# oleg-savchenko/jax_nbody_emulator_with_dj

Hardware: AMD Instinct MI355X
Metric: voxels/sec (disp+vel) on 512^3 box, ndiv=4 (higher is better)
Workload: dtype f32-equivalent: f16x3 split MFMA (3 f16 MFMAs per product, f32 accumulate)

## Files before the change

### include/nbe.h

```cpp
#ifndef NBE_H
#define NBE_H

#include <stddef.h>
#include <stdint.h>

#ifdef __cplusplus
extern "C" {
#endif

typedef struct nbe_ctx nbe_ctx;

typedef void (*nbe_progress_cb)(int done, int total, void* user);

typedef struct nbe_layer_desc {
    const char* block;
    const char* layer;
    int cout, cin, k;
    const float* weight;
    const float* bias;
    const float* style_weight;
    const float* style_bias;
    const float* dweight;
} nbe_layer_desc;

// ... 172 lines not shown
                          double tail_slope, double tail_intercept, double boxsize, double scale, uint64_t seed, int flags,
                          int max_blocks, void* stream);
int nbe_spectrum_colour(void* spectrum, int64_t n, const void* k_table, const void* pk_table, int ntable,
                        double tail_slope, double tail_intercept, double boxsize, double scale, void* stream);
int nbe_gaussian_filter(void* spectrum, int64_t n, double sigma_over_L, void* stream);
int nbe_block_average(const void* src, int64_t n_in, void* dst, int64_t n_out, void* stream);
int nbe_trilinear_upsample(const void* src, int64_t n_in, void* dst, int64_t n_out, void* stream);

#define NBE_VELOCITY_BITS 20
#define NBE_VELOCITY_SUMS 6
int nbe_velocity_words(const void* velocity, int dtype, int lattice, int64_t count, int exponent, const void* sorted,
                       int max_blocks, void* words, void* stream);
int nbe_pair_velocity(const void* sortedA, const void* keysA, const void* wordsA, int64_t countA, const void* sortedB,
                      const void* keysB, const void* wordsB, int64_t countB, int ncell, const int64_t* thresholds, int nbins,
                      int max_blocks, void* sums, void* stream);
int nbe_pair_velocity_form(const void* sortedA, const void* keysA, const void* wordsA, int64_t countA, const void* sortedB,
                           const void* keysB, const void* wordsB, int64_t countB, int ncell, const int64_t* thresholds,
                           int nbins, int max_blocks, int form, void* sums, void* stream);
int nbe_halo_velocity_profiles(const void* sortedA, const void* keysA, const void* wordsA, int64_t countA, const void* sortedB,
                               const void* keysB, const void* wordsB, int64_t countB, int ncell, const int64_t* thresholds,
                               int nbins, int max_blocks, void* sums, void* stream);
int nbe_halo_velocity_profiles_form(const void* sortedA, const void* keysA, const void* wordsA, int64_t countA,
                                    const void* sortedB, const void* keysB, const void* wordsB, int64_t countB, int ncell,
                                    const int64_t* thresholds, int nbins, int max_blocks, int form, void* sums, void* stream);

#define NBE_PROFILE_WAVE_CENTRES 4096
#define NBE_PROFILE_WAVE_BELOW 3000
int nbe_halo_profiles(const void* sortedA, const void* keysA, int64_t countA, const void* sortedB, const void* keysB,
                      int64_t countB, int ncell, const int64_t* thresholds, int nbins, int max_blocks, void* counts,
                      void* stream);
int nbe_halo_profiles_form(const void* sortedA, const void* keysA, int64_t countA, const void* sortedB, const void* keysB,
                           int64_t countB, int ncell, const int64_t* thresholds, int nbins, int max_blocks, int form,
                           void* counts, void* stream);


int nbe_test_layer(nbe_ctx* ctx, int kind, int crop, int flags, const float* x, const float* dx, int cin,
                   int D, int H, int W, const float* w, const float* dw, const float* bias, int cout,
                   const float* res, const float* dres, float* y, float* dy);
int nbe_test_layer_gauged(nbe_ctx* ctx, int flags, const float* x, const float* dx, int cin, int D, int H, int W,
                          const float* w, const float* beta, const float* bias, int cout, float* y, float* dy);
int nbe_test_layer_gauged_res(nbe_ctx* ctx, int flags, const float* x, const float* dx, int cin, int D, int H, int W,
                              const float* w, const float* beta, const float* bias, int cout, const float* res,
                              const float* dres, float* y, float* dy);
enum { NBE_PATH_SKIP_FUSED = 1,
       NBE_PATH_TWO_SOURCE = 2,
       NBE_PATH_WINO_0 = 4,
       NBE_PATH_WINO_1 = 8,
       NBE_PATH_NARROW = 16,
       NBE_PATH_UP8 = 32,
       NBE_PATH_SKIP_NODX = 64,
       NBE_PATH_TWO_SOURCE_SKIP = 128   };
int nbe_test_block(nbe_ctx* ctx, const char* block, int pad, int two_source, const float* x, const float* dx, int D, int H, int W,
                   const float* x2, const float* dx2, float* y, float* dy, float* h, float* dh, float* gauges, int* paths);
int nbe_test_modulate(nbe_ctx* ctx, const float* weight, const float* style_weight, const float* style_bias,
                      int cout, int cin, int k, float s0, float s1, float eps, int first_layer,
                      float* w_n, float* dw_tot);

int nbe_probe_begin(nbe_ctx* ctx, const int64_t origin[3], int nout);
int nbe_probe_slots(nbe_ctx* ctx);
int nbe_probe_layout(nbe_ctx* ctx, int slot, char* name, int name_cap, int dims[3], int64_t* word_offset);
int nbe_probe_read(nbe_ctx* ctx, void* words, int64_t nwords);
int nbe_probe_end(nbe_ctx* ctx);

int nbe_profile_enable(nbe_ctx* ctx, int on);
int nbe_profile_reset(nbe_ctx* ctx);
int nbe_profile_count(nbe_ctx* ctx);
int nbe_profile_entry(nbe_ctx* ctx, int i, char* name, int name_cap, double* ms, int64_t* launches, double* flops);
int64_t nbe_workspace_bytes(nbe_ctx* ctx);
int nbe_debug_phase_cycles(nbe_ctx* ctx, double* out16);

#ifdef __cplusplus
}
#endif
#endif
```

### jax_nbody_emulator_with_dj_amd/_lib.py

```python

import ctypes as C
import os
import subprocess

_HERE = os.path.dirname(os.path.abspath(__file__))
LIB_PATH = os.environ.get("NBE_LIB") or os.path.join(_HERE, "libnbe.so")
CSRC = os.path.join(_HERE, "csrc")
SOURCES = ("nbe_kernels.hip", "nbe_kernels_h3.hip", "nbe_density.hip", "nbe_lpt.hip", "nbe_fof.hip", "nbe_pairs.hip",
           "nbe_profiles.hip", "nbe_pairvel.hip", "nbe_engine.cpp", "nbe_engine_net.cpp", "nbe_engine_weights.cpp", "nbe_engine_box.cpp", "nbe_engine_brick.cpp",
           "nbe_engine_probe.cpp", "nbe_engine_test.cpp")


class NBEError(RuntimeError):
    pass


class NBERangeError(NBEError):
    """A call on an f16-based context produced non-finite values from a finite input (include/nbe.h, "Range")."""


class LayerDesc(C.Structure):
    _fields_ = [
        ("block", C.c_char_p), ("layer", C.c_char_p),
        ("cout", C.c_int), ("cin", C.c_int), ("k", C.c_int),
# ... 84 lines not shown
    "nbe_pair_coords": (C.c_int, [C.c_void_p, C.c_int, C.c_int64, C.c_double, C.c_int, C.c_int, C.c_void_p, C.c_void_p,
                                  C.c_void_p, C.c_void_p]),
    "nbe_pair_count": (C.c_int, [C.c_void_p, C.c_void_p, C.c_int64, C.c_void_p, C.c_void_p, C.c_int64, C.c_int,
                                 C.POINTER(C.c_int64), C.c_int, C.c_int, C.c_int, C.c_int, C.c_void_p, C.c_void_p]),
    "nbe_pair_count_form": (C.c_int, [C.c_void_p, C.c_void_p, C.c_int64, C.c_void_p, C.c_void_p, C.c_int64, C.c_int,
                                      C.POINTER(C.c_int64), C.c_int, C.c_int, C.c_int, C.c_int, C.c_int, C.c_void_p,
                                      C.c_void_p]),
    "nbe_halo_profiles": (C.c_int, [C.c_void_p, C.c_void_p, C.c_int64, C.c_void_p, C.c_void_p, C.c_int64, C.c_int,
                                    C.POINTER(C.c_int64), C.c_int, C.c_int, C.c_void_p, C.c_void_p]),
    "nbe_halo_profiles_form": (C.c_int, [C.c_void_p, C.c_void_p, C.c_int64, C.c_void_p, C.c_void_p, C.c_int64, C.c_int,
                                         C.POINTER(C.c_int64), C.c_int, C.c_int, C.c_int, C.c_void_p, C.c_void_p]),
    "nbe_velocity_words": (C.c_int, [C.c_void_p, C.c_int, C.c_int, C.c_int64, C.c_int, C.c_void_p, C.c_int, C.c_void_p,
                                     C.c_void_p]),
    "nbe_pair_velocity": (C.c_int, [C.c_void_p, C.c_void_p, C.c_void_p, C.c_int64, C.c_void_p, C.c_void_p, C.c_void_p,
                                    C.c_int64, C.c_int, C.POINTER(C.c_int64), C.c_int, C.c_int, C.c_void_p, C.c_void_p]),
    "nbe_pair_velocity_form": (C.c_int, [C.c_void_p, C.c_void_p, C.c_void_p, C.c_int64, C.c_void_p, C.c_void_p, C.c_void_p,
                                         C.c_int64, C.c_int, C.POINTER(C.c_int64), C.c_int, C.c_int, C.c_int, C.c_void_p,
                                         C.c_void_p]),
    "nbe_halo_velocity_profiles": (C.c_int, [C.c_void_p, C.c_void_p, C.c_void_p, C.c_int64, C.c_void_p, C.c_void_p,
                                             C.c_void_p, C.c_int64, C.c_int, C.POINTER(C.c_int64), C.c_int, C.c_int,
                                             C.c_void_p, C.c_void_p]),
    "nbe_halo_velocity_profiles_form": (C.c_int, [C.c_void_p, C.c_void_p, C.c_void_p, C.c_int64, C.c_void_p, C.c_void_p,
                                                  C.c_void_p, C.c_int64, C.c_int, C.POINTER(C.c_int64), C.c_int, C.c_int,
                                                  C.c_int, C.c_void_p, C.c_void_p]),
    "nbe_zeldovich_spectrum": (C.c_int, [C.c_void_p, C.c_int64, C.c_double, C.c_double, C.c_void_p, C.c_void_p]),
    "nbe_divergence_spectrum": (C.c_int, [C.c_void_p, C.c_int64, C.c_double, C.c_void_p, C.c_void_p]),
    "nbe_lpt2_hessian_spectrum": (C.c_int, [C.c_void_p, C.c_int64, C.c_int, C.c_int, C.c_void_p, C.c_int, C.c_void_p]),
    "nbe_lpt2_source": (C.c_int, [C.c_void_p, C.c_int64, C.c_void_p, C.c_int, C.c_void_p]),
    "nbe_lpt2_spectrum": (C.c_int, [C.c_void_p, C.c_void_p, C.c_int64, C.c_double, C.c_double, C.c_double, C.c_void_p,
                                    C.c_int, C.c_void_p]),
    "nbe_spectrum_resize": (C.c_int, [C.c_void_p, C.c_int64, C.c_void_p, C.c_int64, C.c_int, C.c_void_p]),
    "nbe_spectrum_inject": (C.c_int, [C.c_void_p, C.c_int64, C.c_void_p, C.c_int64, C.c_void_p, C.c_void_p, C.c_int,
                                      C.c_double, C.c_double, C.c_double, C.c_uint64, C.c_void_p]),
    "nbe_gaussian_spectrum": (C.c_int, [C.c_void_p, C.c_int64, C.c_void_p, C.c_void_p, C.c_int, C.c_double, C.c_double,
                                        C.c_double, C.c_double, C.c_uint64, C.c_int, C.c_int, C.c_void_p]),
    "nbe_spectrum_colour": (C.c_int, [C.c_void_p, C.c_int64, C.c_void_p, C.c_void_p, C.c_int, C.c_double, C.c_double,
                                      C.c_double, C.c_double, C.c_void_p]),
    "nbe_gaussian_filter": (C.c_int, [C.c_void_p, C.c_int64, C.c_double, C.c_void_p]),
    "nbe_block_average": (C.c_int, [C.c_void_p, C.c_int64, C.c_void_p, C.c_int64, C.c_void_p]),
    "nbe_trilinear_upsample": (C.c_int, [C.c_void_p, C.c_int64, C.c_void_p, C.c_int64, C.c_void_p]),
    "nbe_growth_factor": (C.c_double, [C.c_double, C.c_double]),
    "nbe_vel_norm": (C.c_double, [C.c_double, C.c_double]),
    "nbe_test_layer": (C.c_int, [C.c_void_p, C.c_int, C.c_int, C.c_int, C.c_void_p, C.c_void_p, C.c_int,
                                 C.c_int, C.c_int, C.c_int, C.c_void_p, C.c_void_p, C.c_void_p, C.c_int,
                                 C.c_void_p, C.c_void_p, C.c_void_p, C.c_void_p]),
    "nbe_test_layer_gauged": (C.c_int, [C.c_void_p, C.c_int, C.c_void_p, C.c_void_p, C.c_int, C.c_int, C.c_int, C.c_int,
                                        C.c_void_p, C.c_void_p, C.c_void_p, C.c_int, C.c_void_p, C.c_void_p]),
    "nbe_test_layer_gauged_res": (C.c_int, [C.c_void_p, C.c_int, C.c_void_p, C.c_void_p, C.c_int, C.c_int, C.c_int, C.c_int,
                                            C.c_void_p, C.c_void_p, C.c_void_p, C.c_int, C.c_void_p, C.c_void_p, C.c_void_p,
                                            C.c_void_p]),
    "nbe_test_block": (C.c_int, [C.c_void_p, C.c_char_p, C.c_int, C.c_int, C.c_void_p, C.c_void_p, C.c_int, C.c_int, C.c_int,
                                 C.c_void_p, C.c_void_p, C.c_void_p, C.c_void_p, C.c_void_p, C.c_void_p, C.c_void_p,
                                 C.POINTER(C.c_int)]),
    "nbe_test_modulate": (C.c_int, [C.c_void_p, C.c_void_p, C.c_void_p, C.c_void_p, C.c_int, C.c_int, C.c_int,
                                    C.c_float, C.c_float, C.c_float, C.c_int, C.c_void_p, C.c_void_p]),
    "nbe_probe_begin": (C.c_int, [C.c_void_p, C.POINTER(C.c_int64), C.c_int]),
    "nbe_probe_slots": (C.c_int, [C.c_void_p]),
    "nbe_probe_layout": (C.c_int, [C.c_void_p, C.c_int, C.c_char_p, C.c_int, C.POINTER(C.c_int), C.POINTER(C.c_int64)]),
    "nbe_probe_read": (C.c_int, [C.c_void_p, C.c_void_p, C.c_int64]),
    "nbe_probe_end": (C.c_int, [C.c_void_p]),
    "nbe_profile_enable": (C.c_int, [C.c_void_p, C.c_int]),
    "nbe_profile_reset": (C.c_int, [C.c_void_p]),
    "nbe_profile_count": (C.c_int, [C.c_void_p]),
    "nbe_profile_entry": (C.c_int, [C.c_void_p, C.c_int, C.c_char_p, C.c_int, C.POINTER(C.c_double),
                                    C.POINTER(C.c_int64), C.POINTER(C.c_double)]),
    "nbe_workspace_bytes": (C.c_int64, [C.c_void_p]),
    "nbe_debug_phase_cycles": (C.c_int, [C.c_void_p, C.POINTER(C.c_double)]),
}

_lib = None


def _source_files():
    return [f for f in sorted(os.listdir(CSRC)) if f.endswith((".hip", ".cpp", ".h"))]


def source_hash():
    import hashlib
    h = hashlib.sha256()
    for f in _source_files():
        h.update(f.encode())
        h.update(open(os.path.join(CSRC, f), "rb").read())
    return h.hexdigest()[:16]


def build(force=False, verbose=False):
    srcs = [os.path.join(CSRC, s) for s in SOURCES]
    deps = [os.path.join(CSRC, f) for f in _source_files()] + [os.path.join(_HERE, "..", "include", "nbe.h")]
    if not force and os.path.exists(LIB_PATH):
        if all(os.path.getmtime(LIB_PATH) >= os.path.getmtime(d) for d in deps):
            return LIB_PATH
    hipcc = os.environ.get("HIPCC", "/opt/rocm/bin/hipcc")
    cmd = [hipcc, "--offload-arch=gfx950", "-O3", "-std=c++17", "-fPIC", "-shared", "-o", LIB_PATH] + srcs
    if os.environ.get("NBE_BUILD_DBG") == "1":
        cmd.insert(1, "-DNBE_DBG=1")
    if verbose:
        print(" ".join(cmd))
    subprocess.run(cmd, check=True)
    return LIB_PATH


def lib():
    global _lib
    if _lib is None:
        if not os.path.exists(LIB_PATH):
            raise NBEError(
                "libnbe.so is missing at %s. Build it with `python -c 'import __graft_entry__ as g; g.build()'` "
                "(hipcc, gfx950). There is no CPU fallback." % LIB_PATH)
        l = C.CDLL(LIB_PATH)
        for name, (res, args) in SIGNATURES.items():
            fn = getattr(l, name)
            fn.restype = res
            fn.argtypes = args
        _lib = l
    return _lib


class _PinnedBlock:

    def __init__(self, ptr, nbytes):
        self.ptr, self.nbytes = ptr, nbytes

    def __del__(self):
        try:
            if self.ptr:
                lib().nbe_host_free(C.c_void_p(self.ptr))
                self.ptr = 0
        except Exception:
            pass


def pinned_empty(shape, dtype):
    import numpy as np
    dtype = np.dtype(dtype)
    n = int(np.prod(shape)) * dtype.itemsize
    ptr = lib().nbe_host_alloc(max(n, 1)) if n >= (1 << 20) else None
    if not ptr:
        return np.empty(shape, dtype)
    blk = _PinnedBlock(int(ptr), n)
    buf = (C.c_char * n).from_address(int(ptr))
    buf._nbe_block = blk
    return np.frombuffer(buf, dtype=dtype, count=int(np.prod(shape))).reshape(shape)


def check(rc):
    if rc != 0:
        msg = lib().nbe_last_error().decode("utf-8", "replace")
        raise (NBERangeError if rc == 2 else NBEError)(msg)
```

### jax_nbody_emulator_with_dj_amd/csrc/nbe_conv_select.h

```cpp
#pragma once
#include "nbe_kernels.h"
#include <algorithm>
#include <cstdio>
#include <string>

namespace nbe {

constexpr int H3_CHUNK = 16;
constexpr int HP_ROWS = 8, HP_COLS = 32;
constexpr int H2_ROWS = 16;
#ifndef NBE_STEM_ROWS
#define NBE_STEM_ROWS 1
#endif
constexpr int ST_ROWS = NBE_STEM_ROWS, ST_COLS = 128 / ST_ROWS;
constexpr int UP_MAXCH = 4;
constexpr int HNZ_MAXCH = 4;
constexpr int HNZ_R = 4;
constexpr int NBE_MAX_WSTAGES = 32;
constexpr int NBE_MAX_WSKIP = 16;
constexpr int H3W_F16_CHUNKS = 2;

enum ConvKernel : int {
    CONV_NONE = 0,
    CONV_STEM,
// ... 59 lines not shown
        if (nskip > 0 && ((nskip & 1) || (ka.s_csplit < nskip && (ka.s_csplit & 1)) || (ka.flags & F_SKIP_NODX))) return false;
        nchunk /= H3W_F16_CHUNKS; nskip /= H3W_F16_CHUNKS; if (csplit < (1 << 29)) csplit /= H3W_F16_CHUNKS;
    }
    if (!ka.ww || (!f16 && (ka.flags & F_RES)) || !h3w_pairs_planes(ka.Dv) || 4 * nchunk > NBE_MAX_WSTAGES || (!novel && !ka.beta)) return false;
    if (nskip > 0 && (!ka.wws || 2 * nskip > NBE_MAX_WSKIP)) return false;
    if (!cout_tiles_ok(ka, ctiles, 64)) return false;
    return std::max(ka.in_pstride, csplit < nchunk ? ka.in2_pstride : 0L) * 16 + 16L * (HP_ROWS + 2) * ka.W < (1L << 32) - (1L << 20);
}

inline ConvKernel conv_select(const PackedW& pw, const ConvKArgs& ka, bool vel, bool has_dx) {
    const int ct = pw.ctiles;
    const bool flat3 = pw.mode == MODE_FLAT3;
    const bool plain = ka.in_off == 0 && ka.osz == 1;
    if (!prec_is_half(pw.prec)) {
        if (!ka.beta) return CONV_MFMA;
        return (flat3 && vel && has_dx) ? CONV_MFMA_G : CONV_NONE;
    }
    const bool split = pw.prec == PREC_F16X3;
    if (ka.stem_w && !(vel && has_dx) && flat3 && plain && !(ka.flags & F_RES) && ka.nskip == 0 && !ka.beta)
        return stem_ok(ka) ? CONV_STEM : CONV_NONE;
    if ((ka.nskip > 0 || ka.csplit < ka.nchunk) && !(ka.beta && split)) {
        if (split && !vel && flat3 && plain) return h3w_ok(ka, ct, true, false) ? CONV_H3W_NOVEL : CONV_NONE;
        if (!split && vel && has_dx && ka.beta && flat3 && plain) return h3w_ok(ka, ct, false, true) ? CONV_H3W_F16 : CONV_NONE;
        return CONV_NONE;
    }
    if (ka.beta) {
        if (!(flat3 && vel && has_dx && plain)) return CONV_NONE;
        if (split) {
            if (pw.cout_t == 16) {
                if (h3nz_ok(ka, ct, pw.cout)) return CONV_H3NZ;
                return h3g_ok(ka, ct, true) ? CONV_H3G_NARROW : CONV_NONE;
            }
            if (h3w_ok(ka, ct, false, false)) return CONV_H3W_F16X3;
            return h3g_ok(ka, ct, false) ? CONV_H3G_WIDE : CONV_NONE;
        }
        if (h3w_ok(ka, ct, false, true)) return CONV_H3W_F16;
        return h2q_ok(ka, ct) ? CONV_H2Q_F16_G : CONV_NONE;
    }
    if (flat3) {
        if (!plain) return CONV_NONE;
        if (split && vel && has_dx) return h3q_ok(ka, ct) ? CONV_H3Q : CONV_NONE;
        if (split && !vel && h3w_ok(ka, ct, true, false)) return CONV_H3W_NOVEL;
        if (split && !vel) return h2q_ok(ka, ct) ? CONV_H2Q_SPLIT : CONV_NONE;
        if (!split && vel && has_dx) return h2q_ok(ka, ct) ? CONV_H2Q_F16 : CONV_NONE;
        return CONV_H3P;
    }
    if (pw.mode == MODE_FLAT1) {
        if (!ka.up8) return CONV_H3_FLAT1;
        return ((vel && has_dx) || !vel) && up8_ok(ka) ? CONV_UP8 : CONV_NONE;
    }
    return CONV_H3_DOWN;
}

inline std::string conv_label(ConvKernel k, const PackedW& pw, bool vel, bool has_dx) {
    const char* m = pw.mode == MODE_FLAT3 ? "FLAT3" : pw.mode == MODE_FLAT1 ? "FLAT1" : "DOWN";
    const bool f16 = pw.prec == PREC_F16;
    char b[96];
    switch (k) {
    case CONV_NONE: return "none";
    case CONV_STEM: return vel ? "stem_h3<FLAT3,vel,nodx>" : "stem_h3<FLAT3,novel>";
    case CONV_UP8: return vel ? "up_h3<8 parities,vel,dx>" : "up_h3<8 parities,novel>";
    case CONV_H3W_F16X3: return "conv_h3w<FLAT3,vel,dx>";
    case CONV_H3W_NOVEL: return "conv_h3w<FLAT3,novel>";
    case CONV_H3W_F16: return "conv_h1w<FLAT3,vel,dx>";
    case CONV_H3G_WIDE: case CONV_H3G_NARROW: case CONV_H3NZ: case CONV_H2Q_F16_G:
        snprintf(b, sizeof b, "%s<%s,vel,dx>", k == CONV_H2Q_F16_G ? "conv_h1g" : conv_is_narrow(k) ? "conv_h3n" : "conv_h3g", m);
        return b;
    case CONV_MFMA_G: snprintf(b, sizeof b, "conv_mfma_g<%s,vel,dx,ni%d>", m, pw.ni); return b;
    case CONV_MFMA:
        snprintf(b, sizeof b, "conv_mfma<%s,%s,%s,ni%d>", m, vel ? "vel" : "novel", (vel && has_dx) ? "dx" : "nodx", pw.ni);
        return b;
    default:
        snprintf(b, sizeof b, "%s<%s,%s,%s>", f16 ? "conv_h1" : "conv_h3", m, vel ? "vel" : "novel", (vel && has_dx) ? "dx" : "nodx");
        return b;
    }
}

}
```

### jax_nbody_emulator_with_dj_amd/csrc/nbe_engine_box.cpp

```cpp
#include "nbe_engine_internal.h"

#include <sched.h>

static int host_threads() {
    static const int n = [] {
        if (const char* e = getenv("NBE_HOST_THREADS")) return std::max(1, atoi(e));
        unsigned hw = std::thread::hardware_concurrency();
        cpu_set_t set;
        if (sched_getaffinity(0, sizeof set, &set) == 0) hw = std::min<unsigned>(hw ? hw : 64, (unsigned)CPU_COUNT(&set));
        return (int)std::max(1u, std::min(hw ? hw : 4u, 16u));
    }();
    return n;
}
template <typename F>
static void parallel_for(int nt, F&& fn) {
    std::vector<std::thread> th;
    for (int i = 1; i < nt; ++i) th.emplace_back([&fn, i, nt] { fn(i, nt); });
    fn(0, nt);
    for (auto& t : th) t.join();
}
static void parallel_memcpy(void* dst, const void* src, size_t bytes) {
    const int nt = bytes < (size_t(8) << 20) ? 1 : host_threads();
    parallel_for(nt, [&](int i, int n) {
        const size_t per = ((bytes + n - 1) / n + 4095) & ~size_t(4095), b = std::min(bytes, per * i), e = std::min(bytes, b + per);
// ... 86 lines not shown
    return look > 0 ? pipe_upload(c, t1, t1 + look) : 0;
}

int pipe_output(nbe_ctx* c, int z, int n, int a1, int a2, int e1, int e2) {
    auto& P = c->pipe;
    if (e1 < 0) e1 = P.O1;
    if (e2 < 0) e2 = P.O2;
    HIPCHK(hipEventRecord(c->ev_down, c->stream));
    HIPCHK(hipStreamWaitEvent(c->down_stream, c->ev_down, 0));
    const int64_t plane = (int64_t)P.O1 * P.O2 * P.esz;
    const bool whole = a1 == 0 && a2 == 0 && e1 == P.O1 && e2 == P.O2;
    for (int f = 0; f < (P.hvel ? 2 : 1); ++f) {
        char* h = f ? P.hvel : P.hdisp;
        char* d = f ? P.dvel : P.ddisp;
        for (int ch = 0; ch < c->out_chan; ++ch) {
            if (whole) {
                const int64_t off = ((int64_t)ch * P.O0 + z) * plane;
                HIPCHK(hipMemcpyAsync(h + off, d + off, (size_t)n * plane, hipMemcpyDeviceToHost, c->down_stream));
            } else {
                hipMemcpy3DParms mp;
                memset(&mp, 0, sizeof mp);
                mp.srcPtr = make_hipPitchedPtr(d, (size_t)P.O2 * P.esz, (size_t)P.O2 * P.esz, (size_t)P.O1);
                mp.dstPtr = make_hipPitchedPtr(h, (size_t)P.O2 * P.esz, (size_t)P.O2 * P.esz, (size_t)P.O1);
                mp.srcPos = make_hipPos((size_t)a2 * P.esz, (size_t)a1, (size_t)ch * P.O0 + z);
                mp.dstPos = mp.srcPos;
                mp.extent = make_hipExtent((size_t)e2 * P.esz, (size_t)e1, (size_t)n);
                mp.kind = hipMemcpyDeviceToHost;
                HIPCHK(hipMemcpy3DAsync(&mp, c->down_stream));
            }
        }
    }
    return 0;
}

static int64_t workspace_need(nbe_ctx* c, int D, int H, int W, int slab, bool pyx, bool pz) {
    const int keep_slab = c->slab; const bool keep_pyx = c->pyx, keep_pz = c->pz;
    c->slab = slab; c->pyx = pyx; c->pz = pz;
    c->dry = true;
    c->arena.reset();
    Tensor tin = talloc(c, c->in_chan, D, H, W), y;
    tin.pad = c->pyx ? 1 : 0;
    HeadOut ho{};
    const int rc = c->slab > 0 ? network_stream(c, tin, ho, c->slab) : network(c, tin, &y);
    c->dry = false;
    c->slab = keep_slab; c->pyx = keep_pyx; c->pz = keep_pz;
    return rc ? -1 : c->arena.high;
}

int ensure_workspace(nbe_ctx* c, int D, int H, int W) {
    const int64_t need = workspace_need(c, D, H, W, c->slab, c->pyx, c->pz);
    if (need < 0) return 1;
    if (need > c->ws_bytes) {
        c->sst.valid = false;
        if (c->ws) { HIPCHK(hipStreamSynchronize(c->stream)); HIPCHK(hipFree(c->ws)); c->ws = nullptr; c->ws_bytes = 0; }
        HIPCHK(hipMalloc((void**)&c->ws, need));
        HIPCHK(hipMemsetAsync(c->ws, 0, need, c->stream));
        c->ws_bytes = need;
    }
    return 0;
}

int run_subbox(nbe_ctx* c, const float* box, int Db, int Hb, int Wb, int o0, int o1, int o2,
                      int D, int H, int W, float Dz, float vel_fac, void* disp, void* velo, int out_dtype,
                      int OD, int OH, int OW, int a0, int a1, int a2) {
    c->sst.valid = false;
    c->arena.reset();
    Tensor tin = talloc(c, c->in_chan, D, H, W), y;
    tin.pad = c->pyx ? 1 : 0;
    if (tin.pad) set_org(tin, 0, 48, 48);
    if (!c->pipe.active && !c->pipe.slabwise)
        launch_gather(box, c->in_chan, Db, Hb, Wb, o0, o1, o2, tin.p, Dz / 6.0f * c->act_scale, c->prec, c->stream);
    const HeadOut ho{disp, velo, out_dtype, OD, OH, OW, a0, a1, a2, Dz, vel_fac};
    if (c->slab > 0) return network_stream(c, tin, ho, c->slab);
    if (network(c, tin, &y)) return 1;
    run_head(c, y, tin, ho, 0);
    return 0;
}

void drop_graphs(nbe_ctx* c) {
    for (auto& kv : c->graphs) {
        if (kv.second.exec) (void)hipGraphExecDestroy(kv.second.exec);
        if (kv.second.graph) (void)hipGraphDestroy(kv.second.graph);
    }
    c->graphs.clear();
}

static int run_tile(nbe_ctx* c, const float* box, int Db, int Hb, int Wb, int o0, int o1, int o2,
                    int D, int H, int W, float Dz, float vel_fac, void* disp, void* velo, int out_dtype,
                    int OD, int OH, int OW, int a0, int a1, int a2) {
    const bool off = getenv("NBE_GRAPH") && atoi(getenv("NBE_GRAPH")) == 0;
    if (off || c->prof || c->prog_cb || c->pipe.active || c->pipe.slabwise || c->dry || c->probe.on)
        return run_subbox(c, box, Db, Hb, Wb, o0, o1, o2, D, H, W, Dz, vel_fac, disp, velo, out_dtype, OD, OH, OW, a0, a1, a2);
    nbe_ctx::GraphKey k;
    memset(&k, 0, sizeof k);
    k.box = box; k.disp = disp; k.velo = velo; k.ws = c->ws;
    const int geo[18] = {Db, Hb, Wb, o0, o1, o2, D, H, W, out_dtype, OD, OH, OW, a0, a1, a2, c->slab, c->prec};
    memcpy(k.geo, geo, sizeof geo);
    k.f[0] = Dz; k.f[1] = vel_fac; k.f[2] = c->act_scale;
    k.epoch = c->epoch; k.flags = (c->pyx ? 1 : 0) | (c->pz ? 2 : 0) | (c->gauge_active ? 4 : 0) | (c->fuse ? 8 : 0) | (wino_env_off() ? 16 : 0);
    nbe_ctx::GraphVal& g = c->graphs[k];
    g.used = ++c->graph_clock;
    if (!g.exec && g.seen++ == 0) {
        if (c->graphs.size() > 16) {
            auto lru = c->graphs.begin();
            for (auto it = c->graphs.begin(); it != c->graphs.end(); ++it) if (it->second.used < lru->second.used) lru = it;
            if (lru->second.exec) (void)hipGraphExecDestroy(lru->second.exec);
            if (lru->second.graph) (void)hipGraphDestroy(lru->second.graph);
            c->graphs.erase(lru);
        }
        return run_subbox(c, box, Db, Hb, Wb, o0, o1, o2, D, H, W, Dz, vel_fac, disp, velo, out_dtype, OD, OH, OW, a0, a1, a2);
    }
    if (!c->ev_g0) { HIPCHK(hipEventCreateWithFlags(&c->ev_g0, hipEventDisableTiming)); HIPCHK(hipEventCreateWithFlags(&c->ev_g1, hipEventDisableTiming)); }
    hipStream_t user = c->stream;
    if (!g.exec) {
        c->stream = c->own_stream;
        hipError_t e = hipStreamBeginCapture(c->own_stream, hipStreamCaptureModeThreadLocal);
        int rc = 0;
        if (e == hipSuccess) {
            rc = run_subbox(c, box, Db, Hb, Wb, o0, o1, o2, D, H, W, Dz, vel_fac, disp, velo, out_dtype, OD, OH, OW, a0, a1, a2);
            e = hipStreamEndCapture(c->own_stream, &g.graph);
            if (e == hipSuccess && !rc) e = hipGraphInstantiate(&g.exec, g.graph, nullptr, nullptr, 0);
        }
        c->stream = user;
        if (rc || e != hipSuccess || !g.exec) {
            (void)hipGetLastError();
            if (g.graph) { (void)hipGraphDestroy(g.graph); g.graph = nullptr; }
            g.exec = nullptr; g.seen = -1000000;
            return run_subbox(c, box, Db, Hb, Wb, o0, o1, o2, D, H, W, Dz, vel_fac, disp, velo, out_dtype, OD, OH, OW, a0, a1, a2);
        }
    }
    if (user != c->own_stream) { HIPCHK(hipEventRecord(c->ev_g0, user)); HIPCHK(hipStreamWaitEvent(c->own_stream, c->ev_g0, 0)); }
    HIPCHK(hipGraphLaunch(g.exec, c->own_stream));
    if (user != c->own_stream) { HIPCHK(hipEventRecord(c->ev_g1, c->own_stream)); HIPCHK(hipStreamWaitEvent(user, c->ev_g1, 0)); }
    ++c->graph_replays;
    return 0;
}

extern "C" {

int nbe_plan_tiles(const int64_t region[3], const int ndiv[3], int max_tile, int out_ndiv[3]) {
    if (!region || !ndiv || !out_ndiv) return fail("null argument");
    bool ok = max_tile > 0;
    for (int a = 0; a < 3 && ok; ++a) {
        if (ndiv[a] < 1 || region[a] < 1) return fail("sizes and ndiv must be positive");
        const int64_t crop = region[a] / ndiv[a];
        if (crop % 8 != 0 || crop * ndiv[a] != region[a]) ok = false;
    }
    for (int a = 0; a < 3; ++a) {
        out_ndiv[a] = ndiv[a];
        if (!ok) continue;
        const int64_t crop = region[a] / ndiv[a];
        int best = 1;
        for (int m = 1; m <= ndiv[a]; ++m)
            if (ndiv[a] % m == 0 && crop * m <= max_tile) best = m;
        out_ndiv[a] = ndiv[a] / best;
    }
    return 0;
}

}

int choose_slab(nbe_ctx* c, int D, int H, int W, int64_t budget, int64_t* need_out, bool pyx, bool pz) {
    const int forced = c->slab_forced;
    int result = -1;
    const int cand[4] = {0, 128, 64, 32};
    for (int i = 0; i < 4 && result < 0; ++i) {
        int S = cand[i];
        if (pyx && S == 0) { if (forced == 0) break; continue; }
        if (forced == 0 && S != 0) break;
        if (forced > 0) { if (i > (pyx ? 1 : 0)) break; S = forced & ~1; }
        if (!pyx && S > 0 && D - 8 <= S) continue;
        const int64_t need = workspace_need(c, D, H, W, S, pyx, pyx && pz);
        if (need >= 0 && need <= budget) { result = S; if (need_out) *need_out = need; }
    }
    return result;
}

static bool choose_schedule(nbe_ctx* c, int e0, int e1, int e2, bool spans_yx, bool whole_z, int64_t budget, bool fallback32) {
    const int D = e0 + 96;
    if (spans_yx && !check_dims_pyx(D, e1 + 2, e2 + 2)) {
        const int sl = choose_slab(c, D, e1 + 2, e2 + 2, budget, nullptr, true, whole_z);
        if (sl > 0) { c->slab = sl; c->pyx = true; c->pz = whole_z; return true; }
// ... 166 lines not shown
        P.hdisp = (char*)disp; P.hvel = c->vel ? (char*)vel : nullptr; P.esz = esz; P.O0 = O0; P.O1 = O1; P.O2 = O2;
        if (!c->up_stream) {
            HIPCHK(hipStreamCreateWithFlags(&c->up_stream, hipStreamNonBlocking));
            HIPCHK(hipStreamCreateWithFlags(&c->down_stream, hipStreamNonBlocking));
            HIPCHK(hipEventCreateWithFlags(&c->ev_up, hipEventDisableTiming));
            HIPCHK(hipEventCreateWithFlags(&c->ev_down, hipEventDisableTiming));
            for (int i = 0; i < nbe_ctx::NSTAGE; ++i) HIPCHK(hipEventCreateWithFlags(&c->stage_free[i], hipEventDisableTiming));
        }
        const int64_t sb = (int64_t)PIPE_CHUNK * S1 * S2 * 4 * c->in_chan;
        if (!P.in_pinned && sb > c->stage_bytes) {
            for (int i = 0; i < nbe_ctx::NSTAGE; ++i) {
                if (c->stage_buf[i]) (void)hipHostFree(c->stage_buf[i]);
                c->stage_buf[i] = nullptr;
                HIPCHK(hipHostMalloc((void**)&c->stage_buf[i], sb, hipHostMallocDefault));
            }
            c->stage_bytes = sb;
        }
    }
    c->last_piped = P.active || P.tiles;
    r.piped = P.active || P.tiles;
    if (!in_dev) {
        if (in_bytes > c->box_in_bytes) { (void)hipFree(c->box_in); c->box_in = nullptr; c->box_in_bytes = 0;
                                          HIPCHK(hipMalloc((void**)&c->box_in, in_bytes)); c->box_in_bytes = in_bytes; }
        if (r.piped) {
            HIPCHK(hipStreamSynchronize(c->stream));
        } else {
            HIPCHK(hipMemcpyAsync(c->box_in, box, in_bytes, hipMemcpyHostToDevice, c->stream));
        }
        r.bd = c->box_in;
    }
    r.dd = (char*)disp; r.vd = (char*)vel;
    if (!out_dev) {
        const int64_t need = out_bytes * (c->vel ? 2 : 1);
        if (need > c->box_out_bytes) { (void)hipFree(c->box_out); c->box_out = nullptr; c->box_out_bytes = 0;
                                       HIPCHK(hipMalloc((void**)&c->box_out, need)); c->box_out_bytes = need; }
        r.dd = c->box_out; r.vd = c->box_out + out_bytes;
        P.ddisp = r.dd; P.dvel = c->vel ? r.vd : nullptr;
    }
    return 0;
}

static int region_tiles(nbe_ctx* c, RegionCall& r) {
    const void* box = r.box; void *disp = r.disp, *vel = r.vel;
    const int64_t *origin = r.origin, *oorigin = r.oorigin;
    const int* order = r.order; const int norder = r.norder; const int* ndiv = r.ndiv;
    const int S0 = r.S0, S1 = r.S1, S2 = r.S2, O0 = r.O0, O1 = r.O1, O2 = r.O2;
    const int c0 = r.c0, c1 = r.c1, c2 = r.c2, hal = r.hal, D = r.D, H = r.H, W = r.W;
    const int64_t out_bytes = r.out_bytes;
    const bool in_dev = r.in_dev, out_dev = r.out_dev, piped = r.piped;
    const float Dz = r.Dz, vel_fac = r.vel_fac;
    const float* bd = r.bd; char *dd = r.dd, *vd = r.vd;
    nbe_progress_cb cb = r.cb; void* user = r.user;
    auto& P = c->pipe;
    if ((r.zero_out || !out_dev) && !piped) {
        HIPCHK(hipMemsetAsync(dd, 0, out_bytes, c->stream));
        if (c->vel) HIPCHK(hipMemsetAsync(vd, 0, out_bytes, c->stream));
    }
    const bool trace = piped && getenv("NBE_PIPE_TRACE") && atoi(getenv("NBE_PIPE_TRACE")) != 0;
    const auto t_start = std::chrono::steady_clock::now();
    auto ms_since = [&]() { return std::chrono::duration<double, std::milli>(std::chrono::steady_clock::now() - t_start).count(); };
    double t_up0 = 0, t_range = 0, t_enq = 0;
    std::unique_ptr<Progress> reporter;
    if (cb) reporter.reset(new Progress(cb, user, c->device));
    struct ProgGuard { nbe_ctx* c; ~ProgGuard() { c->prog = nullptr; c->prog_cb = nullptr; } } prog_guard{c};
    c->prog = reporter.get();
    P.slabwise = P.tiles && c->slab > 0;
    if (piped) {
        P.o0 = -48;
        const int zs = c->pyx && c->pz ? 40 : 0;
        if (P.active || P.slabwise ? pipe_upload(c, zs, zs + std::min(c->slab, PIPE_EDGE) + 8) : pipe_upload(c, 0, D)) return 1;
        t_up0 = ms_since();
        if (prepare_range(c, nullptr, (int64_t)c->in_chan * S0 * S1 * S2, Dz, (const float*)box)) return 1;
        t_range = ms_since();
    } else if (prepare_range(c, bd, (int64_t)c->in_chan * S0 * S1 * S2, Dz)) return 1;
    const int total = ndiv[0] * ndiv[1] * ndiv[2];
    const int n = order ? norder : total;
    for (int k = 0; k < n; ++k) {
        const int idx = order ? order[k] : k;
        if (idx < 0 || idx >= total) return fail("sub-box index %d out of range (0..%d)", idx, total - 1);
        const int a0 = (idx / (ndiv[1] * ndiv[2])) * c0, a1 = ((idx / ndiv[2]) % ndiv[1]) * c1, a2 = (idx % ndiv[2]) * c2;
        c->prog_cb = cb; c->prog_user = user; c->prog_k = k; c->prog_n = n;
        if (P.tiles) {
            P.o0 = a0 - 48; P.o1 = a1 - hal; P.o2 = a2 - hal; P.gz = 0;
            if (!P.slabwise) {
                if (pipe_upload(c, 0, D)) return 1;
                HIPCHK(hipEventRecord(c->ev_up, c->up_stream));
                HIPCHK(hipStreamWaitEvent(c->stream, c->ev_up, 0));
            }
        }
        if (c->probe.on) {
            auto& Pb = c->probe;
            const int ta[3] = {(int)oorigin[0] + a0, (int)oorigin[1] + a1, (int)oorigin[2] + a2}, te[3] = {c0, c1, c2};
            Pb.tile = true;
            for (int d = 0; d < 3; ++d) {
                Pb.o[d] = Pb.p[d] - ta[d];
                if (Pb.o[d] < 0 || Pb.o[d] + Pb.nout > te[d] || Pb.o[d] % 8 != 0) Pb.tile = false;
            }
        }
        if (run_tile(c, bd, S0, S1, S2, (int)origin[0] + a0 - 48, (int)origin[1] + a1 - hal, (int)origin[2] + a2 - hal,
                       D, H, W, Dz, vel_fac, dd, vd, r.out_dtype, O0, O1, O2,
                       (int)oorigin[0] + a0, (int)oorigin[1] + a1, (int)oorigin[2] + a2)) return 1;
        if (P.tiles) {
            if (P.out_async && pipe_output(c, a0, c0, a1, a2, c1, c2)) return 1;
            if (k + 1 < n) {
                const int idn = k + 1;
                P.o0 = (idn / (ndiv[1] * ndiv[2])) * c0 - 48;
                if (pipe_upload(c, 0, D)) return 1;
// ... 118 lines not shown
```

### jax_nbody_emulator_with_dj_amd/csrc/nbe_engine_brick.cpp

```cpp
#include "nbe_engine_internal.h"

static Planes brick_planes(nbe_ctx* c, const Tensor& like, const void* buf, int nplanes) {
    Planes p = like.p;
    p.D = nplanes;
    p.pstride = (p.vox() + 63) & ~int64_t(63);
    p.x = (float*)buf;
    p.dx = c->vel ? (float*)buf + (int64_t)p.G * p.pstride * 4 : nullptr;
    return p;
}
void brick_send(nbe_ctx* c, const Tensor& t, int in, int n, void* lo, void* hi) {
    if (c->dry) return;
    for (int s = 0; s < 2; ++s)
        launch_crop(zview(t, s ? t.p.D - in - n : in, n).p, 0, brick_planes(c, t, s ? hi : lo, n), 0, c->vel, c->stream, 0);
}
void brick_recv(nbe_ctx* c, const Tensor& like, const void* lo, const void* hi, int n, const Tensor& dst, int wrap) {
    if (c->dry) return;
    for (int s = 0; s < 2; ++s) {
        const Planes face = brick_planes(c, like, s ? hi : lo, n), to = zview(dst, s ? dst.p.D - n : 0, n).p;
        if (wrap) launch_wrap_pad(face, to, wrap, c->vel, c->stream, 0);
        else launch_crop(face, 0, to, 0, c->vel, c->stream, 0);
    }
}
static int64_t brick_halo_bytes(nbe_ctx* c, int nplanes, int Hd, int Wd) {
    Planes p; p.G = planes_for(c->mid, c->prec); p.D = nplanes; p.H = Hd; p.W = Wd;
// ... 65 lines not shown
    *D = (int)b0 + 96; *H = (int)S1 + 2; *W = (int)S2 + 2;
    if (check_dims_pyx(*D, *H, *W)) return 1;
    HIPCHK(hipSetDevice(c->device));
    c->pyx = true; c->pz = false; c->zx = true;
    if (c->bp_slab > 0 && c->bp_size[0] == b0 && c->bp_size[1] == S1 && c->bp_size[2] == S2 && c->ws_bytes >= c->bp_need) {
        c->slab = c->bp_slab;
        if (need_out) *need_out = c->bp_need;
        return 0;
    }
    const int64_t budget = plan_budget(c, 0);
    int64_t need = 0;
    const int sl = choose_slab(c, *D, *H, *W, budget < 0 ? INT64_MAX / 4 : budget, &need, true, false);
    if (sl <= 0) { c->zx = false; return fail("brick of %lld x %lld x %lld does not fit the device memory that is free", (long long)b0, (long long)S1, (long long)S2); }
    c->slab = sl;
    c->bp_size[0] = b0; c->bp_size[1] = S1; c->bp_size[2] = S2; c->bp_slab = sl; c->bp_need = need;
    if (need_out) *need_out = need;
    return 0;
}

int64_t nbe_brick_halo_bytes(nbe_ctx* c, const int64_t bsize[3], int which) {
    if (!c || !bsize || which < 0 || which > 3) return -1;
    if (which == 3) return brick_halo_bytes(c, BRICK_H0, (int)bsize[1] + 2, (int)bsize[2] + 2);
    if (which == 0) return (int64_t)c->in_chan * BRICK_RAW * bsize[1] * bsize[2] * 4;
    if (which == 1) return brick_halo_bytes(c, BRICK_H1, (int)bsize[1] / 2, (int)bsize[2] / 2) + 16;
    return brick_halo_bytes(c, BRICK_H2, (int)bsize[1] / 4, (int)bsize[2] / 4);
}

int nbe_brick_plan(nbe_ctx* c, const int64_t bsize[3]) {
    if (!c || !bsize) return 0;
    int D, H, W;
    const int keep_slab = c->slab; const bool kp = c->pyx, kz = c->pz;
    int rc = brick_setup(c, bsize, &D, &H, &W);
    if (!rc) { rc = ensure_workspace(c, D, H, W); if (rc) { c->bp_slab = 0; (void)hipGetLastError(); } }
    const int sl = rc ? 0 : c->slab;
    c->zx = false; c->slab = keep_slab; c->pyx = kp; c->pz = kz;
    (void)nbe_last_error();
    return sl;
}

struct BrickOff { nbe_ctx* c; ~BrickOff() { c->phase = 0; c->zx = false; c->bio.skip_ready = nullptr; c->bio.skip_recv_lo = nullptr; } };

int nbe_brick_encode(nbe_ctx* c, const void* box, const int64_t bsize[3], float Dz, float vel_fac, void* send_lo, void* send_hi,
                     void* skip_send_lo, void* skip_send_hi) {
    if (!c || !box || !send_lo || !send_hi || !skip_send_lo || !skip_send_hi) return fail("null argument");
    if (!is_device_ptr(box) || !is_device_ptr(send_lo) || !is_device_ptr(send_hi) || !is_device_ptr(skip_send_lo) || !is_device_ptr(skip_send_hi))
        return fail("nbe_brick_encode takes device pointers");
    int D, H, W;
    if (brick_setup(c, bsize, &D, &H, &W)) return 1;
    BrickOff off{c};
    if (ensure_workspace(c, D, H, W)) return 1;
    const int Dh = (int)bsize[0] + 2 * BRICK_RAW;
    if (prepare_range(c, (const float*)box, (int64_t)c->in_chan * Dh * bsize[1] * bsize[2], Dz)) return 1;
    c->arena.reset();
    Tensor tin = talloc(c, c->in_chan, D, H, W);
    tin.pad = 1; set_org(tin, 0, 48, 48);
    launch_gather((const float*)box, c->in_chan, Dh, (int)bsize[1], (int)bsize[2], 0, -1, -1, zview(tin, 48 - BRICK_RAW, Dh).p,
                  Dz / 6.0f * c->act_scale, c->prec, c->stream);
    c->phase = 1; c->bio.send_lo = send_lo; c->bio.send_hi = send_hi; c->bio.skip_send_lo = skip_send_lo; c->bio.skip_send_hi = skip_send_hi;
    c->sst.D = D; c->sst.H = H; c->sst.W = W;
    c->sst.Dz = Dz; c->sst.vel_fac = vel_fac; c->sst.act_scale = c->act_scale; c->sst.ws = c->ws;
    const HeadOut ho{nullptr, nullptr, NBE_F32, (int)bsize[0], (int)bsize[1], (int)bsize[2], 0, 0, 0, Dz, vel_fac};
    if (network_stream(c, tin, ho, c->slab)) return 1;
    const int64_t body = brick_halo_bytes(c, BRICK_H1, (int)bsize[1] / 2, (int)bsize[2] / 2);
    unsigned bits; memcpy(&bits, &c->act_scale, 4);
    launch_tag_word((unsigned*)((char*)send_lo + body), bits, nullptr, nullptr, 0, c->stream);
    launch_tag_word((unsigned*)((char*)send_hi + body), bits, nullptr, nullptr, 0, c->stream);
    HIPCHK(hipGetLastError());
    return 0;
}

static int brick_resume(nbe_ctx* c, int phase) {
    if (!c->sst.valid) return fail("brick call without a preceding nbe_brick_encode (or another call has used this context's workspace in between)");
    if (c->sst.ws != c->ws) return fail("the workspace was reallocated since nbe_brick_encode");
    HIPCHK(hipSetDevice(c->device));
    c->pyx = true; c->pz = false; c->zx = true; c->phase = phase;
    return 0;
}

int nbe_brick_interior(nbe_ctx* c) {
    if (!c) return fail("null context");
    if (brick_resume(c, 2)) return 1;
    BrickOff off{c};
    const HeadOut ho{};
    if (network_stream(c, c->sst.tin, ho, c->sst.S)) return 1;
    HIPCHK(hipGetLastError());
    return 0;
}

int nbe_brick_exchange(nbe_ctx* c, const void* recv_lo, const void* recv_hi, void* send2_lo, void* send2_hi) {
    if (!c || !recv_lo || !recv_hi || !send2_lo || !send2_hi) return fail("null argument");
    if (brick_resume(c, 3)) return 1;
    BrickOff off{c};
    c->bio.recv_lo = recv_lo; c->bio.recv_hi = recv_hi; c->bio.send_lo = send2_lo; c->bio.send_hi = send2_hi;
    if (c->flags) {
        const int64_t body = brick_halo_bytes(c, BRICK_H1, (c->sst.H - 2) / 2, (c->sst.W - 2) / 2);
        unsigned bits; memcpy(&bits, &c->sst.act_scale, 4);
        launch_tag_word(nullptr, bits, (const unsigned*)((const char*)recv_lo + body), c->flags + 1, 2u, c->stream);
        launch_tag_word(nullptr, bits, (const unsigned*)((const char*)recv_hi + body), c->flags + 1, 2u, c->stream);
    }
    const HeadOut ho{};
    if (network_stream(c, c->sst.tin, ho, c->sst.S)) return 1;
    HIPCHK(hipGetLastError());
    return 0;
}

int nbe_brick_finish(nbe_ctx* c, const void* recv_lo, const void* recv_hi, const void* skip_recv_lo, const void* skip_recv_hi,
// ... 19 lines not shown
```

### jax_nbody_emulator_with_dj_amd/csrc/nbe_engine_internal.h

```cpp
#pragma once

#include "../../include/nbe.h"
#include "nbe_conv_select.h"

#include <cmath>
#include <cstdarg>
#include <cstdio>
#include <cstdlib>
#include <cstring>
#include <algorithm>
#include <atomic>
#include <chrono>
#include <condition_variable>
#include <deque>
#include <functional>
#include <map>
#include <memory>
#include <mutex>
#include <string>
#include <thread>
#include <vector>

#pragma GCC visibility push(hidden)

// ... 8 lines not shown
    } while (0)

static inline int roundup(int v, int m) { return (v + m - 1) / m * m; }

struct Arena {
    struct Blk { int64_t off, size; bool used; };
    std::vector<Blk> blks;
    int64_t high = 0;
    void reset() { blks.clear(); blks.push_back({0, INT64_MAX / 2, false}); high = 0; }
    int64_t alloc(int64_t bytes) {
        bytes = (bytes + 255) & ~int64_t(255);
        for (size_t i = 0; i < blks.size(); ++i) {
            if (!blks[i].used && blks[i].size >= bytes) {
                Blk rest{blks[i].off + bytes, blks[i].size - bytes, false};
                blks[i].size = bytes; blks[i].used = true;
                if (rest.size > 0) blks.insert(blks.begin() + i + 1, rest);
                if (blks[i].off + bytes > high) high = blks[i].off + bytes;
                return blks[i].off;
            }
        }
        return -1;
    }
    void release(int64_t off) {
        for (size_t i = 0; i < blks.size(); ++i) {
            if (blks[i].off == off && blks[i].used) {
                blks[i].used = false;
                if (i + 1 < blks.size() && !blks[i + 1].used) { blks[i].size += blks[i + 1].size; blks.erase(blks.begin() + i + 1); }
                if (i > 0 && !blks[i - 1].used) { blks[i - 1].size += blks[i].size; blks.erase(blks.begin() + i); }
                return;
            }
        }
    }
};

struct Layer {
    std::string block, layer;
    int cout = 0, cin = 0, k = 0, kind = 0;
    bool first = false;
    float *weight = nullptr, *sw = nullptr, *sb = nullptr;
    float *wn = nullptr, *dwn = nullptr;
    PackedW pw;
    PackedW pwn;
    float* bias0 = nullptr;
    float *alpha = nullptr, *beta = nullptr;
    const float* gout = nullptr;
    const float* a_in = nullptr;
    bool g6 = false;
    const Layer* fskip = nullptr;
    const float* b_sub = nullptr;
    float* bias_f = nullptr;
    float* dwn_f = nullptr;
};

struct Tensor { Planes p; int64_t off = -1; int pad = 0; int org[3] = {0, 0, 0}; };

struct ProfEntry { std::string name; double ms = 0; int64_t launches = 0; double flops = 0; };

struct Progress {
    struct Item { hipEvent_t ev; int done, total; };
    nbe_progress_cb cb; void* user; int device;
    std::thread th; std::mutex mu; std::condition_variable cv; std::deque<Item> q; bool stop = false;
    Progress(nbe_progress_cb cb_, void* user_, int dev) : cb(cb_), user(user_), device(dev) {
        th = std::thread([this] {
            (void)hipSetDevice(device);
            for (;;) {
                Item it;
                {
                    std::unique_lock<std::mutex> lk(mu);
                    cv.wait(lk, [this] { return stop || !q.empty(); });
                    if (q.empty()) return;
                    it = q.front(); q.pop_front();
                }
                (void)hipEventSynchronize(it.ev);
                (void)hipEventDestroy(it.ev);
                cb(it.done, it.total, user);
            }
        });
    }
    void post(hipStream_t s, int done, int total) {
        hipEvent_t ev;
        if (hipEventCreateWithFlags(&ev, hipEventDisableTiming) != hipSuccess) return;
        (void)hipEventRecord(ev, s);
        { std::lock_guard<std::mutex> lk(mu); q.push_back({ev, done, total}); }
        cv.notify_one();
    }
    ~Progress() {
        { std::lock_guard<std::mutex> lk(mu); stop = true; }
        cv.notify_one();
        if (th.joinable()) th.join();
    }
};

struct nbe_ctx {
    int device = 0;
    hipStream_t own_stream = nullptr, stream = nullptr;
    int in_chan = 3, out_chan = 3, mid = 64;
    float eps = 1e-8f;
    bool vel = true;
    bool have_weights = false, style = false, modulated = false;
    float mod_Om = NAN, mod_Dz = NAN;
    std::map<std::string, Layer> layers;
    Arena arena;
    char* ws = nullptr;
    int64_t ws_bytes = 0;
    bool dry = false;
    int slab = 0;
    int slab_forced = -1;
// ... 29 lines not shown
    int* wino_flag = nullptr; bool wino_ok = false;
    bool direct_z = false;
    float act_scale = 1.f;
    float bias_scale = 1.f;
    bool bias_dirty = true;
    float bias_max = 0.f;
    float preset_absmax = -1.f;
    bool input_finite = true;
    bool range_pending = false;
    unsigned* flags = nullptr;
    float* box_in = nullptr; int64_t box_in_bytes = 0;
    char* box_out = nullptr; int64_t box_out_bytes = 0;
    struct HostPipe {
        bool active = false, out_async = false;
        bool tiles = false;
        bool slabwise = false;
        int o1 = 0, o2 = 0;
        const float* hbox = nullptr;
        bool in_pinned = false;
        int C = 0, S0 = 0, S1 = 0, S2 = 0, o0 = 0;
        std::vector<char> up;
        int gz = 0;
        char *hdisp = nullptr, *hvel = nullptr;
        char *ddisp = nullptr, *dvel = nullptr;
        int esz = 4, O0 = 0, O1 = 0, O2 = 0;
        int nstage = 0;
    } pipe;
    bool last_piped = false;
    hipStream_t up_stream = nullptr, down_stream = nullptr;
    static constexpr int NSTAGE = 3;
    char* stage_buf[NSTAGE] = {nullptr, nullptr, nullptr}; int64_t stage_bytes = 0;
    hipEvent_t stage_free[NSTAGE] = {nullptr, nullptr, nullptr};
    hipEvent_t ev_up = nullptr, ev_down = nullptr;
    struct GraphKey {
        const void *box, *disp, *velo, *ws;
        int geo[18]; float f[3]; int epoch, flags;
        bool operator<(const GraphKey& o) const { return memcmp(this, &o, sizeof *this) < 0; }
    };
    struct GraphVal { hipGraphExec_t exec = nullptr; hipGraph_t graph = nullptr; int seen = 0; uint64_t used = 0; };
    std::map<GraphKey, GraphVal> graphs;
    uint64_t graph_clock = 0, graph_replays = 0;
    int epoch = 0;
    hipEvent_t ev_g0 = nullptr, ev_g1 = nullptr;
    struct Probe {
        bool on = false, tile = false;
        int p[3] = {0, 0, 0}, nout = 0;
        int o[3] = {0, 0, 0};
        struct Slot { std::string name; int C, n, nw, level; int64_t off; };
        std::vector<Slot> slots;
        unsigned* bits = nullptr; int64_t words = 0;
        unsigned* count = nullptr;
    } probe;
    int* paths = nullptr;
    bool prof = false;
    std::vector<ProfEntry> prof_entries;
    struct Pending { int entry; hipEvent_t a, b; };
    std::vector<Pending> pending;
    std::vector<hipEvent_t> ev_pool;
};

struct HeadOut { void* disp; void* velo; int out_dtype; int OD, OH, OW, a0, a1, a2; float Dz, vel_fac; };

static constexpr int PIPE_EDGE = 32;

static constexpr int BRICK_H1 = 6, BRICK_H2 = 10;
static constexpr int BRICK_H0 = 4;

bool is_device_ptr(const void* p);
int require_ready(nbe_ctx* c);
int prepare_range(nbe_ctx* c, const float* dev_src, int64_t n, float Dz, const float* host_src = nullptr);
int check_range(nbe_ctx* c);

int planes_for(int C, int prec);
Tensor talloc(nbe_ctx* c, int C, int D, int H, int W, bool zero_rest = true);
Tensor tallocp(nbe_ctx* c, int C, int D, int Hi, int Wi, int pad, bool zero_rest = true);
void fill_halo(nbe_ctx* c, const Tensor& t);
void tfree(nbe_ctx* c, Tensor& t);
Tensor zview(const Tensor& t, int z0, int nz);
void set_org(Tensor& t, int z, int y, int x);
bool wino_f16_layer(int prec, bool vel, int cin_pad);
bool wino_env_off();
bool up8_launch(const nbe_ctx* c, const Layer& L, bool has_dx);
int run_conv(nbe_ctx* c, const Layer& L, const ConvLaunch& cl_in, bool has_dx);
const Layer* find_layer(nbe_ctx* c, const char* block, const char* layer);
bool block_fused(const nbe_ctx* c, const Layer* L1, int nres);
bool two_source_width(const nbe_ctx* c);
Tensor alloc_hidden(nbe_ctx* c, int cmid, int nz, const Tensor& x, bool fused);
int resblock_part(nbe_ctx* c, const char* name, const Tensor& x, const Tensor& h, const Tensor& s,
                  int js, int ns, int jh, int nh, bool has_dx, bool final_act, const int* zr, const Tensor* x2 = nullptr,
                  bool halo_s = true);
int resblock(nbe_ctx* c, const char* name, const Tensor& x, bool has_dx, bool final_act, int cout, int cmid, Tensor* out,
             Tensor* hidden_out = nullptr, const int* zr = nullptr, const Tensor* x2 = nullptr);
int down_conv(nbe_ctx* c, const Layer& L, const Tensor& x, Tensor& o, bool probe, const int* zr = nullptr);
int downblock(nbe_ctx* c, const char* name, const Tensor& x, Tensor* out);
int upblock(nbe_ctx* c, const char* name, const Tensor& x, const Tensor& cat, int xcrop = 0, int g0 = -1);
void crop_into(nbe_ctx* c, const Tensor& src, int crop, const Tensor& dst, int cz = -1);
int check_dims(int D, int H, int W);
int check_dims_pyx(int D, int H, int W);
void run_head(nbe_ctx* c, const Tensor& y, const Tensor& xin, const HeadOut& h, int zoff);
int network(nbe_ctx* c, const Tensor& tin, Tensor* yout);
int network_stream(nbe_ctx* c, const Tensor& tin, const HeadOut& ho, int S);

PackedW layer_geometry(int prec, int kind, int cout, int cin);
bool packs_narrow(int prec, bool vel, const Layer& L);
bool packs_wino(int prec, bool vel, const Layer& L);
bool packs_wino_skip(int prec, bool vel, bool style, const Layer& L);
bool packs_stem(int prec, const Layer& L);
int alloc_wino(PackedW& pw);
int alloc_stem(PackedW& pw);
int wino_flag_round_trip(nbe_ctx* c, const std::function<void()>& packs);
void release_layer(Layer& L);
void free_layers(nbe_ctx* c);
int pack_wino(nbe_ctx* c);

unsigned host_absmax_bits(const float* x, int64_t n);
int pipe_input(nbe_ctx* c, const Tensor& tin, int t0, int t1, int look, float scale);
int pipe_output(nbe_ctx* c, int z, int n, int a1 = 0, int a2 = 0, int e1 = -1, int e2 = -1);
int ensure_workspace(nbe_ctx* c, int D, int H, int W);
int run_subbox(nbe_ctx* c, const float* box, int Db, int Hb, int Wb, int o0, int o1, int o2,
               int D, int H, int W, float Dz, float vel_fac, void* disp, void* velo, int out_dtype,
               int OD, int OH, int OW, int a0, int a1, int a2);
void drop_graphs(nbe_ctx* c);
int64_t plan_budget(nbe_ctx* c, int64_t reserve);
int choose_slab(nbe_ctx* c, int D, int H, int W, int64_t budget, int64_t* need_out, bool pyx = false, bool pz = false);

void brick_send(nbe_ctx* c, const Tensor& t, int in, int n, void* lo, void* hi);
void brick_recv(nbe_ctx* c, const Tensor& like, const void* lo, const void* hi, int n, const Tensor& dst, int wrap);
int brick_interior(nbe_ctx* c, nbe_ctx::StreamState& st);
int brick_edges(nbe_ctx* c, nbe_ctx::StreamState& st);
int brick_level2(nbe_ctx* c, nbe_ctx::StreamState& st, Tensor* t_out);

void probe_act(nbe_ctx* c, const Layer& L, const Planes& out, int g0, const int org[3], int ez, int ey, int ex, bool periodic,
               const int* zr = nullptr);
int prof_entry(nbe_ctx* c, const std::string& name);
hipEvent_t get_event(nbe_ctx* c);
void prof_collect(nbe_ctx* c);

#pragma GCC visibility pop
```

### jax_nbody_emulator_with_dj_amd/csrc/nbe_engine_net.cpp

```cpp
#include "nbe_engine_internal.h"

int planes_for(int C, int prec) { return roundup(C, 16) / (prec == PREC_F16 ? 8 : 4); }

static Planes ws_planes(nbe_ctx* c, int G, int D, int H, int W, int64_t* off_out) {
    Planes p;
    p.G = G; p.D = D; p.H = H; p.W = W;
    p.pstride = (p.vox() + 63) & ~int64_t(63);
    const int64_t one = (int64_t)G * p.pstride * 16;
    const int64_t slack = ((int64_t)2 * H * W + 2 * W + 1024) * 16;
    const int64_t off = c->arena.alloc(one * (c->vel ? 2 : 1) + slack);
    *off_out = off;
    if (!c->dry) {
        p.x = (float*)(c->ws + off);
        p.dx = c->vel ? (float*)(c->ws + off + one) : nullptr;
    }
    return p;
}

Tensor talloc(nbe_ctx* c, int C, int D, int H, int W, bool zero_rest) {
    Tensor t;
    t.p = ws_planes(c, planes_for(C, c->prec), D, H, W, &t.off);
    const int gw = c->prec == PREC_F16 ? (C + 7) / 8 : c->prec == PREC_F16X3 ? 2 * ((C + 7) / 8) : (C + 3) / 4;
    if (zero_rest && !c->dry && t.off >= 0 && gw < t.p.G) {
        const size_t off = (size_t)gw * t.p.pstride * 4, bytes = (size_t)(t.p.G - gw) * t.p.pstride * 16;
        launch_zero(t.p.x + off, (int64_t)bytes, c->stream);
        if (t.p.dx) launch_zero(t.p.dx + off, (int64_t)bytes, c->stream);
    }
    return t;
}
Tensor tallocp(nbe_ctx* c, int C, int D, int Hi, int Wi, int pad, bool zero_rest) {
    Tensor t = talloc(c, C, D, Hi + 2 * pad, Wi + 2 * pad, zero_rest);
    t.pad = pad;
    return t;
}
static Planes inner(const Tensor& t) {
    Planes p = t.p;
    const int64_t sh = (int64_t)t.pad * (t.p.W + 1) * 4;
    if (p.x) p.x += sh;
    if (p.dx) p.dx += sh;
    return p;
}
void fill_halo(nbe_ctx* c, const Tensor& t) {
    if (t.pad > 0 && !c->dry) launch_fill_yx(t.p, t.pad, c->vel, c->stream);
}
void tfree(nbe_ctx* c, Tensor& t) { if (t.off >= 0) c->arena.release(t.off); t.off = -1; }
Tensor zview(const Tensor& t, int z0, int nz) {
    Tensor v = t;
    v.off = -1;
    const int64_t sh = (int64_t)z0 * t.p.H * t.p.W * 4;
    if (v.p.x) v.p.x += sh;
    if (v.p.dx) v.p.dx += sh;
    v.p.D = nz;
    v.org[0] += z0;
    return v;
}
static void org_conv(const Tensor& x, int nconv, int out[3]) {
    const int p = x.pad ? nconv : 0;
    out[0] = x.org[0]; out[1] = x.org[1] - p; out[2] = x.org[2] - p;
}
void set_org(Tensor& t, int z, int y, int x) { t.org[0] = z; t.org[1] = y; t.org[2] = x; }

bool wino_f16_layer(int prec, bool vel, int cin_pad) {
    return prec == PREC_F16 && vel && cin_pad % (H3_CHUNK * H3W_F16_CHUNKS) == 0 && h3w_stages_fit(cin_pad, H3W_F16_CHUNKS);
}
bool wino_env_off() { return getenv("NBE_WINO") && atoi(getenv("NBE_WINO")) == 0; }
bool up8_launch(const nbe_ctx* c, const Layer& L, bool has_dx) { return prec_is_half(c->prec) && (!c->vel || has_dx) && up8_fits(L.pw.cin_pad); }

int run_conv(nbe_ctx* c, const Layer& L, const ConvLaunch& cl_in, bool has_dx) {
    if (c->dry) return 0;
    ConvLaunch cl = cl_in;
    const bool g6 = c->gauge_active && L.g6 && has_dx;
    const bool nov = !c->vel && c->prec == PREC_F16X3 && L.kind == 0 && L.pw.ww && c->wino_ok;
    if (c->gauge_active) { cl.gout = L.gout; cl.beta = g6 ? L.beta : nullptr; }
    if (cl.skw) {
        if (!((g6 || nov) && c->fuse && L.fskip)) return fail("internal error: fused skip requested for %s/%s", L.block.c_str(), L.layer.c_str());
        cl.bias = L.bias_f;
    }
    const PackedW& pw = (g6 && L.kind == 0 && L.pwn.w) ? L.pwn : L.pw;
    cl.wino = c->wino_ok && !c->direct_z && !wino_env_off();
    hipEvent_t ea = nullptr, eb = nullptr;
    if (c->prof) {
        ea = get_event(c); eb = get_event(c);
        (void)hipEventRecord(ea, c->stream);
    }
    ConvKernel k;
    if (launch_conv(pw, cl, c->vel, has_dx, c->stream, &k))
        return fail("internal error: no kernel for layer %s/%s (mode %d, gauged %d, input tangent %d, crop offset %ld, output stride %d, selected %s)",
                    L.block.c_str(), L.layer.c_str(), L.pw.mode, (int)g6, (int)has_dx, (long)cl.in_off, cl.osz, conv_kernel_name(k));
    if (c->paths)
        *c->paths |= (cl.skw ? NBE_PATH_SKIP_FUSED : 0) | (cl.skw && (cl.flags & F_SKIP_NODX) ? NBE_PATH_SKIP_NODX : 0) |
                     (cl.csplit_ch ? NBE_PATH_TWO_SOURCE : 0) | (cl.skw && cl.sk_split_ch ? NBE_PATH_TWO_SOURCE_SKIP : 0) |
                     (conv_is_wino(k) ? (L.layer == "conv_1" ? NBE_PATH_WINO_1 : NBE_PATH_WINO_0) : 0) |
                     (conv_is_narrow(k) ? NBE_PATH_NARROW : 0) | (k == CONV_UP8 ? NBE_PATH_UP8 : 0);
    if (c->prof) {
        (void)hipEventRecord(eb, c->stream);
        std::string pn = conv_label(k, pw, c->vel, has_dx);
        static const bool per_layer = getenv("NBE_PROF_LAYERS") && atoi(getenv("NBE_PROF_LAYERS")) == 1;
        if (per_layer) pn += " " + L.block + "/" + L.layer;
        const int pe = prof_entry(c, pn);
        c->pending.push_back({pe, ea, eb});
        const double nout = (double)cl.Dv * cl.Hv * cl.Wv * (cl.set < 0 ? 8.0 : 1.0);
        const int taps = L.kind == 0 ? 27 : L.kind == 2 ? 8 : 1;
        const double gemms = c->vel ? ((has_dx && !g6) ? 3.0 : 2.0) : 1.0;
        c->prof_entries[pe].flops += 2.0 * nout * L.cout * L.cin * taps * gemms;
        if (cl.skw) c->prof_entries[pe].flops += 2.0 * nout * L.cout * L.fskip->cin * (!c->vel ? 1.0 : (cl.flags & F_SKIP_NODX) ? 2.0 : 3.0);
        c->prof_entries[pe].launches += 1;
        if (c->pending.size() > 4096) prof_collect(c);
    }
    return 0;
}

const Layer* find_layer(nbe_ctx* c, const char* block, const char* layer) {
    auto it = c->layers.find(std::string(block) + "/" + layer);
    return it == c->layers.end() ? nullptr : &it->second;
}


static constexpr int L1_CTX = BRICK_H1, L2_CTX = BRICK_H2;

static bool wino_only_fuse(const nbe_ctx* c) { return !c->vel || c->prec == PREC_F16; }
bool block_fused(const nbe_ctx* c, const Layer* L1, int nres) {
    return c->fuse && L1->fskip != nullptr && (!wino_only_fuse(c) || (!c->direct_z && !wino_env_off() && h3w_pairs_planes(nres)));
}

bool two_source_width(const nbe_ctx* c) { return c->mid % two_source_chunk(c->prec) == 0; }

Tensor alloc_hidden(nbe_ctx* c, int cmid, int nz, const Tensor& x, bool fused) {
    const int pad = x.pad, sy = pad ? 0 : 2;
    if (fused && !pad) return talloc(c, cmid, nz, x.p.H, x.p.W);
    return tallocp(c, cmid, nz, x.p.H - 2 * pad - sy, x.p.W - 2 * pad - sy, pad);
}

int resblock_part(nbe_ctx* c, const char* name, const Tensor& x, const Tensor& h, const Tensor& s,
                         int js, int ns, int jh, int nh, bool has_dx, bool final_act, const int* zr, const Tensor* x2, bool halo_s) {
    const Layer *Ls = find_layer(c, name, "skip"), *L0 = find_layer(c, name, "conv_0"), *L1 = find_layer(c, name, "conv_1");
    if (!Ls || !L0 || !L1) return fail("missing layers of block %s", name);
    const int H = x.p.H, W = x.p.W, pad = x.pad;
    const bool fused = block_fused(c, L1, ns);
    if (fused && (h.p.H != H || h.p.W != W)) return fail("internal: hidden tensor of fused block %s lacks the input's pitch", name);
    if (x2 && (!fused || x2->p.H != H || x2->p.W != W || x2->pad != pad)) return fail("internal: two-source input of block %s", name);
    const Tensor sv = zview(s, js, ns), hv = zview(h, jh, nh);
    const Tensor xs = zview(x, js, ns + 4);
    const int64_t sk_off = (2L * H + (pad ? pad : 2)) * W + (pad ? pad : 2);
    if (!fused) {
        ConvLaunch cl; cl.in = xs.p; cl.in_off = sk_off;
        cl.Dv = ns; cl.Hv = s.p.H - 2 * pad; cl.Wv = s.p.W - 2 * pad; cl.out = inner(sv); cl.flags = 0;
        if (run_conv(c, *Ls, cl, has_dx)) return 1;
    }
    int og[3];
    {
        ConvLaunch cl; cl.in = zview(x, jh, nh + 2).p; cl.Dv = nh; cl.Hv = H - 2; cl.Wv = W - 2; cl.out = inner(hv); cl.flags = F_ACT;
        if (x2) { cl.in2 = zview(*x2, jh, nh + 2).p; cl.csplit_ch = c->mid; }
        if (run_conv(c, *L0, cl, has_dx)) return 1;
        org_conv(x, 1, og); og[0] += jh;
        const int zh[3] = {zr ? zr[0] : 0, zr ? zr[1] + 2 : 0, zr ? zr[2] : 0};
        probe_act(c, *L0, cl.out, 0, og, cl.Dv, cl.Hv, cl.Wv, pad != 0, zr ? zh : nullptr);
    }
    fill_halo(c, hv);
    {
        ConvLaunch cl; cl.in = zview(h, js, ns + 2).p; cl.Dv = ns; cl.Hv = s.p.H - 2 * pad; cl.Wv = s.p.W - 2 * pad; cl.out = inner(sv);
        if (fused) { cl.sk = xs.p; cl.sk_off = sk_off; cl.skw = L1->pwn.w ? &Ls->pwn : &Ls->pw; cl.flags = (final_act ? F_ACT : 0) | (has_dx ? 0 : F_SKIP_NODX);
                     if (x2) { cl.sk2 = zview(*x2, js, ns + 4).p; cl.sk_split_ch = c->mid; } }
        else { cl.res = inner(sv); cl.flags = F_RES | (final_act ? F_ACT : 0); }
        if (run_conv(c, *L1, cl, true)) return 1;
        org_conv(x, 2, og); og[0] += js;
        if (final_act) probe_act(c, *L1, cl.out, 0, og, cl.Dv, cl.Hv, cl.Wv, pad != 0, zr);
    }
    if (halo_s) fill_halo(c, sv);
    return 0;
}

int resblock(nbe_ctx* c, const char* name, const Tensor& x, bool has_dx, bool final_act, int cout, int cmid, Tensor* out,
                    Tensor* hidden_out, const int* zr, const Tensor* x2) {
    const Layer* L1 = find_layer(c, name, "conv_1");
    if (!L1) return fail("missing layers of block %s", name);
    const int D = x.p.D, pad = x.pad;
    const int sy = pad ? 0 : 2;
    Tensor s = tallocp(c, cout, D - 4, x.p.H - 2 * pad - 2 * sy, x.p.W - 2 * pad - 2 * sy, pad);
    Tensor h = alloc_hidden(c, cmid, D - 2, x, block_fused(c, L1, D - 4));
    if (s.off < 0 || h.off < 0) return fail("workspace exhausted in block %s", name);
    if (resblock_part(c, name, x, h, s, 0, D - 4, 0, D - 2, has_dx, final_act, zr, x2)) return 1;
    tfree(c, h);
    if (hidden_out) *hidden_out = h;
    int og[3];
    org_conv(x, 2, og);
    set_org(s, og[0], og[1], og[2]);
    *out = s;
    return 0;
}

static void carry_planes(nbe_ctx* c, const Tensor& t, int src, int dst, int n) {
    if (c->dry || n <= 0) return;
    launch_crop(zview(t, src, n).p, 0, zview(t, dst, n).p, 0, c->vel, c->stream, 0);
}

int down_conv(nbe_ctx* c, const Layer& L, const Tensor& x, Tensor& o, bool probe, const int* zr) {
    ConvLaunch cl; cl.in = inner(x); cl.Dv = o.p.D; cl.Hv = o.p.H - 2 * o.pad; cl.Wv = o.p.W - 2 * o.pad; cl.out = inner(o); cl.flags = F_ACT;
    if (run_conv(c, L, cl, true)) return 1;
    set_org(o, x.org[0] / 2, x.org[1] / 2, x.org[2] / 2);
    if (probe) probe_act(c, L, cl.out, 0, o.org, cl.Dv, cl.Hv, cl.Wv, x.pad != 0, zr);
    return 0;
}

static void wrap_z(nbe_ctx* c, const Tensor& t, int cz) {
    const int own = t.p.D - 2 * cz;
    for (int done = 0; done < cz; done += own) {
        const int n = std::min(own, cz - done);
        carry_planes(c, t, cz - done - n + own, cz - done - n, n);
        carry_planes(c, t, cz + done, cz + own + done, n);
    }
}

int downblock(nbe_ctx* c, const char* name, const Tensor& x, Tensor* out) {
    const Layer* L = find_layer(c, name, "conv_0");
    if (!L) return fail("missing layer %s/conv_0", name);
    Tensor o = talloc(c, c->mid, x.p.D / 2, x.p.H / 2, x.p.W / 2);
    if (o.off < 0) return fail("workspace exhausted in %s", name);
    if (down_conv(c, *L, x, o, true)) return 1;
    *out = o;
    return 0;
}

static int mid_planes(const nbe_ctx* c) { return c->mid / (c->prec == PREC_F16 ? 8 : 4); }

int upblock(nbe_ctx* c, const char* name, const Tensor& x, const Tensor& cat, int xcrop, int g0) {
    const Layer* L = find_layer(c, name, "conv_0");
    if (!L) return fail("missing layer %s/conv_0", name);
    xcrop += x.pad;
    const int Hx = x.p.H - 2 * xcrop, Wx = x.p.W - 2 * xcrop;
    if (cat.p.D != 2 * x.p.D || cat.p.H - 2 * cat.pad != 2 * Hx || cat.p.W - 2 * cat.pad != 2 * Wx)
        return fail("internal: concat geometry mismatch in %s", name);
    const bool up8 = up8_launch(c, *L, true);
    const int out_g0 = g0 >= 0 ? g0 : mid_planes(c);
    for (int p = 0; p < (up8 ? 1 : 8); ++p) {
        ConvLaunch cl; cl.in = x.p; cl.in_off = ((int64_t)xcrop * x.p.W + xcrop);
        cl.Dv = x.p.D; cl.Hv = Hx; cl.Wv = Wx; cl.out = inner(cat);
        cl.out_g0 = out_g0; cl.osz = 2; cl.oz = (p >> 2) & 1; cl.oy = (p >> 1) & 1; cl.ox = p & 1;
        cl.flags = F_ACT; cl.set = up8 ? -1 : p;
        if (run_conv(c, *L, cl, true)) return 1;
    }
    const int xc = xcrop - x.pad;
    const int og[3] = {2 * x.org[0], 2 * (x.org[1] + xc), 2 * (x.org[2] + xc)};
    probe_act(c, *L, inner(cat), out_g0, og, 2 * x.p.D, 2 * Hx, 2 * Wx, cat.pad != 0);
    return 0;
}

void crop_into(nbe_ctx* c, const Tensor& src, int crop, const Tensor& dst, int cz) {
    if (c->dry) return;
    Planes s = src.p; s.G = mid_planes(c);
    launch_crop(s, crop, dst.p, 0, c->vel, c->stream, cz);
}

int check_dims(int D, int H, int W) {
    const int v[3] = {D, H, W};
    for (int i = 0; i < 3; ++i)
        if (v[i] < 104 || v[i] % 8 != 0)
            return fail("input spatial size %d unsupported: each of (D,H,W) must be >= 104 and a multiple of 8 "
                        "(all-VALID U-Net with three 2x levels, receptive-field crop 48)", v[i]);
    return 0;
}

void run_head(nbe_ctx* c, const Tensor& y, const Tensor& xin, const HeadOut& h, int zoff) {
    if (c->dry) return;
    const float inv_s = 1.0f / c->act_scale;
    HeadScale hs;
    hs.k_disp = 6.0f * inv_s; hs.k_dy = h.vel_fac * 6.0f * inv_s; hs.k_x0 = h.vel_fac * 6.0f / h.Dz * inv_s;
    hs.bad = c->flags ? (int*)(c->flags + 1) : nullptr;
    launch_head(y.p, xin.p, 48, c->out_chan, hs, c->vel, h.disp, h.velo, h.out_dtype, h.OD, h.OH, h.OW,
                h.a0 + zoff, h.a1, h.a2, c->prec, c->stream, y.pad);
}

static int stream_encode(nbe_ctx* c, const Tensor& tin, const HeadOut& ho, int S, Tensor* skip0_out, Tensor* td_out) {
    const int m = c->mid, pad = tin.pad;
    const int D = tin.p.D, H = tin.p.H, W = tin.p.W;
    const int Hi = H - 2 * pad, Wi = W - 2 * pad;
    const int Y = D - 8;
    const bool zx = pad && c->zx;
    const bool pz = pad && (c->pz || zx);
    const int zlo = pz ? (zx ? 44 : 40) : 0, zhi = pz ? (zx ? Y - 44 : Y - 40) : Y;
    Tensor skip0 = pad ? tallocp(c, m, Y - 80, Hi, Wi, pad) : talloc(c, m, Y - 80, H - 88, W - 88);
    const int cz1 = (pz && !zx) ? L1_CTX : 0, dpad = (pad && !zx) ? 1 : 0;
    const int D1 = pz ? (D - 96) / 2 : Y / 2;
    Tensor td = pad ? tallocp(c, m, D1 + 2 * cz1, Hi / 2, Wi / 2, dpad) : talloc(c, m, Y / 2, (H - 8) / 2, (W - 8) / 2);
    if (skip0.off < 0 || td.off < 0) return fail("workspace exhausted (level 0)");
    const Layer* Ld = find_layer(c, "down_l0", "conv_0");
    if (!Ld) return fail("missing layer down_l0/conv_0");
    const int sy = pad ? 0 : 2;
    const Layer* L00 = find_layer(c, "conv_l00", "conv_1");
    if (!L00) return fail("missing layer conv_l00/conv_1");
    Tensor h0 = alloc_hidden(c, m, S + 6, tin, block_fused(c, L00, S + 4)), a = tallocp(c, m, S + 4, Hi - 2 * sy, Wi - 2 * sy, pad);
    const Layer *L01 = find_layer(c, "conv_l01", "conv_1"), *Lr00 = find_layer(c, "conv_r00", "conv_1"), *Lr01 = find_layer(c, "conv_r01", "conv_1");
    if (!L01 || !Lr00 || !Lr01) return fail("missing conv_1 layers of the level-0 blocks");
    Tensor h1 = alloc_hidden(c, m, S + 2, a, block_fused(c, L01, S));
    Tensor y0r = pz ? Tensor() : tallocp(c, m, S, Hi - 4 * sy, Wi - 4 * sy, pad);
    if (h0.off < 0 || a.off < 0 || h1.off < 0 || (!pz && y0r.off < 0)) return fail("workspace exhausted (level-0 encoder slabs)");
    const int zr00[3] = {zlo, zhi + 4, pz ? D - 96 : 0}, zr01[3] = {zlo, zhi, pz ? D - 96 : 0};
    for (int z = zlo, n = 0; z < zhi; z += n) {
        n = std::min(((c->pipe.active || c->pipe.slabwise) && z == zlo) ? std::min(S, PIPE_EDGE) : S, zhi - z);
        const int n_next = std::min(S, zhi - (z + n));
        const bool first = z == zlo;
        Tensor y0 = pz ? zview(skip0, z - 40, n) : zview(y0r, 0, n);
        if ((c->pipe.active || c->pipe.slabwise) && !c->dry && pipe_input(c, tin, z, z + n + 8, n_next, ho.Dz / 6.0f * c->act_scale)) return 1;
        { int og[3]; org_conv(zview(tin, z, n + 8), 2, og); set_org(a, og[0], og[1], og[2]);
          org_conv(a, 2, og); set_org(y0, og[0], og[1], og[2]); }
        if (first) {
            if (resblock_part(c, "conv_l00", zview(tin, z, n + 8), h0, a, 0, n + 4, 0, n + 6, false, true, zr00)) return 1;
            if (resblock_part(c, "conv_l01", a, h1, y0, 0, n, 0, n + 2, true, true, zr01)) return 1;
        } else {
            if (resblock_part(c, "conv_l00", zview(tin, z, n + 8), h0, a, 4, n, 6, n, false, true, zr00)) return 1;
            if (resblock_part(c, "conv_l01", a, h1, y0, 0, n, 2, n, true, true, zr01)) return 1;
        }
        if (z + n < zhi) {
            carry_planes(c, h0, n, 0, 6);
            carry_planes(c, a, n, 0, 4);
            carry_planes(c, h1, n, 0, 2);
        }
        const int i0 = std::max(0, 40 - z), i1 = std::min(n, Y - 40 - z);
        if (!pz && i1 > i0) crop_into(c, y0, pad ? 0 : 40, zview(skip0, z + i0 - 40, i1 - i0), i0);
        {
            const int d0 = pz ? std::max(z, 44) : z, d1 = pz ? std::min(z + n, Y - 44) : z + n;
            if (d1 > d0) {
                const Tensor tv = zview(td, cz1 + (d0 - (pz ? 44 : 0)) / 2, (d1 - d0) / 2);
                Tensor yv = zview(y0, d0 - z, d1 - d0);
                ConvLaunch cl; cl.in = inner(yv); cl.Dv = tv.p.D; cl.Hv = tv.p.H - 2 * dpad; cl.Wv = tv.p.W - 2 * dpad; cl.out = inner(tv); cl.flags = F_ACT;
                if (run_conv(c, *Ld, cl, true)) return 1;
                const int og[3] = {yv.org[0] / 2, yv.org[1] / 2, yv.org[2] / 2};
                const int zd[3] = {22, 22 + (D - 96) / 2, pz ? (D - 96) / 2 : 0};
                probe_act(c, *Ld, cl.out, 0, og, cl.Dv, cl.Hv, cl.Wv, pad != 0, zd);
            }
        }
    }
    tfree(c, h0); tfree(c, a); tfree(c, h1);
    if (!pz) tfree(c, y0r);
    set_org(skip0, 0, pad ? 4 : 0, pad ? 4 : 0);
    set_org(td, pz ? 22 - cz1 : 0, pad ? 22 : 0, pad ? 22 : 0);
    *skip0_out = skip0; *td_out = td;
    return 0;
}

static int stream_level1(nbe_ctx* c, int pad, bool pz, Tensor td, Tensor* cat1_out, Tensor* y1_out, Tensor* t_out) {
    const int m = c->mid;
    Tensor t = td, y1, cat1;
    *y1_out = Tensor();
    if (!pad) {
        if (resblock(c, "conv_l1", t, true, true, m, m, &y1)) return 1;
        tfree(c, t);
        cat1 = talloc(c, 2 * m, y1.p.D - 32, y1.p.H - 32, y1.p.W - 32);
        if (cat1.off < 0) return fail("workspace exhausted (cat1)");
        crop_into(c, y1, 16, cat1);
        if (downblock(c, "down_l1", y1, &t)) return 1;
        tfree(c, y1);
        *cat1_out = cat1; *t_out = t;
        return 0;
    }
    const int cz1 = pz ? L1_CTX : 0, cz2 = pz ? L2_CTX : 0;
    fill_halo(c, zview(t, cz1, t.p.D - 2 * cz1));
    wrap_z(c, t, cz1);
    const int zr1[3] = {t.org[0], t.org[0] + t.p.D - 4, t.p.D - 2 * cz1};
    if (resblock(c, "conv_l1", t, true, true, m, m, &y1, nullptr, pz ? zr1 : nullptr)) return 1;
    tfree(c, t);

    const int zc = pz ? 0 : 16;
    const Layer *Lr1 = find_layer(c, "conv_r1", "conv_1"), *Ld1 = find_layer(c, "down_l1", "conv_0");
    if (!Lr1 || !Ld1) return fail("missing layer conv_r1/conv_1 or down_l1/conv_0");
    const bool two = block_fused(c, Lr1, y1.p.D - 2 * zc - 4) && two_source_width(c);
    if (!two) {
        cat1 = tallocp(c, 2 * m, y1.p.D - 2 * zc, y1.p.H - 2, y1.p.W - 2, 1);
        if (cat1.off < 0) return fail("workspace exhausted (cat1)");
        crop_into(c, y1, 0, cat1, zc);
        set_org(cat1, y1.org[0] + zc - 16, y1.org[1] - 16, y1.org[2] - 16);
    }
    Tensor y1d = pz ? zview(y1, 4, y1.p.D - 8) : y1;
    t = talloc(c, m, y1d.p.D / 2 + 2 * cz2, (y1.p.H - 2) / 2 + 2 * L2_CTX, (y1.p.W - 2) / 2 + 2 * L2_CTX);
    if (t.off < 0) return fail("workspace exhausted (level 2 input)");
    Tensor tp = zview(t, cz2, y1d.p.D / 2);
    tp.pad = L2_CTX;
    const int zd[3] = {y1d.org[0] / 2, y1d.org[0] / 2 + tp.p.D, tp.p.D};
    if (down_conv(c, *Ld1, y1d, tp, true, pz ? zd : nullptr)) return 1;
    fill_halo(c, tp);
    wrap_z(c, t, cz2);
    set_org(t, tp.org[0] - cz2, tp.org[1] - L2_CTX, tp.org[2] - L2_CTX);
    if (two) *y1_out = y1; else tfree(c, y1);
    *cat1_out = cat1; *t_out = t;
    return 0;
}

static int lower_levels(nbe_ctx* c, Tensor t, Tensor cat1, Tensor y1, Tensor* r_out) {
    const int m = c->mid;
    Tensor y2, cat2, r;
    if (resblock(c, "conv_l2", t, true, true, m, m, &y2)) return 1;
    tfree(c, t);
    cat2 = talloc(c, 2 * m, y2.p.D - 8, y2.p.H - 8, y2.p.W - 8);
    if (cat2.off < 0) return fail("workspace exhausted (cat2)");
    crop_into(c, y2, 4, cat2);
    if (downblock(c, "down_l2", y2, &t)) return 1;
    tfree(c, y2);

    c->direct_z = true;
    const int rc = resblock(c, "conv_c", t, true, true, m, m, &r);
    c->direct_z = false;
    if (rc) return 1;
    tfree(c, t);

    if (upblock(c, "up_r2", r, cat2)) return 1;
    tfree(c, r);
    if (resblock(c, "conv_r2", cat2, true, true, m, 2 * m, &r)) return 1;
    tfree(c, cat2);

    const bool two = y1.off >= 0;
    Tensor sk;
    if (two) {
        cat1 = tallocp(c, m, 2 * r.p.D, y1.p.H - 2, y1.p.W - 2, 1);
        if (cat1.off < 0) return fail("workspace exhausted (up_r1)");
        sk = zview(y1, (y1.p.D - 2 * r.p.D) / 2, 2 * r.p.D);
        set_org(sk, sk.org[0] - 16, y1.org[1] - 16, y1.org[2] - 16);
        set_org(cat1, sk.org[0], sk.org[1], sk.org[2]);
    }
    if (upblock(c, "up_r1", r, cat1, cat1.pad ? 2 : 0, two ? 0 : -1)) return 1;
    fill_halo(c, cat1);
    tfree(c, r);
    if (resblock(c, "conv_r1", two ? sk : cat1, true, true, m, 2 * m, r_out, nullptr, nullptr, two ? &cat1 : nullptr)) return 1;
    tfree(c, cat1);
    if (two) tfree(c, y1);
    return 0;
}

int network(nbe_ctx* c, const Tensor& tin, Tensor* yout) {
    const int m = c->mid;
    Tensor a, y0, t, cat0, cat1, y1, r;
    if (resblock(c, "conv_l00", tin, false, true, m, m, &a)) return 1;
    if (resblock(c, "conv_l01", a, true, true, m, m, &y0)) return 1;
    tfree(c, a);
    cat0 = talloc(c, 2 * m, y0.p.D - 80, y0.p.H - 80, y0.p.W - 80);
    if (cat0.off < 0) return fail("workspace exhausted (cat0)");
    crop_into(c, y0, 40, cat0);
    if (downblock(c, "down_l0", y0, &t)) return 1;
    tfree(c, y0);

    if (stream_level1(c, 0, false, t, &cat1, &y1, &t)) return 1;
    if (lower_levels(c, t, cat1, y1, &r)) return 1;

    if (upblock(c, "up_r0", r, cat0)) return 1;
    tfree(c, r);
    if (resblock(c, "conv_r00", cat0, true, true, m, 2 * m, &r)) return 1;
    tfree(c, cat0);

    if (resblock(c, "conv_r01", r, true, false, c->out_chan, m, yout)) return 1;
    tfree(c, r);
    return 0;
}

static int stream_tail(nbe_ctx* c, const Tensor& tin, const HeadOut& ho, int S, Tensor skip0, Tensor cat1, Tensor y1, Tensor t) {
    const int m = c->mid, pad = tin.pad;
    const int sy = pad ? 0 : 2;
    const Layer *Lr00 = find_layer(c, "conv_r00", "conv_1"), *Lr01 = find_layer(c, "conv_r01", "conv_1");
    if (!Lr00 || !Lr01) return fail("missing conv_1 layers of the level-0 blocks");
    Tensor r;
    if (lower_levels(c, t, cat1, y1, &r)) return 1;
    if (2 * r.p.D != skip0.p.D || 2 * (r.p.H - 2 * r.pad) != skip0.p.H - 2 * pad || 2 * (r.p.W - 2 * r.pad) != skip0.p.W - 2 * pad)
        return fail("internal: level-0 concat geometry mismatch");

    if (pad && c->zx && !c->dry && c->bio.skip_recv_lo) {
        if (c->bio.skip_ready) HIPCHK(hipStreamWaitEvent(c->stream, c->bio.skip_ready, 0));
        brick_recv(c, skip0, c->bio.skip_recv_lo, c->bio.skip_recv_hi, BRICK_H0, skip0, 0);
    }
    const int Yo = skip0.p.D - 8;
    const int Hs = skip0.p.H - 2 * pad, Ws = skip0.p.W - 2 * pad;
    const bool two = block_fused(c, Lr00, S + 4) && two_source_width(c);
    Tensor cat = tallocp(c, two ? m : 2 * m, S + 8, Hs, Ws, pad), hq = alloc_hidden(c, 2 * m, S + 6, cat, block_fused(c, Lr00, S + 4));
    Tensor q = tallocp(c, m, S + 4, Hs - 2 * sy, Ws - 2 * sy, pad), hy = alloc_hidden(c, m, S + 2, q, block_fused(c, Lr01, S));
    Tensor y = tallocp(c, c->out_chan, S, Hs - 4 * sy, Ws - 4 * sy, pad, false);
    if (cat.off < 0 || hq.off < 0 || q.off < 0 || hy.off < 0 || y.off < 0) return fail("workspace exhausted (level-0 decoder slabs)");
    for (int z = 0, n = 0; z < Yo; z += n) {
        n = std::min(S, Yo - z);
        if (c->pipe.active && c->pipe.out_async && Yo - z > PIPE_EDGE && Yo - z - n < PIPE_EDGE)
            n = Yo - z - PIPE_EDGE;
        const bool first = z == 0;
        const int c0 = first ? 0 : 8, cn = first ? n + 8 : n;
        set_org(cat, skip0.org[0] + z, skip0.org[1], skip0.org[2]);
        { int og[3]; org_conv(cat, 2, og); set_org(q, og[0], og[1], og[2]); }
        if (!two && !c->dry) launch_crop(zview(skip0, z + c0, cn).p, 0, zview(cat, c0, cn).p, 0, c->vel, c->stream, 0);
        if (upblock(c, "up_r0", zview(r, (z + c0) / 2, cn / 2), zview(cat, c0, cn), 0, two ? 0 : -1)) return 1;
        fill_halo(c, zview(cat, c0, cn));
        const Tensor sk = two ? zview(skip0, z, std::min(S + 8, skip0.p.D - z)) : cat;
        const Tensor* up2 = two ? &cat : nullptr;
        if (first) {
            if (resblock_part(c, "conv_r00", sk, hq, q, 0, n + 4, 0, n + 6, true, true, nullptr, up2)) return 1;
            if (resblock_part(c, "conv_r01", q, hy, y, 0, n, 0, n + 2, true, false, nullptr, nullptr, false)) return 1;
        } else {
            if (resblock_part(c, "conv_r00", sk, hq, q, 4, n, 6, n, true, true, nullptr, up2)) return 1;
            if (resblock_part(c, "conv_r01", q, hy, y, 0, n, 2, n, true, false, nullptr, nullptr, false)) return 1;
        }
        if (z + n < Yo) {
            carry_planes(c, cat, n, 0, 8);
            carry_planes(c, hq, n, 0, 6);
            carry_planes(c, q, n, 0, 4);
            carry_planes(c, hy, n, 0, 2);
        }
        run_head(c, zview(y, 0, n), zview(tin, z, n + 96), ho, z);
        if (c->pipe.active && c->pipe.out_async && !c->dry && pipe_output(c, z, n)) return 1;
        if (c->prog && !c->dry && z + n < Yo)
            c->prog->post(c->pipe.active && c->pipe.out_async ? c->down_stream : c->stream,
                          c->prog_k * 1000 + (int)(1000L * (z + n) / Yo), c->prog_n * 1000);
    }
    tfree(c, cat); tfree(c, hq); tfree(c, q); tfree(c, hy); tfree(c, y);
    tfree(c, r); tfree(c, skip0);
    return 0;
}

static void stash_arena(nbe_ctx* c) { c->sst.blks = c->arena.blks; c->sst.high = c->arena.high; }

int network_stream(nbe_ctx* c, const Tensor& tin, const HeadOut& ho, int S) {
    auto& st = c->sst;
    const int pad = tin.pad;
    const bool zx = pad && c->zx;
    if (c->phase >= 2) {
        if (!st.valid || st.stage != c->phase - 1) return fail("brick calls out of order (encode, interior, exchange, finish) or the context was used in between");
        c->arena.blks = st.blks; c->arena.high = st.high;
    }
    if (c->phase <= 1) {
        if (stream_encode(c, tin, ho, S, &st.skip0, &st.td)) return 1;
        st.tin = tin; st.S = S;
        if (c->phase == 1) {
            brick_send(c, st.td, 0, BRICK_H1, c->bio.send_lo, c->bio.send_hi);
            brick_send(c, st.skip0, BRICK_H0, BRICK_H0, c->bio.skip_send_lo, c->bio.skip_send_hi);
            st.valid = true; st.stage = 1; stash_arena(c);
            return 0;
        }
    }
    if (!zx) {
        Tensor cat1, y1, t;
        if (stream_level1(c, pad, pad && c->pz, st.td, &cat1, &y1, &t)) return 1;
        return stream_tail(c, tin, ho, S, st.skip0, cat1, y1, t);
    }
    if (c->phase == 0 || c->phase == 2) {
        if (brick_interior(c, st)) return 1;
// ... 20 lines not shown
```

### jax_nbody_emulator_with_dj_amd/csrc/nbe_kernels.h

```cpp
#pragma once
#include <hip/hip_runtime.h>
#include <stdint.h>

namespace nbe {

struct Planes {
    float* x = nullptr;
    float* dx = nullptr;
    int64_t pstride = 0;
    int G = 0;
    int D = 0, H = 0, W = 0;
    int64_t vox() const { return (int64_t)D * H * W; }
};

enum Precision { PREC_F32 = 0, PREC_F16X3 = 1, PREC_F16 = 2 };
inline constexpr bool prec_is_half(int prec) { return prec == PREC_F16X3 || prec == PREC_F16; }
inline constexpr int prec_parts(int prec) { return prec == PREC_F16X3 ? 2 : 1; }
constexpr float H3_SCALE = 2048.0f, H3_INV = 1.0f / 2048.0f;
constexpr int H3_RANGE_UP = 6;

constexpr int NBE_MAX_GROUPS = 64;

enum ConvMode { MODE_FLAT3 = 0, MODE_FLAT1 = 1, MODE_DOWN = 2 };
enum ConvFlags { F_ACT = 1, F_RES = 2, F_SKIP_NODX = 4 };

constexpr int TILE_VOX = 256;
inline constexpr int mode_taps(int mode) { return mode == MODE_FLAT3 ? 3 : 1; }
inline constexpr int mode_nseg(int mode) { return mode == MODE_FLAT3 ? 9 : (mode == MODE_DOWN ? 8 : 1); }
inline constexpr int mode_ck(int mode) { return mode == MODE_FLAT3 ? 8 : 16; }
inline constexpr int prec_ck(int prec, int mode) { return prec_is_half(prec) ? 16 : mode_ck(mode); }

struct PackedW {
    float* w = nullptr;
    float* dw = nullptr;
    float* bias = nullptr;
    int prec = PREC_F32;
    int mode = 0, ni = 2;
    int cout_t = 64;
    int cin = 0, cout = 0;
    int cin_pad = 0;
    int ctiles = 0;
    int64_t floats = 0;
    int nsets = 1;
    float* ww = nullptr;
    float* stem = nullptr;
};

struct ConvLaunch {
    Planes in;
    int64_t in_off = 0;
    int Dv = 0, Hv = 0, Wv = 0;
    Planes out;
    int out_g0 = 0;
    int osz = 1, oz = 0, oy = 0, ox = 0;
    Planes res;
    int flags = 0;
    int set = 0;
    const float* gout = nullptr;
    const float* beta = nullptr;
    const float* bias = nullptr;
    Planes in2;
    int csplit_ch = 0;
    Planes sk, sk2;
    int sk_split_ch = 0;
    int64_t sk_off = 0;
    const PackedW* skw = nullptr;
    bool wino = false;
};

struct ConvGroupSrc { const char* x; const char* dx; const char* w; long psb; };

struct ConvKArgs {
    const float* x; const float* dx; long in_pstride;
    int D, H, W; long P; long in_off;
    int Dv, Hv, Wv; long Q;
    float* y; float* dy; long out_pstride; int out_g0;
    int Ho, Wo; int osz, oz, oy, ox;
    const float* r; const float* dr; long res_pstride;
    const float* bias; const float* w; const float* dw;
    int nchunk; int cout_groups; int flags; int ntiles;
    int tny, tnx;
    int zrun;
    const float* gout;
    const float* beta;
    const float* x2; const float* dx2; long in2_pstride; int csplit;
    const float* xs; const float* dxs; long s_pstride; const float* xs2; const float* dxs2; long s2_pstride; int s_csplit;
    const float* ws; const float* dws; int nskip;
    long dws_delta;
    int up8; long set_stride;
    const float* wws; long wws_set_floats;
    const float* ww;
    const float* stem_w;
    ConvGroupSrc gs[NBE_MAX_GROUPS];
};

enum ConvKernel : int;
int launch_conv(const PackedW& pw, const ConvLaunch& L, bool vel, bool has_dx, hipStream_t s, ConvKernel* ran = nullptr);

void launch_modulate(const float* weight, const float* style_weight, const float* style_bias,
                     int cout, int cin, int k3, float s0, float s1, float eps, int first_layer,
                     float* w_n, float* dw_tot , hipStream_t s,
                     const float* a_in = nullptr, float* beta_out = nullptr, const float* b_sub = nullptr);
void launch_style_alpha(const float* style_weight, const float* style_bias, int cin, float s0, float s1,
                        float* alpha, int* flag, hipStream_t s);
void launch_pack(const float* w_oidhw, int cout, int cin, int kind, const PackedW& pw, float* dst, hipStream_t s);

void launch_pack_h3w(const float* w_oidhw, int cout, int cin, int cin_pad, int ctiles, float* dst, int* flag, hipStream_t s,
                     int prec = PREC_F16X3);
void launch_pack_h3w_skip(const float* w_oidhw, int cout, int cin, const PackedW& pw, float* dst, int* flag, hipStream_t s);

void launch_gather(const float* box, int C, int Db, int Hb, int Wb, int a0, int a1, int a2,
                   const Planes& dst, float scale, int prec, hipStream_t s);
void launch_to_planes(const float* src, int C, const Planes& dst, bool tangent, float scale, int prec, hipStream_t s);
void launch_from_planes(const Planes& src, bool tangent, int C, float* dst, int prec, hipStream_t s);
void launch_crop(const Planes& src, int c, const Planes& dst, int g0, bool vel, hipStream_t s, int cz = -1);
struct HeadScale { float k_disp = 6.f, k_dy = 0.f, k_x0 = 0.f; int* bad = nullptr; };
void launch_head(const Planes& y, const Planes& xin, int c0, int C, const HeadScale& hs, bool vel,
                 void* disp, void* velo, int out_dtype, int Db, int Hb, int Wb, int a0, int a1, int a2,
                 int prec, hipStream_t s, int pad = 0);
void launch_absmax(const float* src, int64_t n, unsigned* out_bits, hipStream_t s);
void launch_zero(void* dst, int64_t bytes, hipStream_t s);
void launch_scale(const float* src, float* dst, int n, float f, hipStream_t s, const float* src2 = nullptr);

void launch_fill_yx(const Planes& t, int pad, bool vel, hipStream_t s);
void launch_wrap_pad(const Planes& src, const Planes& dst, int pad, bool vel, hipStream_t s, int padz = 0);

void launch_tag_word(unsigned* dst, unsigned v, const unsigned* expect_at, unsigned* flag, unsigned bit, hipStream_t s);

struct ProbeLaunch {
    const float* x; int64_t pstride; int H, W, g0, prec, C;
// ... 11 lines not shown
```

### jax_nbody_emulator_with_dj_amd/csrc/nbe_kernels.hip

```cpp

#include "nbe_kernels_internal.h"
#include <algorithm>
#include <cstdint>
#include <cstdio>
#include <cstdlib>

namespace nbe {

#define LDS_AS NBE_LDS_AS
#define GLB_AS NBE_GLB_AS

extern __shared__ __attribute__((aligned(16))) f32x4 lds_dyn[];

template <int MODE, bool VEL, bool HAS_DX, int NI, bool G6 = false>
__global__ __launch_bounds__(256, 2) void conv_mfma_kernel(ConvKArgs a) {
    constexpr int CK = mode_ck(MODE), GL = CK / 4, TAPS = mode_taps(MODE);
    constexpr int COUT_T = 32 * NI;
    constexpr int XV = (MODE == MODE_FLAT3) ? 320 : 256;
    constexpr int WP = TAPS * GL * COUT_T;
    constexpr int XP = GL * XV;
    constexpr bool DX = VEL && HAS_DX;
    constexpr bool DWT = VEL && !G6;
    static_assert(!G6 || (DX && MODE == MODE_FLAT3), "gauged form: 3x3x3 layers with an input tangent");
    constexpr int OFF_W = 0, OFF_DW = WP, OFF_X = OFF_DW + (DWT ? WP : 0), OFF_DXX = OFF_X + XP;
// ... 176 lines not shown
}

template <int MODE, bool VEL, bool HAS_DX, int NI, bool G6 = false>
static void launch_conv_t(const ConvKArgs& ka, int ctiles, hipStream_t s) {
    constexpr int CK = mode_ck(MODE), GL = CK / 4, TAPS = mode_taps(MODE);
    constexpr int XV = (MODE == MODE_FLAT3) ? 320 : 256;
    constexpr int WP = TAPS * GL * 32 * NI, XP = GL * XV;
    constexpr int BUF = WP * ((VEL && !G6) ? 2 : 1) + XP * ((VEL && HAS_DX) ? 2 : 1);
    constexpr size_t smem = (size_t)2 * BUF * 16 + 256 * sizeof(int);
    auto kern = conv_mfma_kernel<MODE, VEL, HAS_DX, NI, G6>;
    ensure_lds_limit((const void*)kern, smem);
    dim3 grid(ka.ntiles, ctiles, 1), block(256, 1, 1);
    hipLaunchKernelGGL(kern, grid, block, smem, s, ka);
}

int launch_conv(const PackedW& pw, const ConvLaunch& L, bool vel, bool has_dx, hipStream_t s, ConvKernel* ran) {
    if (ran) *ran = CONV_NONE;
    ConvKArgs ka;
    ka.x = L.in.x; ka.dx = L.in.dx; ka.in_pstride = L.in.pstride;
    ka.D = L.in.D; ka.H = L.in.H; ka.W = L.in.W; ka.P = L.in.vox(); ka.in_off = L.in_off;
    ka.Dv = L.Dv; ka.Hv = L.Hv; ka.Wv = L.Wv;
    if (pw.mode == MODE_DOWN) ka.Q = (long)L.Dv * L.Hv * L.Wv;
    else ka.Q = ((long)(L.Dv - 1) * L.in.H + (L.Hv - 1)) * L.in.W + L.Wv;
    ka.y = L.out.x; ka.dy = L.out.dx; ka.out_pstride = L.out.pstride; ka.out_g0 = L.out_g0;
    ka.Ho = L.out.H; ka.Wo = L.out.W; ka.osz = L.osz; ka.oz = L.oz; ka.oy = L.oy; ka.ox = L.ox;
    ka.r = L.res.x; ka.dr = L.res.dx; ka.res_pstride = L.res.pstride;
    ka.bias = L.bias ? L.bias : pw.bias;
    const int set = L.set < 0 ? 0 : L.set;
    ka.up8 = L.set < 0 ? 1 : 0; ka.set_stride = (long)pw.floats * 4;
    ka.stem_w = pw.stem;
    ka.ww = L.wino ? pw.ww : nullptr;
    ka.wws = (L.wino && L.skw) ? L.skw->ww : nullptr; ka.wws_set_floats = L.skw ? L.skw->floats : 0;
    ka.w = pw.w + (size_t)set * pw.floats;
    ka.dw = pw.dw ? pw.dw + (size_t)set * pw.floats : nullptr;
    ka.nchunk = pw.cin_pad / prec_ck(pw.prec, pw.mode);
    ka.cout_groups = prec_is_half(pw.prec) ? (pw.cout + 7) / 8 : (pw.cout + 3) / 4;
    ka.flags = L.flags;
    ka.gout = L.gout; ka.beta = L.beta;
    ka.x2 = L.in2.x; ka.dx2 = L.in2.dx; ka.in2_pstride = L.in2.pstride;
    if (L.csplit_ch % 16 != 0 || L.sk_split_ch % 16 != 0) return 1;
    ka.csplit = L.csplit_ch > 0 ? L.csplit_ch / 16 : (1 << 30);
    ka.xs = ka.dxs = ka.xs2 = ka.dxs2 = nullptr; ka.s_pstride = ka.s2_pstride = 0; ka.s_csplit = 1 << 30;
    ka.ws = ka.dws = nullptr; ka.nskip = 0; ka.dws_delta = 0;
    if (L.skw) {
        if (L.sk.H != L.in.H || L.sk.W != L.in.W) return 1;
        const int64_t o = (L.sk_off - L.sk.W - 1) * 4;
        ka.xs = L.sk.x + o; ka.dxs = (L.flags & F_SKIP_NODX) ? ka.xs : L.sk.dx + o; ka.s_pstride = L.sk.pstride;
        if (L.sk_split_ch > 0) { ka.xs2 = L.sk2.x + o; ka.dxs2 = L.sk2.dx + o; ka.s2_pstride = L.sk2.pstride; ka.s_csplit = L.sk_split_ch / 16; }
        ka.ws = L.skw->w; ka.dws = L.skw->dw; ka.nskip = L.skw->cin_pad / 16;
    }
    ka.ntiles = (int)((ka.Q + TILE_VOX - 1) / TILE_VOX);
    const ConvKernel k = conv_select(pw, ka, vel, has_dx);
    if (ran) *ran = k;
    if (prec_is_half(pw.prec)) return launch_conv_h3(k, pw, ka, vel, has_dx, s);
    const int ct = pw.ctiles;
#define NBE_DISPATCH(MODE)                                                                   \
    if (vel) {                                                                               \
        if (has_dx) { if (pw.ni == 2) launch_conv_t<MODE, true, true, 2>(ka, ct, s);        \
                      else launch_conv_t<MODE, true, true, 1>(ka, ct, s); }                 \
        else        { if (pw.ni == 2) launch_conv_t<MODE, true, false, 2>(ka, ct, s);       \
                      else launch_conv_t<MODE, true, false, 1>(ka, ct, s); }                \
    } else {                                                                                 \
        if (pw.ni == 2) launch_conv_t<MODE, false, false, 2>(ka, ct, s);                     \
        else launch_conv_t<MODE, false, false, 1>(ka, ct, s);                                \
    }
    switch (k) {
    case CONV_MFMA_G:
        if (pw.ni == 2) launch_conv_t<MODE_FLAT3, true, true, 2, true>(ka, ct, s);
        else launch_conv_t<MODE_FLAT3, true, true, 1, true>(ka, ct, s);
        return 0;
    case CONV_MFMA:
        if (pw.mode == MODE_FLAT3) { NBE_DISPATCH(MODE_FLAT3) }
        else if (pw.mode == MODE_FLAT1) { NBE_DISPATCH(MODE_FLAT1) }
        else { NBE_DISPATCH(MODE_DOWN) }
        return 0;
    default: return 1;
    }
#undef NBE_DISPATCH
}


__device__ __forceinline__ double block_sum(double v, double* scratch) {
#pragma unroll
    for (int off = 32; off > 0; off >>= 1) v += __shfl_down(v, off, 64);
    const int lane = threadIdx.x & 63, wave = threadIdx.x >> 6;
    __syncthreads();
    if (lane == 0) scratch[wave] = v;
    __syncthreads();
    double t = 0.0;
    for (int i = 0; i < (int)(blockDim.x >> 6); ++i) t += scratch[i];
    return t;
}

__global__ __launch_bounds__(256) void modulate_kernel(const float* __restrict__ weight,
                                                       const float* __restrict__ sw,
                                                       const float* __restrict__ sb,
                                                       int cin, int k3, float s0, float s1, float eps,
                                                       int first_layer, float* __restrict__ w_n,
                                                       float* __restrict__ dw_tot, const float* __restrict__ a_in,
                                                       float* __restrict__ beta_out, const float* __restrict__ b_sub) {
    __shared__ double scratch[4];
    const int co = blockIdx.x;
    const int n = cin * k3;
    const float* wr = weight + (size_t)co * n;
    double sww = 0.0, swd = 0.0;
    for (int e = threadIdx.x; e < n; e += blockDim.x) {
// ... 380 lines not shown
```

### jax_nbody_emulator_with_dj_amd/csrc/nbe_kernels_h3.hip

```cpp

#include "nbe_kernels_internal.h"
#include <cstdlib>
#include <cstdio>
#include <algorithm>

#ifndef NBE_DBG
#define NBE_DBG 0
#endif

namespace nbe {

extern __shared__ __attribute__((aligned(16))) f32x4 lds_h3[];

__device__ __forceinline__ void split4(const f32x4 v, half4& hi, half4& lo) {
#pragma unroll
    for (int e = 0; e < 4; ++e) {
        hi[e] = (_Float16)v[e];
        lo[e] = (_Float16)__builtin_fmaf((float)hi[e], -H3_SCALE, v[e] * H3_SCALE);
    }
}
__device__ __forceinline__ f32x4 join4(const half4 hi, const half4 lo) {
    f32x4 v;
#pragma unroll
    for (int e = 0; e < 4; ++e) v[e] = (float)hi[e] + (float)lo[e] * H3_INV;
    return v;
}

template <bool VEL, bool SPLIT>
__device__ __forceinline__ void h3_store2(const ConvKArgs& a, int ct, int it, int lh, const long (&o)[2],
                                          const bool (&ok)[2], const f32x16 (&ym)[2], const f32x16 (&yc)[2],
                                          const f32x16 (&dm)[2], const f32x16 (&dc)[2]) {
    constexpr int PARTS = SPLIT ? 2 : 1;
    const bool act = a.flags & F_ACT, res = a.flags & F_RES;
    int unit[4];
    bool uok[4];
    f32x4 bv[4], gv[4];
    const bool gauge = VEL && a.gout;
#pragma unroll
    for (int k = 0; k < 4; ++k) {
        unit[k] = ct * 8 + 4 * it + k;
        uok[k] = unit[k] < a.cout_groups;
        if (!uok[k]) unit[k] = a.cout_groups - 1;
        bv[k] = *(const f32x4*)(a.bias + unit[k] * 8 + 4 * lh);
        if (gauge) gv[k] = *(const f32x4*)(a.gout + unit[k] * 8 + 4 * lh);
    }
    half4 rh[8], rl[8], dh[8], dl[8];
    if (res) {
#pragma unroll
        for (int p = 0; p < 8; ++p) {
            const long rb = ((long)(PARTS * unit[p & 3]) * a.res_pstride + o[p >> 2]) * 16 + 8 * lh;
            const long rlo = rb + a.res_pstride * 16;
            rh[p] = *(const half4*)((const char*)a.r + rb);
            if (SPLIT) rl[p] = *(const half4*)((const char*)a.r + rlo);
            if (VEL) {
                dh[p] = *(const half4*)((const char*)a.dr + rb);
                if (SPLIT) dl[p] = *(const half4*)((const char*)a.dr + rlo);
            }
        }
    }
#pragma unroll
    for (int p = 0; p < 8; ++p) {
        const int jt = p >> 2, k = p & 3;
        f32x4 v, dv;
#pragma unroll
        for (int e = 0; e < 4; ++e) {
            v[e] = ym[jt][4 * k + e] + (SPLIT ? yc[jt][4 * k + e] * H3_INV : 0.f) + bv[k][e];
            dv[e] = dm[jt][4 * k + e] + (SPLIT ? dc[jt][4 * k + e] * H3_INV : 0.f);
        }
        if (res) {
            if (SPLIT) {
                v += join4(rh[p], rl[p]);
                if (VEL) dv += join4(dh[p], dl[p]);
            } else {
#pragma unroll
                for (int e = 0; e < 4; ++e) {
                    v[e] += (float)rh[p][e];
                    if (VEL) dv[e] += (float)dh[p][e];
                }
            }
        }
        if (act) {
#pragma unroll
            for (int e = 0; e < 4; ++e) {
                if (VEL) dv[e] = v[e] > 0.f ? dv[e] : 0.01f * dv[e];
                v[e] = v[e] >= 0.f ? v[e] : 0.01f * v[e];
            }
        }
        if (gauge) {
#pragma unroll
            for (int e = 0; e < 4; ++e) dv[e] += gv[k][e] * v[e];
        }
        if (uok[k] && ok[jt]) {
            const long ob = ((long)(a.out_g0 + PARTS * unit[k]) * a.out_pstride + o[jt]) * 16 + 8 * lh;
            const long ol = ob + a.out_pstride * 16;
            half4 hi, lo;
            split4(v, hi, lo);
            *(half4*)((char*)a.y + ob) = hi;
            if (SPLIT) *(half4*)((char*)a.y + ol) = lo;
            if (VEL) {
                split4(dv, hi, lo);
                *(half4*)((char*)a.dy + ob) = hi;
                if (SPLIT) *(half4*)((char*)a.dy + ol) = lo;
            }
        }
    }
}


template <int MODE, bool SPLIT>
struct H3Geom {
    static constexpr int PARTS = SPLIT ? 2 : 1, UN = 2 * PARTS;
    static_assert(MODE != MODE_FLAT3, "3x3x3 layers run on the patch kernels");
    static constexpr int XV = 256;
    static constexpr int WP = UN * 64;
    static constexpr int XP = UN * XV;
};

template <int MODE, bool VEL, bool HAS_DX, bool SPLIT>
__global__ __launch_bounds__(512, 2) void conv_h3_kernel(ConvKArgs a) {
    typedef H3Geom<MODE, SPLIT> G;
    constexpr int XV = G::XV, WP = G::WP, XP = G::XP, PARTS = G::PARTS, UN = G::UN;
    constexpr bool DX = VEL && HAS_DX;
    constexpr int WB = WP * (VEL ? 2 : 1);
    constexpr int XB = XP * (DX ? 2 : 1);
    constexpr int OFF_DW = WP, OFF_DXX = XP;
    constexpr int XRING = 2 * WB;
    constexpr int NW_TOT = WB / 64, NX_TOT = (XB + 63) / 64;
    constexpr int NWS = (NW_TOT + 7) / 8, NXS = (NX_TOT + 7) / 8;
    static_assert(WB % 64 == 0, "weight stage must be whole wave-instructions");
    static_assert(XP % 32 == 0, "activation planes must be half-wave multiples");
    static_assert(NWS + NXS <= 9, "more DMA slots per wave than MFMA pairs in one stage");

    f32x4* lds = lds_h3;
    const int tid = threadIdx.x;
    const int lane = tid & 63;
    const int wave = __builtin_amdgcn_readfirstlane(tid >> 6);
    const int li = lane & 31, lh = lane >> 5;
    const int it = wave & 1, jq = wave >> 1;

    const int tile = xcd_tile(blockIdx.x, a.ntiles);
    const int ct = blockIdx.y;
    const long q0 = (long)tile * TILE_VOX;
    const int nstage = mode_nseg(MODE) * a.nchunk;
    const long HW = (long)a.H * a.W;

    int* inbase = (int*)(lds + XRING + 2 * XB);
    if (MODE == MODE_DOWN) {
        if (tid < TILE_VOX) {
            long o = q0 + tid;
            if (o > a.Q - 1) o = a.Q - 1;
            const int hw = a.Hv * a.Wv;
            const int zo = (int)(o / hw), rem = (int)(o - (long)zo * hw);
            const int yo = rem / a.Wv, xo = rem - yo * a.Wv;
            inbase[tid] = (int)((2L * zo * a.H + 2 * yo) * a.W + 2 * xo);
        }
        __syncthreads();
// ... 74 lines not shown
        if (SPLIT && k == 1) yc[jt] = __builtin_amdgcn_mfma_f32_32x32x16_f16(o.wh, o.xl[jt], yc[jt], 0, 0, 0);
        if (SPLIT && k == 2) yc[jt] = __builtin_amdgcn_mfma_f32_32x32x16_f16(o.wl, o.xh[jt], yc[jt], 0, 0, 0);
        if (VEL) {
            if (k == 3) dm[jt] = __builtin_amdgcn_mfma_f32_32x32x16_f16(o.dwh, o.xh[jt], dm[jt], 0, 0, 0);
            if (SPLIT && k == 4) dc[jt] = __builtin_amdgcn_mfma_f32_32x32x16_f16(o.dwh, o.xl[jt], dc[jt], 0, 0, 0);
            if (SPLIT && k == 5) dc[jt] = __builtin_amdgcn_mfma_f32_32x32x16_f16(o.dwl, o.xh[jt], dc[jt], 0, 0, 0);
        }
        if (DX) {
            if (k == 6) dm[jt] = __builtin_amdgcn_mfma_f32_32x32x16_f16(o.wh, o.dxh[jt], dm[jt], 0, 0, 0);
            if (SPLIT && k == 7) dc[jt] = __builtin_amdgcn_mfma_f32_32x32x16_f16(o.wh, o.dxl[jt], dc[jt], 0, 0, 0);
            if (SPLIT && k == 8) dc[jt] = __builtin_amdgcn_mfma_f32_32x32x16_f16(o.wl, o.dxh[jt], dc[jt], 0, 0, 0);
        }
    };

    {
        const long x0 = seg_offset(0);
#pragma unroll
        for (int t = 0; t < NXS; ++t) dma_x(t, x0, 0);
#pragma unroll
        for (int t = 0; t < NWS; ++t) dma_w(t, 0);
        wait_all();
        barrier();
    }

    int ring = 0;
    for (int s = 0; s < nstage; ++s) {
        const bool pw = s + 1 < nstage, px = s + 1 < nstage;
        const long xoff2 = px ? seg_offset(s + 1) : 0;
        const int ring2 = ring ^ 1;
        const half8* wb = (const half8*)(lds + (s & 1) * WB);
        const half8* xb = (const half8*)(lds + XRING + ring * XB);
        Ops o0, o1;
        load_ops(wb, xb, o0);
        __builtin_amdgcn_sched_barrier(0);
#pragma unroll
        for (int i = 0; i < 18; ++i) {
            mfma1(o0, i);
            if (i & 1) {
                const int t = i >> 1;
                if (t < NWS) { if (pw) dma_w(t, s + 1); }
                else if (t - NWS < NXS) { if (px) dma_x(t - NWS, xoff2, ring2); }
                __builtin_amdgcn_sched_barrier(0);
            }
        }
        __builtin_amdgcn_sched_barrier(0);
        __builtin_amdgcn_sched_barrier(0);
        wait_all();
        barrier();
        ring = ring == 1 ? 0 : ring + 1;
    }

    long o[2];
    bool ok[2];
#pragma unroll
    for (int jt = 0; jt < 2; ++jt) {
        const long q = q0 + jq * 64 + 32 * jt + li;
        ok[jt] = q < a.Q;
        if (MODE == MODE_DOWN) {
            o[jt] = q;
            if (a.Ho != a.Hv || a.Wo != a.Wv) {
                const int hw = a.Hv * a.Wv;
                const int z = (int)(q / hw), rem = (int)(q - (long)z * hw);
                const int yy = rem / a.Wv, xx = rem - yy * a.Wv;
                o[jt] = ((long)z * a.Ho + yy) * a.Wo + xx;
            }
        } else {
            const int z = (int)(q / HW), rem = (int)(q - (long)z * HW);
            const int yy = rem / a.W, xx = rem - yy * a.W;
            ok[jt] = ok[jt] && xx < a.Wv && yy < a.Hv && z < a.Dv;
            o[jt] = ((long)(z * a.osz + a.oz) * a.Ho + (yy * a.osz + a.oy)) * a.Wo + (xx * a.osz + a.ox);
        }
        if (!ok[jt]) o[jt] = 0;
    }
    h3_store2<VEL, SPLIT>(a, ct, it, lh, o, ok, ym, yc, dm, dc);
}

constexpr int UP_XV = 256;
template <bool SPLIT> struct UpGeom {
    static constexpr int UN = SPLIT ? 4 : 2;
    static constexpr int XC = 2 * UN * UP_XV;
    static constexpr int WS = 2 * 2 * UN * 64;
    static constexpr int WBASE = UP_MAXCH * XC;
    static constexpr int LDS_UNITS = WBASE + 2 * WS;
};

template <bool SPLIT, bool VEL = true>
__global__ __launch_bounds__(512, 2) void up_h3_kernel(ConvKArgs a) {
    constexpr int UN = UpGeom<SPLIT>::UN, UP_XC = UpGeom<SPLIT>::XC, UP_WS = UpGeom<SPLIT>::WS, UP_WBASE = UpGeom<SPLIT>::WBASE;
    constexpr int PS = SPLIT ? 2 : 1;
    f32x4* lds = lds_h3;
    const half8* L8 = (const half8*)lds_h3;
    const int tid = threadIdx.x;
    const int lane = tid & 63;
    const int wave = __builtin_amdgcn_readfirstlane(tid >> 6);
    const int li = lane & 31, lh = lane >> 5;
    const int it = wave & 1, jq = wave >> 1;
    const int tile = xcd_tile(blockIdx.x, a.ntiles);
    const int ct = blockIdx.y;
    const long q0 = (long)tile * UP_XV;
    const int nchunk = a.nchunk, nstage = 2 * 4 * nchunk;
    const long HW = (long)a.H * a.W;

    for (int c = 0; c < nchunk; ++c) {
#pragma unroll
        for (int k = 0; k < (VEL ? UN : UN / 2); ++k) {
            const int n = wave + 8 * k;
            const int t = n / (4 * UN), u = (n >> 2) % UN, qd = n & 3;
            const long v = q0 + a.in_off + qd * 64 + lane;
            const char* src = (const char*)(t ? a.dx : a.x) + (((long)c * UN + u) * a.in_pstride + v) * 16;
            dma16((const float*)src, lds + c * UP_XC + (t * UN + u) * UP_XV + qd * 64);
        }
    }
    auto dma_w = [&](int st) {
        const int c = st % nchunk, pp = (st / nchunk) & 3;
#pragma unroll
        for (int k = 0; k < UN / 2; ++k) {
            const int n = wave + 8 * k;
            const int par = n / (2 * UN), d = (n / UN) & 1, m = n % UN;
            if (!VEL && d) continue;
            const char* src = (const char*)(d ? a.dw : a.w) + (long)(2 * pp + par) * a.set_stride +
                              (((long)ct * nchunk + c) * (UN * 64) + m * 64 + lane) * 16;
            dma16((const float*)src, lds + UP_WBASE + (st & 1) * UP_WS + n * 64);
        }
    };
    dma_w(0);
    asm volatile("s_waitcnt vmcnt(0)" ::: "memory");
    __syncthreads();
// ... 4 lines not shown
        for (int jt = 0; jt < 2; ++jt)
#pragma unroll
            for (int e = 0; e < 16; ++e) { ym[jt][e] = 0.f; yc[jt][e] = 0.f; dm[jt][e] = 0.f; dc[jt][e] = 0.f; }
    };
    zero_acc();

    for (int st = 0; st < nstage; ++st) {
        const int c = st % nchunk, pp = (st / nchunk) & 3, half = st / (4 * nchunk);
        if (st + 1 < nstage) dma_w(st + 1);
        const half8* wb = L8 + UP_WBASE + (st & 1) * UP_WS;
        const half8* xb = L8 + c * UP_XC;
        const int xo = (PS * lh) * UP_XV + half * 128 + jq * 32 + li;
        const half8 xh = xb[xo];
        half8 dxh = xh, xl = xh, dxl = xh;
        if (VEL) dxh = xb[UN * UP_XV + xo];
        if (SPLIT) { xl = xb[xo + UP_XV]; if (VEL) dxl = xb[UN * UP_XV + xo + UP_XV]; }
#pragma unroll
        for (int jt = 0; jt < 2; ++jt) {
            const int wo = jt * (2 * UN * 64) + (PS * lh) * 64 + 32 * it + li;
            const half8 wh = wb[wo];
            half8 dwh = wh;
            if (VEL) dwh = wb[UN * 64 + wo];
            if (!SPLIT) {
                ym[jt] = __builtin_amdgcn_mfma_f32_32x32x16_f16(wh, xh, ym[jt], 0, 0, 0);
                if (VEL) {
                    dm[jt] = __builtin_amdgcn_mfma_f32_32x32x16_f16(dwh, xh, dm[jt], 0, 0, 0);
                    dm[jt] = __builtin_amdgcn_mfma_f32_32x32x16_f16(wh, dxh, dm[jt], 0, 0, 0);
                }
                continue;
            }
            const half8 wl = wb[wo + 64];
            ym[jt] = __builtin_amdgcn_mfma_f32_32x32x16_f16(wh, xh, ym[jt], 0, 0, 0);
            yc[jt] = __builtin_amdgcn_mfma_f32_32x32x16_f16(wh, xl, yc[jt], 0, 0, 0);
            yc[jt] = __builtin_amdgcn_mfma_f32_32x32x16_f16(wl, xh, yc[jt], 0, 0, 0);
            if (!VEL) continue;
            const half8 dwl = wb[UN * 64 + wo + 64];
            dm[jt] = __builtin_amdgcn_mfma_f32_32x32x16_f16(dwh, xh, dm[jt], 0, 0, 0);
            dc[jt] = __builtin_amdgcn_mfma_f32_32x32x16_f16(dwh, xl, dc[jt], 0, 0, 0);
            dc[jt] = __builtin_amdgcn_mfma_f32_32x32x16_f16(dwl, xh, dc[jt], 0, 0, 0);
            dm[jt] = __builtin_amdgcn_mfma_f32_32x32x16_f16(wh, dxh, dm[jt], 0, 0, 0);
            dc[jt] = __builtin_amdgcn_mfma_f32_32x32x16_f16(wh, dxl, dc[jt], 0, 0, 0);
            dc[jt] = __builtin_amdgcn_mfma_f32_32x32x16_f16(wl, dxh, dc[jt], 0, 0, 0);
        }
        const bool epi = c == nchunk - 1;
        if (epi) {
            asm volatile("s_waitcnt vmcnt(0)" ::: "memory");
            const long q = q0 + half * 128 + jq * 32 + li;
            const int z = (int)(q / HW), rem = (int)(q - (long)z * HW);
            const int yy = rem / a.W, xx = rem - yy * a.W;
            const bool okq = q < a.Q && xx < a.Wv && yy < a.Hv && z < a.Dv;
            const long o0 = okq ? ((long)(2 * z + (pp >> 1)) * a.Ho + (2 * yy + (pp & 1))) * a.Wo + 2 * xx : 0;
            const long o[2] = {o0, o0 + (okq ? 1 : 0)};
            const bool ok[2] = {okq, okq};
            h3_store2<VEL, SPLIT>(a, ct, it, lh, o, ok, ym, yc, dm, dc);
            zero_acc();
            asm volatile("s_waitcnt lgkmcnt(0)\n\ts_barrier" ::: "memory");
        } else {
            asm volatile("s_waitcnt vmcnt(0) lgkmcnt(0)" ::: "memory");
            __syncthreads();
        }
    }
}

template <bool SPLIT, bool VEL = true>
static int launch_up_h3(ConvKArgs ka, int ctiles, hipStream_t s) {
    constexpr size_t smem = (size_t)UpGeom<SPLIT>::LDS_UNITS * 16;
    static_assert(smem <= 160 * 1024, "LDS budget of one CU");
    if (!up8_ok(ka)) return 2;
    ensure_lds_limit((const void*)up_h3_kernel<SPLIT, VEL>, smem);
    dim3 grid(ka.ntiles, ctiles, 1), block(512, 1, 1);
    hipLaunchKernelGGL((up_h3_kernel<SPLIT, VEL>), grid, block, smem, s, ka);
    return 0;
}

constexpr int HP_RS = HP_COLS + 2;
constexpr int HP_PL = (HP_ROWS + 2) * HP_RS;

template <bool VEL, bool HAS_DX, bool SPLIT>
__global__ __launch_bounds__(512, 2) void conv_h3p_kernel(ConvKArgs a) {
    constexpr bool DX = VEL && HAS_DX;
    constexpr int PARTS = SPLIT ? 2 : 1, UN = 2 * PARTS;
    constexpr int HP_XP = UN * HP_PL;
    constexpr int HP_XPP = (HP_XP + 63) / 64 * 64;
    constexpr int WP = 3 * UN * 64;
    constexpr int WB = WP * (VEL ? 2 : 1);
    constexpr int XB = HP_XPP * (DX ? 2 : 1);
    constexpr int OFF_DW = WP, OFF_DXX = HP_XPP;
    constexpr int XBASE = 2 * WB;
    constexpr int NW_TOT = WB / 64, NX_TOT = XB / 64;
    constexpr int NWS = (NW_TOT + 7) / 8;
    constexpr int XPARTS = 3;
    constexpr int NXS = (NX_TOT + 8 * XPARTS - 1) / (8 * XPARTS);
    static_assert(NWS + NXS <= 9 && NXS <= 4, "DMA slots per wave");

    f32x4* lds = lds_h3;
    const int tid = threadIdx.x;
    const int lane = tid & 63;
    const int wave = __builtin_amdgcn_readfirstlane(tid >> 6);
    const int li = lane & 31, lh = lane >> 5;
    const int it = wave & 1, jq = wave >> 1;

    const int tile = xcd_tile(blockIdx.x, a.ntiles);
    const int ct = blockIdx.y;
    const int z = tile % a.Dv, tyx = tile / a.Dv;
    const int ty = tyx / a.tnx, tx = tyx - ty * a.tnx;
    const int y0 = ty * HP_ROWS, x0 = tx * HP_COLS;
    const int nstage = 9 * a.nchunk;
// ... 94 lines not shown
#pragma unroll
            for (int t = 0; t < NXS; ++t) dma_x(p, t, x0off, 0);
#pragma unroll
        for (int t = 0; t < NWS; ++t) dma_w(t, 0);
        __syncthreads();
    }

    int g = 0, dy = 0;
    for (int s = 0; s < nstage; ++s) {
        const bool pw = s + 1 < nstage, px = 3 * (g + 1) < nstage;
        const long xoff = px ? patch_offset(g + 1) : 0;
        const half8* wb = (const half8*)(lds + (s & 1) * WB);
        const half8* xb = (const half8*)(lds + XBASE + (g & 1) * XB);
        const int nb = (g + 1) & 1;
        Ops o0, o1;
        load_ops(wb, xb, dy, 0, o0);
        load_ops(wb, xb, dy, 1, o1);
        __builtin_amdgcn_sched_barrier(0);
#pragma unroll
        for (int i = 0; i < 18; ++i) {
            mfma1(o0, i);
            if (i & 1) {
                const int t = i >> 1;
                if (t < NWS) { if (pw) dma_w(t, s + 1); }
                else if (t - NWS < NXS) {
                    if (px) {
                        if (dy == 0) dma_x(0, t - NWS, xoff, nb);
                        else if (dy == 1) dma_x(1, t - NWS, xoff, nb);
                        else dma_x(2, t - NWS, xoff, nb);
                    }
                }
                __builtin_amdgcn_sched_barrier(0);
            }
        }
        __builtin_amdgcn_sched_barrier(0);
        load_ops(wb, xb, dy, 2, o0);
        __builtin_amdgcn_sched_barrier(0);
        mfma_ops(o1);
        __builtin_amdgcn_sched_barrier(0);
        mfma_ops(o0);
        __builtin_amdgcn_sched_barrier(0);
        __syncthreads();
        if (++dy == 3) { dy = 0; ++g; }
    }

    long o[2];
    bool ok[2];
#pragma unroll
    for (int jt = 0; jt < 2; ++jt) {
        const int yy = y0 + 2 * jq + jt, xx = x0 + li;
        ok[jt] = yy < a.Hv && xx < a.Wv;
        o[jt] = ok[jt] ? ((long)z * a.Ho + yy) * a.Wo + xx : (long)z * a.Ho * a.Wo;
    }
    h3_store2<VEL, SPLIT>(a, ct, it, lh, o, ok, ym, yc, dm, dc);
}

constexpr int HQ_TAPU = 4 * 64;
constexpr int HQ_WA = 5 * HQ_TAPU, HQ_WB = 4 * HQ_TAPU;
constexpr int HQ_OFF_B = 2 * HQ_WA;
constexpr int HQ_PP = (HP_PL + 7) / 8 * 8;
constexpr int HQ_XT = 4 * HQ_PP;
constexpr int HQ_XB = 2 * HQ_XT;
constexpr int HQ_XBASE = HQ_OFF_B + 2 * HQ_WB;
constexpr int HQ_LDS_UNITS = HQ_XBASE + 2 * HQ_XB;

__device__ __forceinline__ float acc_read(const float& acc) {
    float v;
    asm volatile("v_accvgpr_read_b32 %0, %1" : "=v"(v) : "a"(acc));
    return v;
}

__device__ __forceinline__ void dma16s(const char* ubase, unsigned voff, f32x4* dst_wave_base) {
    const unsigned long ub = (unsigned long)ubase;
    ubase = (const char*)(((unsigned long)(unsigned)__builtin_amdgcn_readfirstlane((int)(ub >> 32)) << 32) |
                          (unsigned long)(unsigned)__builtin_amdgcn_readfirstlane((int)(unsigned)ub));
    asm volatile("" : "+v"(voff));
    __builtin_amdgcn_global_load_lds((const NBE_GLB_AS void*)(ubase + voff), (NBE_LDS_AS void*)dst_wave_base, 16, 0, 0);
}

__device__ unsigned long long h3q_stamps[16];

void h3q_read_stamps(double* out, hipStream_t s) {
    unsigned long long h[16] = {0};
    (void)hipStreamSynchronize(s);
    (void)hipMemcpyFromSymbol(h, HIP_SYMBOL(h3q_stamps), sizeof h, 0, hipMemcpyDeviceToHost);
    for (int i = 0; i < 16; ++i) out[i] = (double)h[i];
    unsigned long long z[16] = {0};
    (void)hipMemcpyToSymbol(HIP_SYMBOL(h3q_stamps), z, sizeof z, 0, hipMemcpyHostToDevice);
}

__global__ __launch_bounds__(512, 2) void conv_h3q_kernel(ConvKArgs a) {
#if NBE_DBG
    unsigned long long tk0 = __builtin_amdgcn_s_memtime(), tk[8] = {0, 0, 0, 0, 0, 0, 0, 0};
#define NBE_STAMP(i) { const unsigned long long t_ = __builtin_amdgcn_s_memtime(); tk[i] += t_ - tk0; tk0 = t_; }
#define NBE_STAGE_END(i, keep) { NBE_STAMP(i) wait_keep(keep); NBE_STAMP(i + 1) \
                                 asm volatile("s_barrier" ::: "memory"); NBE_STAMP(i + 2) }
#else
#define NBE_STAMP(i)
#define NBE_STAGE_END(i, keep) { wait_keep(keep); asm volatile("s_barrier" ::: "memory"); }
#endif
    f32x4* lds = lds_h3;
    const half8* L8 = (const half8*)lds_h3;
    const int tid = threadIdx.x;
    const int lane = tid & 63;
    const int wave = __builtin_amdgcn_readfirstlane(tid >> 6);
    const int c = lane & 15, q = lane >> 4, kh = q & 1, ks = q >> 1;
    const int it = wave & 1, jq = wave >> 1;
// ... 1319 lines not shown
```

### jax_nbody_emulator_with_dj_amd/csrc/nbe_kernels_wino.h

```cpp

#ifndef NBE_EPI_MAX
#define NBE_EPI_MAX 1
#endif
#ifndef NBE_WINO_ZROW
#define NBE_WINO_ZROW 1
#endif
#ifndef NBE_WINO_ITEMREG
#define NBE_WINO_ITEMREG 1
#endif
#ifndef NBE_WINO_LOU
#define NBE_WINO_LOU (NBE_XF_F32 ? 0 : 1)
#endif
constexpr float WINO_WSCALE = 16384.0f;
constexpr float WINO_WSCALE_F16 = 256.0f;

struct WinoSrc { const char* xa; const char* xb; long dxd; const char* w; long psb; float sb; int pad_; };

struct WinoKArgs {
    int H, W, Dv, Hv, Wv, Ho, Wo;
    int nchunk, cout_groups, flags, ntiles, tny, tnx;
    int zblock;
    float* y; float* dy; long out_pstride; int out_g0;
    const float* bias; const float* gout; const float* beta;
    const float* r; const float* dr; long res_pstride;
    float inv_scale;
    int nskip;
    long dws_delta;
    WinoSrc st[NBE_MAX_WSTAGES + NBE_MAX_WSKIP];
};

template <bool SKIP, bool NOVEL, bool F16 = false>
__global__ __launch_bounds__(512, 2) void conv_h3w_kernel(WinoKArgs a) {
    static_assert(!(F16 && NOVEL), "the float16 form has no displacement-only variant");
    typedef HGGeom<false> G;
    constexpr int NW = 8, CT = 64, TAPU = G::TAPU, WGU = G::WG, XBASE = G::XBASE, MT = 4, NT = 2, NTILE = 8;
    constexpr int ZROW = G::LDS_UNITS;
    f32x4* lds = lds_h3;
    const half8* L8 = (const half8*)lds_h3;
    half8* L8w = (half8*)lds_h3;
    const int tid = threadIdx.x;
    const int lane = tid & 63;
    const int wave = __builtin_amdgcn_readfirstlane(tid >> 6);
    const int c = lane & 15, q = lane >> 4, kh = q & 1, ks = q >> 1;

    const int nct = (a.cout_groups + 7) / 8;
    const int vt = xcd_tile(blockIdx.x, a.ntiles * nct);
    const int tile = vt / nct, ct = vt - tile * nct;
    const int npair = a.Dv >> 1;
    int zp, ty, tx;
    {
        const int zb = a.zblock;
        const int full = (npair / zb) * zb;
        const int per_blk = zb * a.tny * a.tnx;
        if (tile < (npair / zb) * per_blk) {
            const int blk = tile / per_blk, r = tile - blk * per_blk;
            const int zi = r % zb, tyx = r / zb;
            zp = blk * zb + zi; ty = tyx / a.tnx; tx = tyx - ty * a.tnx;
        } else {
            const int r = tile - (npair / zb) * per_blk, rem = npair - full;
            const int zi = r % rem, tyx = r / rem;
            zp = full + zi; ty = tyx / a.tnx; tx = tyx - ty * a.tnx;
        }
    }
    const int y0 = ty * (NOVEL ? 2 * HP_ROWS : HP_ROWS), x0 = tx * HP_COLS, z0 = 2 * zp;
    const int nst = 4 * a.nchunk;

    const long to = (((long)z0 * a.H + y0) * a.W + x0) * 16;
    const long wcm = (long)ct * nst * WGU * 16, wcs = (long)ct * a.nskip * TAPU * 16;

    struct Nxt { const char *xa, *xb, *w0; long dxd, psb; float sb; } nx;
    auto set_next = [&](int s) {
        const WinoSrc e = a.st[s];
        nx.xa = e.xa + to; nx.xb = e.xb + to; nx.dxd = e.dxd; nx.psb = e.psb; nx.w0 = e.w + (SKIP && F16 && s >= nst ? wcs : wcm); nx.sb = e.sb;
    };
// ... 440 lines not shown
            LA(wh, aP); LB(xl, XBASE + bP1 + HQ_PP); LB(xh, XBASE + bP1);
    };
    const int npairs = 2 * a.nchunk;
    for (int s2 = 0; s2 + 1 < npairs; ++s2) {
        if (s2 == a.nchunk) butterfly();
        stage(YA, DA, 2 * s2, std::integral_constant<int, 1>());
        stage(YB, DB, 2 * s2 + 1, std::integral_constant<int, 1>());
    }
    if (npairs - 1 == a.nchunk) butterfly();
    stage(YA, DA, 2 * npairs - 2, std::integral_constant<int, 1>());
    stage(YB, DB, 2 * npairs - 1, std::integral_constant<int, SKIP ? 2 : 0>());
    if (SKIP && F16) {
        for (int sc = 0; sc < a.nskip; ++sc) {
            raw_stage(YA, DA, nst + 2 * sc, true);
            raw_stage(YB, DB, nst + 2 * sc + 1, sc + 1 < a.nskip);
        }
    }
    if (SKIP && !F16) {
        sk_hi(sk_wbase(0));
        sk_lo(sk_wbase(0));
        __builtin_amdgcn_s_waitcnt(0x0F70);
        int sc = 0;
        for (; sc + 1 < a.nskip; sc += 2) {
            sk_chunk(skP, skQ, sc, sc + 1);
            sk_chunk(skQ, skP, sc + 1, sc + 2 < a.nskip ? sc + 2 : sc + 1);
        }
        if (sc < a.nskip) sk_chunk(skP, skQ, sc, -1);
    }
#undef NBE_SB
#undef SNAKE
    asm volatile("s_nop 15\n\ts_nop 15" ::: "memory");

    const bool act = a.flags & F_ACT, gauge = !NOVEL && a.gout != nullptr;
    f32x4 bv[MT], be[MT], gv[MT];
    int unit[MT];
    bool uok[MT];
#pragma unroll
    for (int mt = 0; mt < MT; ++mt) {
        unit[mt] = ct * (CT / 8) + 2 * mt + ks;
        uok[mt] = unit[mt] < a.cout_groups;
        if (!uok[mt]) unit[mt] = a.cout_groups - 1;
        bv[mt] = *(const f32x4*)(a.bias + unit[mt] * 8 + 4 * kh);
        be[mt] = f32x4{0.f, 0.f, 0.f, 0.f};
        if (!NOVEL) be[mt] = *(const f32x4*)(a.beta + unit[mt] * 8 + 4 * kh);
        gv[mt] = f32x4{0.f, 0.f, 0.f, 0.f};
        if (!NOVEL && gauge) gv[mt] = *(const f32x4*)(a.gout + unit[mt] * 8 + 4 * kh);
    }
#pragma unroll
    for (int mt = 0; mt < MT; ++mt) asm volatile("" : "+v"(bv[mt]), "+v"(be[mt]), "+v"(gv[mt]));
    long ob_mt[MT];
#pragma unroll
    for (int mt = 0; mt < MT; ++mt) ob_mt[mt] = (long)(a.out_g0 + (F16 ? 1 : 2) * unit[mt]) * a.out_pstride * 16 + 8 * kh;
    const long ol_off = a.out_pstride * 16;
    auto epilogue = [&](f32x4 (&Y)[NTILE], f32x4 (&DY)[NTILE], int z) {
        int o[NT];
        bool ook[NT], ook2[NT];
#pragma unroll
        for (int nt = 0; nt < NT; ++nt) {
            const int yy = y0 + rowp, xx = x0 + 16 * nt + c;
            ook[nt] = yy < a.Hv && xx < a.Wv;
            ook2[nt] = NOVEL && yy + HP_ROWS < a.Hv && xx < a.Wv;
            o[nt] = ook[nt] ? (z * a.Ho + yy) * a.Wo + xx : z * a.Ho * a.Wo;
        }
        half4 r0[F16 ? NTILE : 1], r1[F16 ? NTILE : 1];
        const bool res = F16 && (a.flags & F_RES);
        if (F16 && res) {
#pragma unroll
            for (int t = 0; t < NTILE; ++t) {
                const int mt = t / NT, nt = t % NT;
                const long rb = ((long)unit[mt] * a.res_pstride + (long)o[nt]) * 16 + 8 * kh;
                r0[t] = *(const half4*)((const char*)a.r + rb);
                r1[t] = *(const half4*)((const char*)a.dr + rb);
            }
#pragma unroll
            for (int t = 0; t < NTILE; ++t) asm volatile("" : "+v"(r0[t]), "+v"(r1[t]));
        }
#pragma unroll
        for (int mt = 0; mt < MT; ++mt) {
#pragma unroll
            for (int nt = 0; nt < NT; ++nt) {
                const int t = mt * NT + nt;
                f32x4 v, dv;
                __builtin_amdgcn_sched_barrier(0);
#pragma unroll
                for (int e = 0; e < 4; ++e) {
                    const float yp = acc_read(Y[t][e]) * a.inv_scale;
                    v[e] = yp + bv[mt][e];
                    dv[e] = acc_read(DY[t][e]) * a.inv_scale + be[mt][e] * yp;
                }
                if (F16 && res) {
#pragma unroll
                    for (int e = 0; e < 4; ++e) { v[e] += (float)r0[t][e]; dv[e] += (float)r1[t][e]; }
                }
                if (act) {
#pragma unroll
                    for (int e = 0; e < 4; ++e) {
                        dv[e] = v[e] > 0.f ? dv[e] : 0.01f * dv[e];
                        v[e] = (F16 || !NBE_EPI_MAX) ? (v[e] >= 0.f ? v[e] : 0.01f * v[e]) : __builtin_fmaxf(v[e], 0.01f * v[e]);
                    }
                }
                if (gauge) {
#pragma unroll
                    for (int e = 0; e < 4; ++e) dv[e] += gv[mt][e] * v[e];
                }
                if (F16) {
                    if (uok[mt] && ook[nt]) {
                        const long ob = ob_mt[mt] + (long)o[nt] * 16;
                        half4 h, dh;
#pragma unroll
                        for (int e = 0; e < 4; ++e) { h[e] = (_Float16)v[e]; dh[e] = (_Float16)dv[e]; }
                        *(half4*)((char*)a.y + ob) = h;
                        *(half4*)((char*)a.dy + ob) = dh;
                    }
                } else
                if (NOVEL) {
#pragma unroll
                    for (int e = 0; e < 4; ++e) {
                        dv[e] = acc_read(DY[t][e]) * a.inv_scale + bv[mt][e];
                        if (act) dv[e] = dv[e] >= 0.f ? dv[e] : 0.01f * dv[e];
                    }
                    const long ob = ob_mt[mt] + (long)o[nt] * 16;
                    const long ol = ob + ol_off;
                    const long r8 = (long)HP_ROWS * a.Wo * 16;
                    half4 hi, lo;
                    if (uok[mt] && ook[nt]) {
                        split4(v, hi, lo);
                        *(half4*)((char*)a.y + ob) = hi;
                        *(half4*)((char*)a.y + ol) = lo;
                    }
                    if (uok[mt] && ook2[nt]) {
                        split4(dv, hi, lo);
                        *(half4*)((char*)a.y + ob + r8) = hi;
                        *(half4*)((char*)a.y + ol + r8) = lo;
                    }
                } else
                if (uok[mt] && ook[nt]) {
                    const long ob = ob_mt[mt] + (long)o[nt] * 16;
                    const long ol = ob + ol_off;
                    half4 hi, lo;
                    split4(v, hi, lo);
                    *(half4*)((char*)a.y + ob) = hi;
                    *(half4*)((char*)a.y + ol) = lo;
                    split4(dv, hi, lo);
                    *(half4*)((char*)a.dy + ob) = hi;
                    *(half4*)((char*)a.dy + ol) = lo;
                }
            }
        }
    };
    epilogue(YA, DA, z0);
    epilogue(YB, DB, z0 + 1);
}

__global__ __launch_bounds__(256) void pack_h3w_kernel(const float* __restrict__ w, int cout, int cin, int nchunk, long total,
                                                       _Float16* __restrict__ dst, int* __restrict__ flag, int f16) {
    const long idx = (long)blockIdx.x * blockDim.x + threadIdx.x;
    if (idx >= total) return;
    long r = idx;
    const int j = (int)(r % 8); r /= 8;
    const int co = (int)(r % 64); r /= 64;
    const int u = (int)(r % 4); r /= 4;
    const int tap = (int)(r % 9); r /= 9;
    const int stage = (int)(r % (4 * nchunk)); r /= 4 * nchunk;
    const int ct = (int)r;
    const int chunk = stage >> 2, xi = stage & 3;
    const int h = u >> 1, part = u & 1;
    const int ci = f16 ? chunk * 32 + 8 * u + j : chunk * 16 + 8 * h + j, oc = ct * 64 + co;
    float v = 0.f;
    if (oc < cout && ci < cin) {
        const float* p = w + (((size_t)oc * cin + ci) * 3) * 9 + tap;
        const float w0 = p[0], w1 = p[9], w2 = p[18];
        v = xi == 0 ? w0 : xi == 1 ? 0.5f * (w0 + w1 + w2) : xi == 2 ? 0.5f * (w0 - w1 + w2) : -w2;
    }
    v *= f16 ? WINO_WSCALE_F16 : WINO_WSCALE;
    if (!(fabsf(v) <= 60000.f)) { atomicOr(flag, 1); v = 0.f; }
    const _Float16 hi = (_Float16)v;
    dst[idx] = (part == 0 || f16) ? hi : (_Float16)(v - (float)hi);
}

void launch_pack_h3w(const float* w_oidhw, int cout, int cin, int cin_pad, int ctiles, float* dst, int* flag, hipStream_t s, int prec) {
    const bool f16 = prec == PREC_F16;
    const int nchunk = cin_pad / (f16 ? 32 : 16);
    const long total = (long)ctiles * 4 * nchunk * 9 * 4 * 64 * 8;
    hipLaunchKernelGGL(pack_h3w_kernel, dim3((unsigned)((total + 255) / 256)), dim3(256), 0, s, w_oidhw, cout, cin, nchunk, total,
                       (_Float16*)dst, flag, f16 ? 1 : 0);
}

static int launch_h3w(ConvKArgs ka, int ctiles, hipStream_t s, bool novel, bool f16) {
    typedef HGGeom<false> G;
    constexpr size_t smem = (size_t)(G::LDS_UNITS + 64) * 16;
    static_assert(smem <= 160 * 1024, "LDS budget of one CU");
    if (!h3w_ok(ka, ctiles, novel, f16)) return 2;
    const float *ww = ka.ww, *wws = ka.wws;
    if (f16) {
        ka.nchunk /= H3W_F16_CHUNKS; if (ka.csplit < (1 << 29)) ka.csplit /= H3W_F16_CHUNKS;
        ka.nskip /= H3W_F16_CHUNKS; if (ka.s_csplit < (1 << 29)) ka.s_csplit /= H3W_F16_CHUNKS;
    }
    WinoKArgs wa;
    wa.H = ka.H; wa.W = ka.W; wa.Dv = ka.Dv; wa.Hv = ka.Hv; wa.Wv = ka.Wv; wa.Ho = ka.Ho; wa.Wo = ka.Wo;
    wa.nchunk = ka.nchunk; wa.cout_groups = ka.cout_groups; wa.flags = ka.flags;
    const int trows = novel ? 2 * HP_ROWS : HP_ROWS;
    wa.ntiles = (int)patch_tiles(ka, trows, HP_COLS, ka.Dv / 2);
    wa.tny = ka.tny; wa.tnx = ka.tnx;
    wa.y = ka.y; wa.dy = ka.dy; wa.out_pstride = ka.out_pstride; wa.out_g0 = ka.out_g0;
    wa.bias = ka.bias; wa.gout = novel ? nullptr : ka.gout; wa.beta = novel ? nullptr : ka.beta;
    const long rows8 = (long)HP_ROWS * ka.W * 16;
    wa.inv_scale = 1.0f / (f16 ? WINO_WSCALE_F16 : WINO_WSCALE);
    wa.r = ka.r; wa.dr = ka.dr; wa.res_pstride = ka.res_pstride;
    wa.zblock = std::min(8, ka.Dv / 2);
    wa.nskip = ka.nskip; wa.dws_delta = ka.wws_set_floats * 4;
    static const int XI[2][2] = {{1, 2}, {0, 3}};
    static const int PA[4] = {0, 1, 2, 1}, PB[4] = {2, 2, 1, 3};
    static const float SB[4] = {-1.f, 1.f, -1.f, -1.f};
    const long plane = (long)ka.H * ka.W * 16;
    for (int ph = 0; ph < 2; ++ph)
        for (int chunk = 0; chunk < ka.nchunk; ++chunk)
            for (int ab = 0; ab < 2; ++ab) {
                const int xi = XI[ph][ab];
                const ChunkSrc c = input_chunk(ka, chunk);
                WinoSrc& e = wa.st[(ph * ka.nchunk + chunk) * 2 + ab];
                e.xa = c.x + PA[xi] * plane; e.xb = c.x + PB[xi] * plane; e.dxd = novel ? rows8 : c.dx - c.x;
                e.w = (const char*)ww + (long)(chunk * 4 + xi) * G::WG * 16; e.psb = c.psb; e.sb = SB[xi]; e.pad_ = 0;
            }
    for (int sc = 0; sc < ka.nskip; ++sc)
        for (int ab = 0; ab < 2; ++ab) {
            const ChunkSrc c = skip_chunk(ka, sc);
            WinoSrc& e = wa.st[4 * ka.nchunk + 2 * sc + ab];
            e.xa = c.x + ab * plane; e.xb = e.xa; e.dxd = novel ? rows8 : c.dx - c.x; e.w = (const char*)wws + (long)sc * G::TAPU * 16; e.psb = c.psb; e.sb = 0.f; e.pad_ = 0;
        }
    const bool skip = ka.nskip > 0;
    if (novel) wa.dws_delta = 0;
    auto kern = f16 ? (skip ? conv_h3w_kernel<true, false, true> : conv_h3w_kernel<false, false, true>)
              : novel ? (skip ? conv_h3w_kernel<true, true> : conv_h3w_kernel<false, true>)
              : (skip ? conv_h3w_kernel<true, false> : conv_h3w_kernel<false, false>);
    ensure_lds_limit((const void*)kern, smem);
    dim3 grid(wa.ntiles * ctiles, 1, 1), block(512, 1, 1);
    hipLaunchKernelGGL(kern, grid, block, smem, s, wa);
    return 0;
}
```

### jax_nbody_emulator_with_dj_amd/engine.py

```python

import ctypes as C

import numpy as np

from . import _lib
from ._lib import LayerDesc, NBEError, NBERangeError, check

try:
    import torch
except Exception:
    torch = None

BLOCKS = ('conv_l00', 'conv_l01', 'down_l0', 'conv_l1', 'down_l1', 'conv_l2', 'down_l2', 'conv_c',
          'up_r2', 'conv_r2', 'up_r1', 'conv_r1', 'up_r0', 'conv_r00', 'conv_r01')


def _is_torch(x):
    return torch is not None and isinstance(x, torch.Tensor)


def _f32(a):
    return np.ascontiguousarray(np.asarray(a, dtype=np.float32))


# ... 296 lines not shown
        dres = None if dres is None else _f32(dres)
        y = np.empty((cout,) + osp, np.float32)
        dy = np.empty_like(y) if vel else None
        flags = (1 if act else 0) | (2 if res is not None else 0)
        check(self._l.nbe_test_layer(self._h, k, int(crop), flags, _ptr(x), _ptr(dx), cin, D, H, W, _ptr(w), _ptr(dw),
                                     _ptr(bias), cout, _ptr(res), _ptr(dres), _ptr(y), _ptr(dy)))
        return (y, dy) if vel else y

    def test_layer_gauged(self, x, dx, w, beta, bias, act=False, res=None, dres=None):
        x, dx, w, beta, bias = _f32(x), _f32(dx), _f32(w), _f32(beta), _f32(bias)
        cin, D, H, W = x.shape
        cout = w.shape[0]
        y = np.empty((cout, D - 2, H - 2, W - 2), np.float32)
        dy = np.empty_like(y)
        if res is not None:
            res, dres = _f32(res), _f32(dres)
            check(self._l.nbe_test_layer_gauged_res(self._h, (1 if act else 0) | 2, _ptr(x), _ptr(dx), cin, D, H, W, _ptr(w),
                                                    _ptr(beta), _ptr(bias), cout, _ptr(res), _ptr(dres), _ptr(y), _ptr(dy)))
            return y, dy
        check(self._l.nbe_test_layer_gauged(self._h, 1 if act else 0, _ptr(x), _ptr(dx), cin, D, H, W, _ptr(w), _ptr(beta),
                                            _ptr(bias), cout, _ptr(y), _ptr(dy)))
        return y, dy

    PATHS = {"skip_fused": 1, "two_source": 2, "wino_0": 4, "wino_1": 8, "narrow": 16, "up8": 32, "skip_nodx": 64,
             "two_source_skip": 128}

    def test_block(self, block, x, dx=None, x2=None, dx2=None, pad=0, two_source=False):
        x = _f32(x)
        dx, x2, dx2 = (None if a is None else _f32(a) for a in (dx, x2, dx2))
        m, vel = self.mid_chan, self.compute_vel
        _, D, H, W = x.shape
        res = block.startswith('conv_')
        if res:
            cout = self.out_chan if block == 'conv_r01' else m
            cmid = 2 * m if block in ('conv_r2', 'conv_r1', 'conv_r00') else m
            sy = 0 if pad else 2
            y = np.empty((cout, D - 4, H - 2 * sy, W - 2 * sy), np.float32)
            h = np.empty((cmid, D - 2, H - sy, W - sy), np.float32)
        elif block.startswith('down_'):
            y, h = np.empty((m, D // 2, H // 2, W // 2), np.float32), None
        else:
            y, h = np.empty((m if x2 is None else 2 * m, 2 * D, 2 * H, 2 * W), np.float32), None
        dy = np.empty_like(y) if vel else None
        dh = np.empty_like(h) if (vel and h is not None) else None
        g = np.zeros((3, 2 * m), np.float32)
        word = C.c_int(0)
        check(self._l.nbe_test_block(self._h, block.encode(), int(pad), 1 if two_source else 0, _ptr(x), _ptr(dx), D, H, W,
                                     _ptr(x2), _ptr(dx2), _ptr(y), _ptr(dy), _ptr(h), _ptr(dh), _ptr(g), C.byref(word)))
        cin = x.shape[0] if (x2 is None or not res) else 2 * m
        return {"y": y, "dy": dy, "h": h, "dh": dh, "gauge_in": g[0, :cin], "gauge_hidden": None if h is None else g[1, :h.shape[0]],
                "gauge_out": g[2, :(m if not res else y.shape[0])],
                "paths": {k for k, b in self.PATHS.items() if word.value & b}}

    def test_modulate(self, weight, style_weight, style_bias, s, first_layer, eps=1e-8, vel=True):
        weight, sw, sb = _f32(weight), _f32(style_weight), _f32(style_bias)
        cout, cin, k = weight.shape[:3]
        wn = np.empty_like(weight)
        dw = np.empty_like(weight) if vel else None
        check(self._l.nbe_test_modulate(self._h, _ptr(weight), _ptr(sw), _ptr(sb), cout, cin, k, float(s[0]),
                                        float(s[1]), float(eps), 1 if first_layer else 0, _ptr(wn), _ptr(dw)))
        return (wn, dw) if vel else wn

    def probe_begin(self, origin, nout=8):
        o = (C.c_int64 * 3)(*[int(v) for v in origin])
        check(self._l.nbe_probe_begin(self._h, o, int(nout)))

    def probe_read(self):
        out, total, lay = {}, 0, []
        for i in range(self._l.nbe_probe_slots(self._h)):
            name = C.create_string_buffer(64)
            dims, off = (C.c_int * 3)(), C.c_int64()
            check(self._l.nbe_probe_layout(self._h, i, name, 64, dims, C.byref(off)))
            lay.append((name.value.decode(), dims[0], dims[1], dims[2], off.value))
            total = max(total, off.value + dims[0] * dims[1] * dims[1] * dims[2])
        words = np.empty(total, dtype=np.uint32)
        check(self._l.nbe_probe_read(self._h, words.ctypes.data_as(C.c_void_p), total))
        for name, c, n, nw, off in lay:
            w = words[off:off + c * n * n * nw].reshape(c, n, n, nw)
            bits = np.unpackbits(w.view(np.uint8), axis=-1, bitorder='little')
            out[name] = bits[..., :n].astype(bool)
        return out

    def probe_end(self):
        check(self._l.nbe_probe_end(self._h))

    def profile_enable(self, on=True):
        check(self._l.nbe_profile_enable(self._h, 1 if on else 0))

    def profile_reset(self):
        check(self._l.nbe_profile_reset(self._h))

    def profile_read(self):
        n = self._l.nbe_profile_count(self._h)
        out = []
        for i in range(n):
            name = C.create_string_buffer(128)
            ms, la, fl = C.c_double(), C.c_int64(), C.c_double()
            check(self._l.nbe_profile_entry(self._h, i, name, 128, C.byref(ms), C.byref(la), C.byref(fl)))
            out.append({'kernel': name.value.decode(), 'ms': ms.value, 'launches': la.value, 'flops': fl.value})
        return out

    def workspace_bytes(self):
        return int(self._l.nbe_workspace_bytes(self._h))

    def debug_phase_cycles(self):
        out = (C.c_double * 16)()
# ... 3 lines not shown
```

Baseline: 101.4 million.

## Store mirrored y/x halos from conv epilogues instead of separate fill passes

Conv kernels (f16x3 Winograd, up8, down) now write each edge voxel's value into the mirrored halo positions directly from the epilogue. The separate fill_halo launch is skipped when the halo was stored. The change also caches zeroing of the input tensor's unused planes across calls and skips the output memset when the subboxes fully cover the output. This removes extra kernel launches and memory passes, at the cost of more complex epilogues, a template split for edge tiles, and cache invalidation state tied to workspace reallocation.

New measurement: 101.9 million, median of 6. Within noise of the previous version (+0.5%).

```diff
diff --git a/include/nbe.h b/include/nbe.h
--- a/include/nbe.h
+++ b/include/nbe.h
@@ -248,6 +248,9 @@
        NBE_PATH_TWO_SOURCE_SKIP = 128   };
 int nbe_test_block(nbe_ctx* ctx, const char* block, int pad, int two_source, const float* x, const float* dx, int D, int H, int W,
                    const float* x2, const float* dx2, float* y, float* dy, float* h, float* dh, float* gauges, int* paths);
+int nbe_test_block_halo(nbe_ctx* ctx, const char* block, int two_source, const float* x, const float* dx, int D, int H, int W,
+                        const float* x2, const float* dx2, float* y, float* dy, float* h, float* dh, uint64_t* ws_hash,
+                        int* halos_stored);
 int nbe_test_modulate(nbe_ctx* ctx, const float* weight, const float* style_weight, const float* style_bias,
                       int cout, int cin, int k, float s0, float s1, float eps, int first_layer,
                       float* w_n, float* dw_tot);
diff --git a/jax_nbody_emulator_with_dj_amd/_lib.py b/jax_nbody_emulator_with_dj_amd/_lib.py
--- a/jax_nbody_emulator_with_dj_amd/_lib.py
+++ b/jax_nbody_emulator_with_dj_amd/_lib.py
@@ -160,6 +160,9 @@
     "nbe_test_block": (C.c_int, [C.c_void_p, C.c_char_p, C.c_int, C.c_int, C.c_void_p, C.c_void_p, C.c_int, C.c_int, C.c_int,
                                  C.c_void_p, C.c_void_p, C.c_void_p, C.c_void_p, C.c_void_p, C.c_void_p, C.c_void_p,
                                  C.POINTER(C.c_int)]),
+    "nbe_test_block_halo": (C.c_int, [C.c_void_p, C.c_char_p, C.c_int, C.c_void_p, C.c_void_p, C.c_int, C.c_int, C.c_int,
+                                      C.c_void_p, C.c_void_p, C.c_void_p, C.c_void_p, C.c_void_p, C.c_void_p,
+                                      C.POINTER(C.c_uint64), C.POINTER(C.c_int)]),
     "nbe_test_modulate": (C.c_int, [C.c_void_p, C.c_void_p, C.c_void_p, C.c_void_p, C.c_int, C.c_int, C.c_int,
                                     C.c_float, C.c_float, C.c_float, C.c_int, C.c_void_p, C.c_void_p]),
     "nbe_probe_begin": (C.c_int, [C.c_void_p, C.POINTER(C.c_int64), C.c_int]),
@@ -217,6 +220,8 @@
                 "(hipcc, gfx950). There is no CPU fallback." % LIB_PATH)
         l = C.CDLL(LIB_PATH)
         for name, (res, args) in SIGNATURES.items():
+            if os.environ.get("NBE_LIB") and not hasattr(l, name):
+                continue
             fn = getattr(l, name)
             fn.restype = res
             fn.argtypes = args
diff --git a/jax_nbody_emulator_with_dj_amd/csrc/nbe_conv_select.h b/jax_nbody_emulator_with_dj_amd/csrc/nbe_conv_select.h
--- a/jax_nbody_emulator_with_dj_amd/csrc/nbe_conv_select.h
+++ b/jax_nbody_emulator_with_dj_amd/csrc/nbe_conv_select.h
@@ -135,6 +135,13 @@
     return CONV_H3_DOWN;
 }
 
+inline bool stores_halo(ConvKernel k, const PackedW& pw, const ConvLaunch& L, bool vel) {
+    if (L.halo != 1 || pw.prec != PREC_F16X3 || !vel) return false;
+    if (k != CONV_H3W_F16X3 && k != CONV_UP8 && k != CONV_H3_DOWN) return false;
+    if (L.osz != (k == CONV_UP8 ? 2 : 1) || (k != CONV_UP8 && (L.oz || L.oy || L.ox))) return false;
+    return L.out.H == L.osz * L.Hv + 2 && L.out.W == L.osz * L.Wv + 2;
+}
+
 inline std::string conv_label(ConvKernel k, const PackedW& pw, bool vel, bool has_dx) {
     const char* m = pw.mode == MODE_FLAT3 ? "FLAT3" : pw.mode == MODE_FLAT1 ? "FLAT1" : "DOWN";
     const bool f16 = pw.prec == PREC_F16;
diff --git a/jax_nbody_emulator_with_dj_amd/csrc/nbe_engine_box.cpp b/jax_nbody_emulator_with_dj_amd/csrc/nbe_engine_box.cpp
--- a/jax_nbody_emulator_with_dj_amd/csrc/nbe_engine_box.cpp
+++ b/jax_nbody_emulator_with_dj_amd/csrc/nbe_engine_box.cpp
@@ -162,6 +162,7 @@
     if (need < 0) return 1;
     if (need > c->ws_bytes) {
         c->sst.valid = false;
+        workspace_disturbed(c);
         if (c->ws) { HIPCHK(hipStreamSynchronize(c->stream)); HIPCHK(hipFree(c->ws)); c->ws = nullptr; c->ws_bytes = 0; }
         HIPCHK(hipMalloc((void**)&c->ws, need));
         HIPCHK(hipMemsetAsync(c->ws, 0, need, c->stream));
@@ -175,7 +176,8 @@
                       int OD, int OH, int OW, int a0, int a1, int a2) {
     c->sst.valid = false;
     c->arena.reset();
-    Tensor tin = talloc(c, c->in_chan, D, H, W), y;
+    Tensor tin = talloc(c, c->in_chan, D, H, W, false), y;
+    zero_input_rest(c, tin, c->in_chan);
     tin.pad = c->pyx ? 1 : 0;
     if (tin.pad) set_org(tin, 0, 48, 48);
     if (!c->pipe.active && !c->pipe.slabwise)
@@ -207,7 +209,8 @@
     const int geo[18] = {Db, Hb, Wb, o0, o1, o2, D, H, W, out_dtype, OD, OH, OW, a0, a1, a2, c->slab, c->prec};
     memcpy(k.geo, geo, sizeof geo);
     k.f[0] = Dz; k.f[1] = vel_fac; k.f[2] = c->act_scale;
-    k.epoch = c->epoch; k.flags = (c->pyx ? 1 : 0) | (c->pz ? 2 : 0) | (c->gauge_active ? 4 : 0) | (c->fuse ? 8 : 0) | (wino_env_off() ? 16 : 0);
+    k.epoch = c->epoch; k.flags = (c->pyx ? 1 : 0) | (c->pz ? 2 : 0) | (c->gauge_active ? 4 : 0) | (c->fuse ? 8 : 0) | (wino_env_off() ? 16 : 0) |
+                                 (store_halo_env_off() ? 32 : 0);
     nbe_ctx::GraphVal& g = c->graphs[k];
     g.used = ++c->graph_clock;
     if (!g.exec && g.seen++ == 0) {
@@ -238,6 +241,11 @@
             g.exec = nullptr; g.seen = -1000000;
             return run_subbox(c, box, Db, Hb, Wb, o0, o1, o2, D, H, W, Dz, vel_fac, disp, velo, out_dtype, OD, OH, OW, a0, a1, a2);
         }
+    }
+    if (c->input_rest.ws != c->ws) {
+        c->sst.valid = false;
+        c->arena.reset();
+        zero_input_rest(c, talloc(c, c->in_chan, D, H, W, false), c->in_chan);
     }
     if (user != c->own_stream) { HIPCHK(hipEventRecord(c->ev_g0, user)); HIPCHK(hipStreamWaitEvent(c->own_stream, c->ev_g0, 0)); }
     HIPCHK(hipGraphLaunch(g.exec, c->own_stream));
@@ -510,7 +518,8 @@
     const float* bd = r.bd; char *dd = r.dd, *vd = r.vd;
     nbe_progress_cb cb = r.cb; void* user = r.user;
     auto& P = c->pipe;
-    if ((r.zero_out || !out_dev) && !piped) {
+    const bool covered = r.zero_out && !order && (int64_t)c0 * ndiv[0] == O0 && (int64_t)c1 * ndiv[1] == O1 && (int64_t)c2 * ndiv[2] == O2;
+    if ((r.zero_out || !out_dev) && !piped && !covered) {
         HIPCHK(hipMemsetAsync(dd, 0, out_bytes, c->stream));
         if (c->vel) HIPCHK(hipMemsetAsync(vd, 0, out_bytes, c->stream));
     }
diff --git a/jax_nbody_emulator_with_dj_amd/csrc/nbe_engine_brick.cpp b/jax_nbody_emulator_with_dj_amd/csrc/nbe_engine_brick.cpp
--- a/jax_nbody_emulator_with_dj_amd/csrc/nbe_engine_brick.cpp
+++ b/jax_nbody_emulator_with_dj_amd/csrc/nbe_engine_brick.cpp
@@ -141,6 +141,7 @@
     const int Dh = (int)bsize[0] + 2 * BRICK_RAW;
     if (prepare_range(c, (const float*)box, (int64_t)c->in_chan * Dh * bsize[1] * bsize[2], Dz)) return 1;
     c->arena.reset();
+    workspace_disturbed(c);
     Tensor tin = talloc(c, c->in_chan, D, H, W);
     tin.pad = 1; set_org(tin, 0, 48, 48);
     launch_gather((const float*)box, c->in_chan, Dh, (int)bsize[1], (int)bsize[2], 0, -1, -1, zview(tin, 48 - BRICK_RAW, Dh).p,
diff --git a/jax_nbody_emulator_with_dj_amd/csrc/nbe_engine_internal.h b/jax_nbody_emulator_with_dj_amd/csrc/nbe_engine_internal.h
--- a/jax_nbody_emulator_with_dj_amd/csrc/nbe_engine_internal.h
+++ b/jax_nbody_emulator_with_dj_amd/csrc/nbe_engine_internal.h
@@ -84,7 +84,7 @@
     float* dwn_f = nullptr;
 };
 
-struct Tensor { Planes p; int64_t off = -1; int pad = 0; int org[3] = {0, 0, 0}; };
+struct Tensor { Planes p; int64_t off = -1; int pad = 0; int org[3] = {0, 0, 0}; bool halo_stored = false; };
 
 struct ProfEntry { std::string name; double ms = 0; int64_t launches = 0; double flops = 0; };
 
@@ -220,6 +220,8 @@
         unsigned* count = nullptr;
     } probe;
     int* paths = nullptr;
+    struct InputRest { const char* ws = nullptr; int64_t off = 0, pstride = 0; int G = 0; } input_rest;
+    int halos_stored = 0;
     bool prof = false;
     std::vector<ProfEntry> prof_entries;
     struct Pending { int entry; hipEvent_t a, b; };
@@ -242,14 +244,17 @@
 int planes_for(int C, int prec);
 Tensor talloc(nbe_ctx* c, int C, int D, int H, int W, bool zero_rest = true);
 Tensor tallocp(nbe_ctx* c, int C, int D, int Hi, int Wi, int pad, bool zero_rest = true);
-void fill_halo(nbe_ctx* c, const Tensor& t);
+void fill_halo(nbe_ctx* c, const Tensor& t, bool stored = false);
+void zero_input_rest(nbe_ctx* c, const Tensor& t, int C);
+inline void workspace_disturbed(nbe_ctx* c);
 void tfree(nbe_ctx* c, Tensor& t);
 Tensor zview(const Tensor& t, int z0, int nz);
 void set_org(Tensor& t, int z, int y, int x);
 bool wino_f16_layer(int prec, bool vel, int cin_pad);
 bool wino_env_off();
+bool store_halo_env_off();
 bool up8_launch(const nbe_ctx* c, const Layer& L, bool has_dx);
-int run_conv(nbe_ctx* c, const Layer& L, const ConvLaunch& cl_in, bool has_dx);
+int run_conv(nbe_ctx* c, const Layer& L, const ConvLaunch& cl_in, bool has_dx, bool* halo_stored = nullptr);
 const Layer* find_layer(nbe_ctx* c, const char* block, const char* layer);
 bool block_fused(const nbe_ctx* c, const Layer* L1, int nres);
 bool two_source_width(const nbe_ctx* c);
@@ -259,9 +264,9 @@
                   bool halo_s = true);
 int resblock(nbe_ctx* c, const char* name, const Tensor& x, bool has_dx, bool final_act, int cout, int cmid, Tensor* out,
              Tensor* hidden_out = nullptr, const int* zr = nullptr, const Tensor* x2 = nullptr);
-int down_conv(nbe_ctx* c, const Layer& L, const Tensor& x, Tensor& o, bool probe, const int* zr = nullptr);
+int down_conv(nbe_ctx* c, const Layer& L, const Tensor& x, Tensor& o, bool probe, const int* zr = nullptr, bool* halo_stored = nullptr);
 int downblock(nbe_ctx* c, const char* name, const Tensor& x, Tensor* out);
-int upblock(nbe_ctx* c, const char* name, const Tensor& x, const Tensor& cat, int xcrop = 0, int g0 = -1);
+int upblock(nbe_ctx* c, const char* name, const Tensor& x, const Tensor& cat, int xcrop = 0, int g0 = -1, bool* halo_stored = nullptr);
 void crop_into(nbe_ctx* c, const Tensor& src, int crop, const Tensor& dst, int cz = -1);
 int check_dims(int D, int H, int W);
 int check_dims_pyx(int D, int H, int W);
@@ -304,4 +309,6 @@
 hipEvent_t get_event(nbe_ctx* c);
 void prof_collect(nbe_ctx* c);
 
+inline void workspace_disturbed(nbe_ctx* c) { c->input_rest.ws = nullptr; }
+
 #pragma GCC visibility pop
diff --git a/jax_nbody_emulator_with_dj_amd/csrc/nbe_engine_net.cpp b/jax_nbody_emulator_with_dj_amd/csrc/nbe_engine_net.cpp
--- a/jax_nbody_emulator_with_dj_amd/csrc/nbe_engine_net.cpp
+++ b/jax_nbody_emulator_with_dj_amd/csrc/nbe_engine_net.cpp
@@ -17,16 +17,28 @@
     return p;
 }
 
+static void zero_rest_planes(nbe_ctx* c, const Tensor& t, int C);
 Tensor talloc(nbe_ctx* c, int C, int D, int H, int W, bool zero_rest) {
     Tensor t;
     t.p = ws_planes(c, planes_for(C, c->prec), D, H, W, &t.off);
-    const int gw = c->prec == PREC_F16 ? (C + 7) / 8 : c->prec == PREC_F16X3 ? 2 * ((C + 7) / 8) : (C + 3) / 4;
-    if (zero_rest && !c->dry && t.off >= 0 && gw < t.p.G) {
+    if (zero_rest) zero_rest_planes(c, t, C);
+    return t;
+}
+static int written_planes(const nbe_ctx* c, int C) { return c->prec == PREC_F16 ? (C + 7) / 8 : c->prec == PREC_F16X3 ? 2 * ((C + 7) / 8) : (C + 3) / 4; }
+static void zero_rest_planes(nbe_ctx* c, const Tensor& t, int C) {
+    const int gw = written_planes(c, C);
+    if (!c->dry && t.off >= 0 && gw < t.p.G) {
         const size_t off = (size_t)gw * t.p.pstride * 4, bytes = (size_t)(t.p.G - gw) * t.p.pstride * 16;
         launch_zero(t.p.x + off, (int64_t)bytes, c->stream);
         if (t.p.dx) launch_zero(t.p.dx + off, (int64_t)bytes, c->stream);
     }
-    return t;
+}
+void zero_input_rest(nbe_ctx* c, const Tensor& t, int C) {
+    if (c->dry || t.off < 0 || written_planes(c, C) >= t.p.G) return;
+    auto& r = c->input_rest;
+    if (r.ws == c->ws && r.off == t.off && r.pstride == t.p.pstride && r.G == t.p.G) return;
+    zero_rest_planes(c, t, C);
+    r.ws = c->ws; r.off = t.off; r.pstride = t.p.pstride; r.G = t.p.G;
 }
 Tensor tallocp(nbe_ctx* c, int C, int D, int Hi, int Wi, int pad, bool zero_rest) {
     Tensor t = talloc(c, C, D, Hi + 2 * pad, Wi + 2 * pad, zero_rest);
@@ -40,8 +52,10 @@
     if (p.dx) p.dx += sh;
     return p;
 }
-void fill_halo(nbe_ctx* c, const Tensor& t) {
-    if (t.pad > 0 && !c->dry) launch_fill_yx(t.p, t.pad, c->vel, c->stream);
+void fill_halo(nbe_ctx* c, const Tensor& t, bool stored) {
+    if (t.pad <= 0 || c->dry) return;
+    if (stored || t.halo_stored) ++c->halos_stored;
+    else launch_fill_yx(t.p, t.pad, c->vel, c->stream);
 }
 void tfree(nbe_ctx* c, Tensor& t) { if (t.off >= 0) c->arena.release(t.off); t.off = -1; }
 Tensor zview(const Tensor& t, int z0, int nz) {
@@ -64,11 +78,14 @@
     return prec == PREC_F16 && vel && cin_pad % (H3_CHUNK * H3W_F16_CHUNKS) == 0 && h3w_stages_fit(cin_pad, H3W_F16_CHUNKS);
 }
 bool wino_env_off() { return getenv("NBE_WINO") && atoi(getenv("NBE_WINO")) == 0; }
+bool store_halo_env_off() { return getenv("NBE_STORE_HALO") && atoi(getenv("NBE_STORE_HALO")) == 0; }
 bool up8_launch(const nbe_ctx* c, const Layer& L, bool has_dx) { return prec_is_half(c->prec) && (!c->vel || has_dx) && up8_fits(L.pw.cin_pad); }
 
-int run_conv(nbe_ctx* c, const Layer& L, const ConvLaunch& cl_in, bool has_dx) {
+int run_conv(nbe_ctx* c, const Layer& L, const ConvLaunch& cl_in, bool has_dx, bool* halo_stored) {
+    if (halo_stored) *halo_stored = false;
     if (c->dry) return 0;
     ConvLaunch cl = cl_in;
+    if (store_halo_env_off()) cl.halo = 0;
     const bool g6 = c->gauge_active && L.g6 && has_dx;
     const bool nov = !c->vel && c->prec == PREC_F16X3 && L.kind == 0 && L.pw.ww && c->wino_ok;
     if (c->gauge_active) { cl.gout = L.gout; cl.beta = g6 ? L.beta : nullptr; }
@@ -87,6 +104,7 @@
     if (launch_conv(pw, cl, c->vel, has_dx, c->stream, &k))
         return fail("internal error: no kernel for layer %s/%s (mode %d, gauged %d, input tangent %d, crop offset %ld, output stride %d, selected %s)",
                     L.block.c_str(), L.layer.c_str(), L.pw.mode, (int)g6, (int)has_dx, (long)cl.in_off, cl.osz, conv_kernel_name(k));
+    if (halo_stored) *halo_stored = stores_halo(k, pw, cl, c->vel);
     if (c->paths)
         *c->paths |= (cl.skw ? NBE_PATH_SKIP_FUSED : 0) | (cl.skw && (cl.flags & F_SKIP_NODX) ? NBE_PATH_SKIP_NODX : 0) |
                      (cl.csplit_ch ? NBE_PATH_TWO_SOURCE : 0) | (cl.skw && cl.sk_split_ch ? NBE_PATH_TWO_SOURCE_SKIP : 0) |
@@ -148,25 +166,28 @@
         if (run_conv(c, *Ls, cl, has_dx)) return 1;
     }
     int og[3];
+    bool stored = false;
     {
         ConvLaunch cl; cl.in = zview(x, jh, nh + 2).p; cl.Dv = nh; cl.Hv = H - 2; cl.Wv = W - 2; cl.out = inner(hv); cl.flags = F_ACT;
+        cl.halo = pad;
         if (x2) { cl.in2 = zview(*x2, jh, nh + 2).p; cl.csplit_ch = c->mid; }
-        if (run_conv(c, *L0, cl, has_dx)) return 1;
+        if (run_conv(c, *L0, cl, has_dx, &stored)) return 1;
         org_conv(x, 1, og); og[0] += jh;
         const int zh[3] = {zr ? zr[0] : 0, zr ? zr[1] + 2 : 0, zr ? zr[2] : 0};
         probe_act(c, *L0, cl.out, 0, og, cl.Dv, cl.Hv, cl.Wv, pad != 0, zr ? zh : nullptr);
     }
-    fill_halo(c, hv);
+    fill_halo(c, hv, stored);
     {
         ConvLaunch cl; cl.in = zview(h, js, ns + 2).p; cl.Dv = ns; cl.Hv = s.p.H - 2 * pad; cl.Wv = s.p.W - 2 * pad; cl.out = inner(sv);
+        cl.halo = halo_s ? pad : 0;
         if (fused) { cl.sk = xs.p; cl.sk_off = sk_off; cl.skw = L1->pwn.w ? &Ls->pwn : &Ls->pw; cl.flags = (final_act ? F_ACT : 0) | (has_dx ? 0 : F_SKIP_NODX);
                      if (x2) { cl.sk2 = zview(*x2, js, ns + 4).p; cl.sk_split_ch = c->mid; } }
         else { cl.res = inner(sv); cl.flags = F_RES | (final_act ? F_ACT : 0); }
-        if (run_conv(c, *L1, cl, true)) return 1;
+        if (run_conv(c, *L1, cl, true, &stored)) return 1;
         org_conv(x, 2, og); og[0] += js;
         if (final_act) probe_act(c, *L1, cl.out, 0, og, cl.Dv, cl.Hv, cl.Wv, pad != 0, zr);
     }
-    if (halo_s) fill_halo(c, sv);
+    if (halo_s) fill_halo(c, sv, stored);
     return 0;
 }
 
@@ -194,9 +215,10 @@
     launch_crop(zview(t, src, n).p, 0, zview(t, dst, n).p, 0, c->vel, c->stream, 0);
 }
 
-int down_conv(nbe_ctx* c, const Layer& L, const Tensor& x, Tensor& o, bool probe, const int* zr) {
+int down_conv(nbe_ctx* c, const Layer& L, const Tensor& x, Tensor& o, bool probe, const int* zr, bool* halo_stored) {
     ConvLaunch cl; cl.in = inner(x); cl.Dv = o.p.D; cl.Hv = o.p.H - 2 * o.pad; cl.Wv = o.p.W - 2 * o.pad; cl.out = inner(o); cl.flags = F_ACT;
-    if (run_conv(c, L, cl, true)) return 1;
+    cl.halo = halo_stored ? o.pad : 0;
+    if (run_conv(c, L, cl, true, halo_stored)) return 1;
     set_org(o, x.org[0] / 2, x.org[1] / 2, x.org[2] / 2);
     if (probe) probe_act(c, L, cl.out, 0, o.org, cl.Dv, cl.Hv, cl.Wv, x.pad != 0, zr);
     return 0;
@@ -223,7 +245,8 @@
 
 static int mid_planes(const nbe_ctx* c) { return c->mid / (c->prec == PREC_F16 ? 8 : 4); }
 
-int upblock(nbe_ctx* c, const char* name, const Tensor& x, const Tensor& cat, int xcrop, int g0) {
+int upblock(nbe_ctx* c, const char* name, const Tensor& x, const Tensor& cat, int xcrop, int g0, bool* halo_stored) {
+    if (halo_stored) *halo_stored = false;
     const Layer* L = find_layer(c, name, "conv_0");
     if (!L) return fail("missing layer %s/conv_0", name);
     xcrop += x.pad;
@@ -237,7 +260,8 @@
         cl.Dv = x.p.D; cl.Hv = Hx; cl.Wv = Wx; cl.out = inner(cat);
         cl.out_g0 = out_g0; cl.osz = 2; cl.oz = (p >> 2) & 1; cl.oy = (p >> 1) & 1; cl.ox = p & 1;
         cl.flags = F_ACT; cl.set = up8 ? -1 : p;
-        if (run_conv(c, *L, cl, true)) return 1;
+        cl.halo = (up8 && g0 >= 0 && halo_stored) ? cat.pad : 0;
+        if (run_conv(c, *L, cl, true, halo_stored)) return 1;
     }
     const int xc = xcrop - x.pad;
     const int og[3] = {2 * x.org[0], 2 * (x.org[1] + xc), 2 * (x.org[2] + xc)};
@@ -283,6 +307,7 @@
     const int D1 = pz ? (D - 96) / 2 : Y / 2;
     Tensor td = pad ? tallocp(c, m, D1 + 2 * cz1, Hi / 2, Wi / 2, dpad) : talloc(c, m, Y / 2, (H - 8) / 2, (W - 8) / 2);
     if (skip0.off < 0 || td.off < 0) return fail("workspace exhausted (level 0)");
+    td.halo_stored = dpad == 1;
     const Layer* Ld = find_layer(c, "down_l0", "conv_0");
     if (!Ld) return fail("missing layer down_l0/conv_0");
     const int sy = pad ? 0 : 2;
@@ -323,7 +348,10 @@
                 const Tensor tv = zview(td, cz1 + (d0 - (pz ? 44 : 0)) / 2, (d1 - d0) / 2);
                 Tensor yv = zview(y0, d0 - z, d1 - d0);
                 ConvLaunch cl; cl.in = inner(yv); cl.Dv = tv.p.D; cl.Hv = tv.p.H - 2 * dpad; cl.Wv = tv.p.W - 2 * dpad; cl.out = inner(tv); cl.flags = F_ACT;
-                if (run_conv(c, *Ld, cl, true)) return 1;
+                cl.halo = dpad;
+                bool stored;
+                if (run_conv(c, *Ld, cl, true, &stored)) return 1;
+                td.halo_stored = td.halo_stored && stored;
                 const int og[3] = {yv.org[0] / 2, yv.org[1] / 2, yv.org[2] / 2};
                 const int zd[3] = {22, 22 + (D - 96) / 2, pz ? (D - 96) / 2 : 0};
                 probe_act(c, *Ld, cl.out, 0, og, cl.Dv, cl.Hv, cl.Wv, pad != 0, zd);
@@ -376,8 +404,9 @@
     Tensor tp = zview(t, cz2, y1d.p.D / 2);
     tp.pad = L2_CTX;
     const int zd[3] = {y1d.org[0] / 2, y1d.org[0] / 2 + tp.p.D, tp.p.D};
-    if (down_conv(c, *Ld1, y1d, tp, true, pz ? zd : nullptr)) return 1;
-    fill_halo(c, tp);
+    bool stored;
+    if (down_conv(c, *Ld1, y1d, tp, true, pz ? zd : nullptr, &stored)) return 1;
+    fill_halo(c, tp, stored);
     wrap_z(c, t, cz2);
     set_org(t, tp.org[0] - cz2, tp.org[1] - L2_CTX, tp.org[2] - L2_CTX);
     if (two) *y1_out = y1; else tfree(c, y1);
@@ -416,8 +445,9 @@
         set_org(sk, sk.org[0] - 16, y1.org[1] - 16, y1.org[2] - 16);
         set_org(cat1, sk.org[0], sk.org[1], sk.org[2]);
     }
-    if (upblock(c, "up_r1", r, cat1, cat1.pad ? 2 : 0, two ? 0 : -1)) return 1;
-    fill_halo(c, cat1);
+    bool stored;
+    if (upblock(c, "up_r1", r, cat1, cat1.pad ? 2 : 0, two ? 0 : -1, &stored)) return 1;
+    fill_halo(c, cat1, stored);
     tfree(c, r);
     if (resblock(c, "conv_r1", two ? sk : cat1, true, true, m, 2 * m, r_out, nullptr, nullptr, two ? &cat1 : nullptr)) return 1;
     tfree(c, cat1);
@@ -480,8 +510,9 @@
         set_org(cat, skip0.org[0] + z, skip0.org[1], skip0.org[2]);
         { int og[3]; org_conv(cat, 2, og); set_org(q, og[0], og[1], og[2]); }
         if (!two && !c->dry) launch_crop(zview(skip0, z + c0, cn).p, 0, zview(cat, c0, cn).p, 0, c->vel, c->stream, 0);
-        if (upblock(c, "up_r0", zview(r, (z + c0) / 2, cn / 2), zview(cat, c0, cn), 0, two ? 0 : -1)) return 1;
-        fill_halo(c, zview(cat, c0, cn));
+        bool stored;
+        if (upblock(c, "up_r0", zview(r, (z + c0) / 2, cn / 2), zview(cat, c0, cn), 0, two ? 0 : -1, &stored)) return 1;
+        fill_halo(c, zview(cat, c0, cn), stored);
         const Tensor sk = two ? zview(skip0, z, std::min(S + 8, skip0.p.D - z)) : cat;
         const Tensor* up2 = two ? &cat : nullptr;
         if (first) {
diff --git a/jax_nbody_emulator_with_dj_amd/csrc/nbe_kernels.h b/jax_nbody_emulator_with_dj_amd/csrc/nbe_kernels.h
--- a/jax_nbody_emulator_with_dj_amd/csrc/nbe_kernels.h
+++ b/jax_nbody_emulator_with_dj_amd/csrc/nbe_kernels.h
@@ -66,6 +66,7 @@
     int64_t sk_off = 0;
     const PackedW* skw = nullptr;
     bool wino = false;
+    int halo = 0;
 };
 
 struct ConvGroupSrc { const char* x; const char* dx; const char* w; long psb; };
@@ -76,6 +77,7 @@
     int Dv, Hv, Wv; long Q;
     float* y; float* dy; long out_pstride; int out_g0;
     int Ho, Wo; int osz, oz, oy, ox;
+    int mirror;
     const float* r; const float* dr; long res_pstride;
     const float* bias; const float* w; const float* dw;
     int nchunk; int cout_groups; int flags; int ntiles;
diff --git a/jax_nbody_emulator_with_dj_amd/csrc/nbe_kernels.hip b/jax_nbody_emulator_with_dj_amd/csrc/nbe_kernels.hip
--- a/jax_nbody_emulator_with_dj_amd/csrc/nbe_kernels.hip
+++ b/jax_nbody_emulator_with_dj_amd/csrc/nbe_kernels.hip
@@ -252,6 +252,7 @@
     ka.ntiles = (int)((ka.Q + TILE_VOX - 1) / TILE_VOX);
     const ConvKernel k = conv_select(pw, ka, vel, has_dx);
     if (ran) *ran = k;
+    ka.mirror = stores_halo(k, pw, L, vel) ? 1 : 0;
     if (prec_is_half(pw.prec)) return launch_conv_h3(k, pw, ka, vel, has_dx, s);
     const int ct = pw.ctiles;
 #define NBE_DISPATCH(MODE)                                                                   \
diff --git a/jax_nbody_emulator_with_dj_amd/csrc/nbe_kernels_h3.hip b/jax_nbody_emulator_with_dj_amd/csrc/nbe_kernels_h3.hip
--- a/jax_nbody_emulator_with_dj_amd/csrc/nbe_kernels_h3.hip
+++ b/jax_nbody_emulator_with_dj_amd/csrc/nbe_kernels_h3.hip
@@ -3,6 +3,7 @@
 #include <cstdlib>
 #include <cstdio>
 #include <algorithm>
+#include <type_traits>
 
 #ifndef NBE_DBG
 #define NBE_DBG 0
@@ -26,9 +27,25 @@
     return v;
 }
 
+__device__ __forceinline__ int halo_edges(int yy, int xx, int Hv, int Wv) {
+    return (yy == 0 ? 1 : 0) | (yy == Hv - 1 ? 2 : 0) | (xx == 0 ? 4 : 0) | (xx == Wv - 1 ? 8 : 0);
+}
+template <class Store>
+__device__ __forceinline__ void halo_images(int edges, long py, long px, Store&& store) {
+#pragma unroll
+    for (int sy = -1; sy <= 1; ++sy) {
+#pragma unroll
+        for (int sx = -1; sx <= 1; ++sx) {
+            if (sy == 0 && sx == 0) continue;
+            const bool iny = sy == 0 || (edges & (sy > 0 ? 1 : 2)), inx = sx == 0 || (edges & (sx > 0 ? 4 : 8));
+            if (iny && inx) store(sy * py + sx * px);
+        }
+    }
+}
+
 template <bool VEL, bool SPLIT>
 __device__ __forceinline__ void h3_store2(const ConvKArgs& a, int ct, int it, int lh, const long (&o)[2],
-                                          const bool (&ok)[2], const f32x16 (&ym)[2], const f32x16 (&yc)[2],
+                                          const bool (&ok)[2], const int (&em)[2], const f32x16 (&ym)[2], const f32x16 (&yc)[2],
                                           const f32x16 (&dm)[2], const f32x16 (&dc)[2]) {
     constexpr int PARTS = SPLIT ? 2 : 1;
     const bool act = a.flags & F_ACT, res = a.flags & F_RES;
@@ -93,15 +110,24 @@
         if (uok[k] && ok[jt]) {
             const long ob = ((long)(a.out_g0 + PARTS * unit[k]) * a.out_pstride + o[jt]) * 16 + 8 * lh;
             const long ol = ob + a.out_pstride * 16;
-            half4 hi, lo;
+            half4 hi, lo, dhi, dlo;
             split4(v, hi, lo);
             *(half4*)((char*)a.y + ob) = hi;
             if (SPLIT) *(half4*)((char*)a.y + ol) = lo;
             if (VEL) {
-                split4(dv, hi, lo);
-                *(half4*)((char*)a.dy + ob) = hi;
-                if (SPLIT) *(half4*)((char*)a.dy + ol) = lo;
-            }
+                split4(dv, dhi, dlo);
+                *(half4*)((char*)a.dy + ob) = dhi;
+                if (SPLIT) *(half4*)((char*)a.dy + ol) = dlo;
+            }
+            if (em[jt])
+                halo_images(em[jt], (long)a.osz * a.Hv * a.Wo * 16, (long)a.osz * a.Wv * 16, [&](long d) {
+                    *(half4*)((char*)a.y + ob + d) = hi;
+                    if (SPLIT) *(half4*)((char*)a.y + ol + d) = lo;
+                    if (VEL) {
+                        *(half4*)((char*)a.dy + ob + d) = dhi;
+                        if (SPLIT) *(half4*)((char*)a.dy + ol + d) = dlo;
+                    }
+                });
         }
     }
 }
@@ -282,6 +308,7 @@
 
     long o[2];
     bool ok[2];
+    int em[2] = {0, 0};
 #pragma unroll
     for (int jt = 0; jt < 2; ++jt) {
         const long q = q0 + jq * 64 + 32 * jt + li;
@@ -293,6 +320,7 @@
                 const int z = (int)(q / hw), rem = (int)(q - (long)z * hw);
                 const int yy = rem / a.Wv, xx = rem - yy * a.Wv;
                 o[jt] = ((long)z * a.Ho + yy) * a.Wo + xx;
+                if (a.mirror && ok[jt]) em[jt] = halo_edges(yy, xx, a.Hv, a.Wv);
             }
         } else {
             const int z = (int)(q / HW), rem = (int)(q - (long)z * HW);
@@ -302,7 +330,7 @@
         }
         if (!ok[jt]) o[jt] = 0;
     }
-    h3_store2<VEL, SPLIT>(a, ct, it, lh, o, ok, ym, yc, dm, dc);
+    h3_store2<VEL, SPLIT>(a, ct, it, lh, o, ok, em, ym, yc, dm, dc);
 }
 
 constexpr int UP_XV = 256;
@@ -413,7 +441,12 @@
             const long o0 = okq ? ((long)(2 * z + (pp >> 1)) * a.Ho + (2 * yy + (pp & 1))) * a.Wo + 2 * xx : 0;
             const long o[2] = {o0, o0 + (okq ? 1 : 0)};
             const bool ok[2] = {okq, okq};
-            h3_store2<VEL, SPLIT>(a, ct, it, lh, o, ok, ym, yc, dm, dc);
+            int em[2] = {0, 0};
+            if (a.mirror && okq) {
+                em[0] = halo_edges(2 * yy + (pp & 1), 2 * xx, 2 * a.Hv, 2 * a.Wv);
+                em[1] = halo_edges(2 * yy + (pp & 1), 2 * xx + 1, 2 * a.Hv, 2 * a.Wv);
+            }
+            h3_store2<VEL, SPLIT>(a, ct, it, lh, o, ok, em, ym, yc, dm, dc);
             zero_acc();
             asm volatile("s_waitcnt lgkmcnt(0)\n\ts_barrier" ::: "memory");
         } else {
@@ -614,7 +647,8 @@
         ok[jt] = yy < a.Hv && xx < a.Wv;
         o[jt] = ok[jt] ? ((long)z * a.Ho + yy) * a.Wo + xx : (long)z * a.Ho * a.Wo;
     }
-    h3_store2<VEL, SPLIT>(a, ct, it, lh, o, ok, ym, yc, dm, dc);
+    const int em[2] = {0, 0};
+    h3_store2<VEL, SPLIT>(a, ct, it, lh, o, ok, em, ym, yc, dm, dc);
 }
 
 constexpr int HQ_TAPU = 4 * 64;
diff --git a/jax_nbody_emulator_with_dj_amd/csrc/nbe_kernels_wino.h b/jax_nbody_emulator_with_dj_amd/csrc/nbe_kernels_wino.h
--- a/jax_nbody_emulator_with_dj_amd/csrc/nbe_kernels_wino.h
+++ b/jax_nbody_emulator_with_dj_amd/csrc/nbe_kernels_wino.h
@@ -20,6 +20,7 @@
     int H, W, Dv, Hv, Wv, Ho, Wo;
     int nchunk, cout_groups, flags, ntiles, tny, tnx;
     int zblock;
+    int mirror;
     float* y; float* dy; long out_pstride; int out_g0;
     const float* bias; const float* gout; const float* beta;
     const float* r; const float* dr; long res_pstride;
@@ -566,8 +567,10 @@
 #pragma unroll
     for (int mt = 0; mt < MT; ++mt) ob_mt[mt] = (long)(a.out_g0 + (F16 ? 1 : 2) * unit[mt]) * a.out_pstride * 16 + 8 * kh;
     const long ol_off = a.out_pstride * 16;
-    auto epilogue = [&](f32x4 (&Y)[NTILE], f32x4 (&DY)[NTILE], int z) {
-        int o[NT];
+    const bool edge_tile = !NOVEL && !F16 && a.mirror && (y0 == 0 || y0 + HP_ROWS >= a.Hv || x0 == 0 || x0 + HP_COLS >= a.Wv);
+    auto epilogue = [&](auto mirror, f32x4 (&Y)[NTILE], f32x4 (&DY)[NTILE], int z) {
+        constexpr bool MIRROR = decltype(mirror)::value;
+        int o[NT], em[MIRROR ? NT : 1];
         bool ook[NT], ook2[NT];
 #pragma unroll
         for (int nt = 0; nt < NT; ++nt) {
@@ -575,6 +578,7 @@
             ook[nt] = yy < a.Hv && xx < a.Wv;
             ook2[nt] = NOVEL && yy + HP_ROWS < a.Hv && xx < a.Wv;
             o[nt] = ook[nt] ? (z * a.Ho + yy) * a.Wo + xx : z * a.Ho * a.Wo;
+            if (MIRROR) em[nt] = ook[nt] ? halo_edges(yy, xx, a.Hv, a.Wv) : 0;
         }
         half4 r0[F16 ? NTILE : 1], r1[F16 ? NTILE : 1];
         const bool res = F16 && (a.flags & F_RES);
@@ -655,15 +659,30 @@
                     split4(v, hi, lo);
                     *(half4*)((char*)a.y + ob) = hi;
                     *(half4*)((char*)a.y + ol) = lo;
+                    if (MIRROR && em[MIRROR ? nt : 0])
+                        halo_images(em[MIRROR ? nt : 0], (long)a.Hv * a.Wo * 16, (long)a.Wv * 16, [&](long d) {
+                            *(half4*)((char*)a.y + ob + d) = hi;
+                            *(half4*)((char*)a.y + ol + d) = lo;
+                        });
                     split4(dv, hi, lo);
                     *(half4*)((char*)a.dy + ob) = hi;
                     *(half4*)((char*)a.dy + ol) = lo;
+                    if (MIRROR && em[MIRROR ? nt : 0])
+                        halo_images(em[MIRROR ? nt : 0], (long)a.Hv * a.Wo * 16, (long)a.Wv * 16, [&](long d) {
+                            *(half4*)((char*)a.dy + ob + d) = hi;
+                            *(half4*)((char*)a.dy + ol + d) = lo;
+                        });
                 }
             }
         }
     };
-    epilogue(YA, DA, z0);
-    epilogue(YB, DB, z0 + 1);
+    if (edge_tile) {
+        epilogue(std::true_type{}, YA, DA, z0);
+        epilogue(std::true_type{}, YB, DB, z0 + 1);
+    } else {
+        epilogue(std::false_type{}, YA, DA, z0);
+        epilogue(std::false_type{}, YB, DB, z0 + 1);
+    }
 }
 
 __global__ __launch_bounds__(256) void pack_h3w_kernel(const float* __restrict__ w, int cout, int cin, int nchunk, long total,
@@ -722,6 +741,7 @@
     wa.inv_scale = 1.0f / (f16 ? WINO_WSCALE_F16 : WINO_WSCALE);
     wa.r = ka.r; wa.dr = ka.dr; wa.res_pstride = ka.res_pstride;
     wa.zblock = std::min(8, ka.Dv / 2);
+    wa.mirror = ka.mirror;
     wa.nskip = ka.nskip; wa.dws_delta = ka.wws_set_floats * 4;
     static const int XI[2][2] = {{1, 2}, {0, 3}};
     static const int PA[4] = {0, 1, 2, 1}, PB[4] = {2, 2, 1, 3};
diff --git a/jax_nbody_emulator_with_dj_amd/engine.py b/jax_nbody_emulator_with_dj_amd/engine.py
--- a/jax_nbody_emulator_with_dj_amd/engine.py
+++ b/jax_nbody_emulator_with_dj_amd/engine.py
@@ -372,6 +372,29 @@
                 "gauge_out": g[2, :(m if not res else y.shape[0])],
                 "paths": {k for k, b in self.PATHS.items() if word.value & b}}
 
+    def test_block_halo(self, block, x, dx=None, x2=None, dx2=None, two_source=False):
+        x = _f32(x)
+        dx, x2, dx2 = (None if a is None else _f32(a) for a in (dx, x2, dx2))
+        m, vel = self.mid_chan, self.compute_vel
+        _, D, H, W = x.shape
+        h = None
+        if block.startswith('conv_'):
+            cout = self.out_chan if block == 'conv_r01' else m
+            cmid = 2 * m if block in ('conv_r2', 'conv_r1', 'conv_r00') else m
+            y = np.empty((cout, D - 4, H + 2, W + 2), np.float32)
+            h = np.empty((cmid, D - 2, H + 2, W + 2), np.float32)
+        elif block.startswith('down_'):
+            y = np.empty((m, D // 2, H // 2 + 2, W // 2 + 2), np.float32)
+        else:
+            y = np.empty((m if x2 is None else 2 * m, 2 * D, 2 * H + 2, 2 * W + 2), np.float32)
+        dy = np.empty_like(y) if vel else None
+        dh = np.empty_like(h) if (vel and h is not None) else None
+        word, nst = C.c_uint64(0), C.c_int(0)
+        check(self._l.nbe_test_block_halo(self._h, block.encode(), 1 if two_source else 0, _ptr(x), _ptr(dx), D, H, W,
+                                          _ptr(x2), _ptr(dx2), _ptr(y), _ptr(dy), _ptr(h), _ptr(dh), C.byref(word),
+                                          C.byref(nst)))
+        return {"y": y, "dy": dy, "h": h, "dh": dh, "ws_hash": word.value, "halos_stored": nst.value}
+
     def test_modulate(self, weight, style_weight, style_bias, s, first_layer, eps=1e-8, vel=True):
         weight, sw, sb = _f32(weight), _f32(style_weight), _f32(style_bias)
         cout, cin, k = weight.shape[:3]
```
